# mschubert/NMFconsensus

Measured on AMD Instinct MI355X. Metric: NMF restarts/sec (k=2..10 sweep, 20k×500 fp64) + fp64-MFMA/HBM roofline %, higher is better.
Workload: dtype f64

## Files before the change

### nmfconsensus_amd/build.py

```python
from __future__ import annotations

import os
import subprocess
import sys

HERE = os.path.dirname(os.path.abspath(__file__))
ROOT = os.path.dirname(HERE)
CSRC = os.path.join(HERE, "csrc")
LIB = os.path.join(HERE, "lib", "libnmf.so")
SOURCES = ["engine.hip", "compat.hip", "brunet.hip", "generic.hip", "solo.hip", "hclust.cpp"]
HEADERS = ["nmfc_kernels.hpp", "nmfc_tuning.hpp", "nmfc_internal.hpp", "lane_pool.hpp", "rmt.hpp", "../../include/nmfc.h", "../../include/libnmf_compat.h"]
ARCH = os.environ.get("NMFC_OFFLOAD_ARCH", "gfx950")
HIPCC = os.environ.get("HIPCC", "/opt/rocm/bin/hipcc")


def source_sha256() -> str:
    import hashlib
    h = hashlib.sha256()
    for f in ("nmfc_kernels.hpp", "engine.hip", "nmfc_tuning.hpp"):
        with open(os.path.join(CSRC, f), "rb") as fh:
            h.update(fh.read())
    return h.hexdigest()


def _stale(target: str, deps: list[str]) -> bool:
    if not os.path.exists(target):
        return True
    t = os.path.getmtime(target)
    return any(os.path.getmtime(d) > t for d in deps)


def build_lib(force: bool = False, verbose: bool = True) -> str:
    os.makedirs(os.path.dirname(LIB), exist_ok=True)
    deps = [os.path.join(CSRC, s) for s in SOURCES + HEADERS]
    if not force and not _stale(LIB, deps):
        return LIB
    from concurrent.futures import ThreadPoolExecutor

    def compile_one(src):
        obj = os.path.join(CSRC, os.path.splitext(src)[0] + ".o")
        lang = [] if src.endswith(".hip") else ["-x", "c++"]
        off = [f"--offload-arch={ARCH}"] if src.endswith(".hip") else []
        cmd = [HIPCC, *off, "-O3", "-fPIC", "-std=c++17", "-Wall", "-Wno-unused-result", "-Wno-unused-function", *lang, "-c",
               os.path.join(CSRC, src), "-o", obj]
        if verbose:
            print(" ".join(cmd), file=sys.stderr)
        subprocess.run(cmd, check=True, cwd=CSRC)
        return obj

    jobs = max(1, min(len(SOURCES), int(os.environ.get("MAX_JOBS", "6"))))
    with ThreadPoolExecutor(max_workers=jobs) as pool:
        objs = list(pool.map(compile_one, SOURCES))
    cmd = [HIPCC, f"--offload-arch={ARCH}", "-shared", "-fPIC", "-o", LIB, *objs,
           "-Wl,-soname,libnmf.so", "-Wl,-rpath,/opt/rocm/lib", "-Wl,-z,defs"]
    if verbose:
        print(" ".join(cmd), file=sys.stderr)
    subprocess.run(cmd, check=True, cwd=CSRC)
    for o in objs:
        os.remove(o)
    return LIB


def build_oracle(verbose: bool = True) -> None:
    odir = os.path.join(ROOT, "oracle")
    subprocess.run(["make", "-s", "-C", odir, "liboracle.so"], check=True)
    if os.path.isdir("/root/reference/libnmf"):
        subprocess.run(["make", "-s", "-C", odir, "ref"], check=True)


if __name__ == "__main__":
    build_lib(force="--force" in sys.argv)
    build_oracle()
```

### nmfconsensus_amd/csrc/engine.hip

```cpp
#include <hip/hip_runtime.h>

#include <algorithm>
#include <chrono>
#include <climits>
#include <cmath>
#include <cstdarg>
#include <cstdio>
#include <cstdlib>
#include <cstring>
#include <string>
#include <vector>

#include "../../include/nmfc.h"
#include "nmfc_internal.hpp"
#include "nmfc_kernels.hpp"

using namespace nmfc;

namespace {

thread_local std::string g_err;

void set_err(const char* fmt, ...) {
  char buf[512];
  va_list ap;
  va_start(ap, fmt);
  vsnprintf(buf, sizeof buf, fmt, ap);
  va_end(ap);
  g_err = buf;
}

#define HCHECK(expr)                                                                        \
  do {                                                                                      \
    hipError_t e_ = (expr);                                                                 \
    if (e_ != hipSuccess) {                                                                 \
      set_err("%s failed: %s (%s:%d)", #expr, hipGetErrorString(e_), __FILE__, __LINE__); \
      return -1;                                                                            \
    }                                                                                       \
  } while (0)

long round_up(long v, long a) { return (v + a - 1) / a * a; }

struct DevBuf {
  void* p = nullptr;
  size_t bytes = 0;
  DevBuf() = default;
  DevBuf(const DevBuf&) = delete;
  DevBuf& operator=(const DevBuf&) = delete;
  ~DevBuf() { release(); }
  int ensure(size_t need) {
    if (need <= bytes) return 0;
    if (p) (void)hipFree(p);
    p = nullptr;
    bytes = 0;
    if (need == 0) return 0;
    hipError_t e = hipMalloc(&p, need);
    if (e != hipSuccess) {
      set_err("hipMalloc(%zu) failed: %s", need, hipGetErrorString(e));
      p = nullptr;
      return -1;
    }
    bytes = need;
    return 0;
  }
  void release() {
    if (p) (void)hipFree(p);
    p = nullptr;
    bytes = 0;
  }
  template <class T>
  T* as() const {
    return static_cast<T*>(p);
  }
};

void mat_mul31(const uint32_t* A, const uint32_t* B, uint32_t* C) {
  for (int i = 0; i < 31; ++i)
    for (int j = 0; j < 31; ++j) {
      uint32_t s = 0;
      for (int q = 0; q < 31; ++q) s += A[i * 31 + q] * B[q * 31 + j];
      C[i * 31 + j] = s;
    }
}

std::vector<uint32_t> make_jump_table(int nchunks, int rchunk) {
  std::vector<uint32_t> M(31 * 31, 0), P(31 * 31, 0), T(31 * 31);
  for (int q = 0; q < 30; ++q) M[q * 31 + q + 1] = 1;
  M[30 * 31 + 0] = 1;
  M[30 * 31 + 28] += 1;
  for (int i = 0; i < 31; ++i) P[i * 31 + i] = 1;
  std::vector<uint32_t> base = M;
  for (int e = rchunk; e > 0; e >>= 1) {
    if (e & 1) {
      mat_mul31(P.data(), base.data(), T.data());
      P = T;
    }
    mat_mul31(base.data(), base.data(), T.data());
    base = T;
  }
  std::vector<uint32_t> table((size_t)std::max(nchunks, 1) * 961, 0);
  for (int i = 0; i < 31; ++i) table[i * 31 + i] = 1;
  for (int c = 1; c < nchunks; ++c) mat_mul31(P.data(), &table[(size_t)(c - 1) * 961], &table[(size_t)c * 961]);
  return table;
}

enum { KID_WTA = 0, KID_HUPD = 1, KID_AHTW = 2, KID_INIT = 3, KID_OTHER = 4, KID_LABELS = 5, KID_COUNTS = 6, KID_SMALL = 7, KID_RESID = 8, KID_N = 9 };

constexpr int WTA_NPT = 4;
constexpr int NARROW_NBUF = NMFC_NARROW_NBUF;
constexpr bool WTA_MID_GREG = NMFC_WTA_MID_GREG != 0;
constexpr bool SMALL_NW8 = NMFC_SMALL_NW8 != 0;
constexpr bool WTA_GREG = NMFC_WTA_GREG != 0;
constexpr bool WTA_W16 = NMFC_WTA_W16 != 0 && WTA_GREG;
constexpr int WTA_MID_NBUF = NMFC_WTA_MID_NBUF;
constexpr int WTA_MID_MINW = NMFC_WTA_MID_MINW;
constexpr int AHTW_NBUF = NMFC_AHTW_NBUF;
constexpr bool AHTW_LATE = NMFC_AHTW_LATE != 0;
struct Packing {
  std::vector<RestartInfo> ri;
  std::vector<int> prb, pre;
  std::vector<ColInfo> ci;
  int npanels = 0;
};

Packing pack(const std::vector<RestartInfo>& in) {
  std::vector<RestartInfo> srt(in);
  std::stable_sort(srt.begin(), srt.end(), [](const RestartInfo& a, const RestartInfo& b) {
    return a.k != b.k ? a.k > b.k : a.rid < b.rid;
  });
  std::vector<int> fill;
  std::vector<std::vector<RestartInfo>> members;
  size_t first_open = 0;
  for (RestartInfo r : srt) {
    size_t b = first_open;
    while (b < fill.size() && fill[b] + r.k > 16) ++b;
    if (b == fill.size()) {
      fill.push_back(0);
      members.emplace_back();
    }
    r.col0 = (int)b * 16 + fill[b];
    fill[b] += r.k;
    members[b].push_back(r);
    while (first_open < fill.size() && fill[first_open] > 14) ++first_open;
  }
  const int nblocks = (int)members.size();
  Packing pk;
  pk.npanels = std::max(1, (nblocks + 3) / 4);
  for (int p = 0; p < pk.npanels; ++p) {
    pk.prb.push_back((int)pk.ri.size());
    for (int b = 4 * p; b < std::min(nblocks, 4 * p + 4); ++b)
      for (const RestartInfo& r : members[b]) pk.ri.push_back(r);
    pk.pre.push_back((int)pk.ri.size());
  }
  while (pk.npanels % WTA_NPT) {
    pk.prb.push_back((int)in.size());
    pk.pre.push_back((int)in.size());
    ++pk.npanels;
  }
  pk.ci.assign((size_t)pk.npanels * PANEL, ColInfo{0, 0, 0, 0});
  for (const RestartInfo& r : pk.ri)
    for (int a = 0; a < r.k; ++a) pk.ci[r.col0 + a] = ColInfo{r.sq_off, r.col0 % PANEL, r.k, r.rid};
  return pk;
}

int narrow_blocks(const Packing& pk, int maxb) {
  if (pk.ri.empty()) return 0;
  int nb = 0;
  for (const RestartInfo& r : pk.ri) {
    if (r.col0 / 16 != (r.col0 + r.k - 1) / 16) return 0;
    nb = std::max(nb, (r.col0 + r.k + 15) / 16);
  }
  return nb <= maxb ? nb : 0;
}

Packing pack_small(const std::vector<RestartInfo>& in, std::vector<SmallBlock>& blocks) {
  std::vector<RestartInfo> srt(in);
  std::stable_sort(srt.begin(), srt.end(), [](const RestartInfo& a, const RestartInfo& b) {
    return a.k != b.k ? a.k > b.k : a.rid < b.rid;
  });
  std::vector<int> fill;
  blocks.clear();
  Packing pk;
  for (RestartInfo r : srt) {
    size_t b = 0;
    while (b < fill.size() && (fill[b] + r.k > 16 || blocks[b].nr == SMALL_MAXR)) ++b;
    if (b == fill.size()) {
      fill.push_back(0);
      SmallBlock sb{};
      sb.col0 = (int)b * 16;
      blocks.push_back(sb);
    }
    SmallBlock& sb = blocks[b];
    r.col0 = sb.col0 + fill[b];
    sb.rid[sb.nr] = r.rid;
    sb.k[sb.nr] = r.k;
    sb.lc0[sb.nr] = fill[b];
    ++sb.nr;
    fill[b] += r.k;
    pk.ri.push_back(r);
  }
  pk.npanels = std::max(1, (int)((blocks.size() * 16 + PANEL - 1) / PANEL));
  while (pk.npanels % WTA_NPT) ++pk.npanels;
  pk.prb.assign(pk.npanels, 0);
  pk.pre.assign(pk.npanels, 0);
  pk.ci.assign((size_t)pk.npanels * PANEL, ColInfo{0, 0, 0, 0});
  return pk;
}

int live_panels(const Packing& pk) {
  int np = 0;
  for (int p = 0; p < pk.npanels; ++p)
    if (pk.pre[p] > pk.prb[p]) np = p + 1;
  return np;
}

std::vector<SoloJob> place_solo(Packing& pk, std::vector<RestartInfo> solo, int col_base, int n) {
  std::stable_sort(solo.begin(), solo.end(), [n](const RestartInfo& a, const RestartInfo& b) {
    const int ka = nmfc_solo_batch_rank(n, a.k), kb = nmfc_solo_batch_rank(n, b.k);
    return ka != kb ? ka > kb : a.k != b.k ? a.k > b.k : a.rid < b.rid;
  });
  std::vector<SoloJob> jobs;
  int col = col_base;
  for (RestartInfo r : solo) {
    r.col0 = col;
    col += nmfc_solo_batch_rank(n, r.k) <= 4 ? 4 : 8;
    pk.ri.push_back(r);
    jobs.push_back(SoloJob{r.col0, r.k, r.rid, 0});
  }
  pk.npanels = std::max(pk.npanels, (col + PANEL - 1) / PANEL);
  while (pk.npanels % WTA_NPT) ++pk.npanels;
  pk.prb.assign(pk.npanels, 0);
  pk.pre.assign(pk.npanels, 0);
  pk.ci.assign((size_t)pk.npanels * PANEL, ColInfo{0, 0, 0, 0});
  return jobs;
}

}

void nmfc_set_error(const char* msg) { g_err = msg; }

struct nmfc_engine {
  int dev = 0;
  hipStream_t st = nullptr;
  int m = 0, n = 0;
  long m_pad = 0, n_pad = 0, n_cols_pad = 0;
  int kchunk = 0, nsplit = 0, ngt = 0;
  int ncu = 256;
  int force_wta = -1, force_ahtw = -1;
  int repack_div = 20;
  bool narrow_ok = true;
  int narrow_maxb = 3;
  bool small_ok = true;
  int small_kernel = 0;
  DevBuf Acm, Arm, Ablk;
  DevBuf W[2], H[2], Gpart, SWpart, SH, SHP, colact, Hfin, Wfin;
  DevBuf rinfo, stop_iter, stop_reason, unchanged, classes, n_stopped, Hstat, Wsnap;
  DevBuf prb, pre, colinfo, moves, finfo;
  DevBuf initjobs, chunk_job, chunk_idx, jump, labels, slot, grp_begin, grp_list, counts_tmp, cons_tmp, smallblk;
  DevBuf teamG, teamSW, teamFlag;
  DevBuf solojobs;
  bool narrow_lc = true;
  bool wta_sk = true;
  bool wta_sk_mid = true;
  bool wta_lastsum = false;
  int sk_dp_xcd = 0;
  DevBuf skfix, skflag, sktcnt;
  unsigned sk_epoch = 0;
  bool gram_model = true;
  bool solo_ok = true;
  hipStream_t aux[4] = {nullptr, nullptr, nullptr, nullptr};
  hipEvent_t fork_ev = nullptr, join_ev[4] = {nullptr, nullptr, nullptr, nullptr};
  int team_occ = 0;
  DevBuf mu1_dev, mu1_G, mu1_SW, mu1_flag;
  char* mu1_host = nullptr;
  size_t mu1_host_bytes = 0;
  int mu1_base = -1;
  int mu1_kprev = 16;
  int jump_chunks = 0, jump_rchunk = 0;
  int* h_stopped = nullptr;
  bool timing = false;
  int timing_stride = 1;
  std::vector<hipEvent_t> ev_pool;
  struct Pending {
    int kid;
    hipEvent_t a, b;
  };
  std::vector<Pending> pending;
  double kms[KID_N] = {0};
  long long kcount[KID_N] = {0};
  long long klaunch[KID_N] = {0};
  double kflops[KID_N] = {0};
  double kbytes[KID_N] = {0};
  double kbytes_algo[KID_N] = {0};
  int repacks = 0;
  struct RunInfo {
    int small = 0, repacks_skipped = 0, polls = 0, iterations_enqueued = 0, panels_first = 0, panels_min = 0;
    long long wta_narrow = 0, wta_sk = 0, wta_big = 0, wta_mid = 0, wta_small = 0, wta_tiny = 0;
    long long ahtw_narrow = 0, ahtw_128 = 0, ahtw_64 = 0;
  } info;
  std::string info_str;
  bool residuals = false, resid_valid = false;
  DevBuf ssq, respart;
  std::vector<double> h_ssq;
  std::vector<int> last_ks, last_row;
  long last_jb = 0;
};

namespace {

struct TileChoice {
  int wta;
  bool ahtw_small;
};

constexpr double WTA_SK_COST = 1.01;
bool sk_big_ok(const nmfc_engine* e, int ntj) { return e->wta_sk && WTA_W16 && ntj >= 4; }
bool sk_mid_ok(const nmfc_engine* e, int ntj) { return e->wta_sk && e->wta_sk_mid && WTA_MID_GREG && ntj >= 4; }
bool sk_grid_fits(const nmfc_engine* e, long ngroups, int ntj) {
  const long ipc = ngroups * ntj, nitems = ipc * e->nsplit;
  const long nst_full = e->kchunk / 16, nst_last = (e->m_pad - (long)(e->nsplit - 1) * e->kchunk) / 16;
  const long nst_max = e->nsplit > 1 ? nst_full : nst_last;
  const long S = ipc * (e->nsplit - 1) * nst_full + ipc * nst_last;
  return nitems >= e->ncu && S >= (long)e->ncu * nst_max;
}
int sk_groups(const nmfc_engine* e, int tile, int big_panels, int mid_panels, int ntj) {
  const bool big = tile == 0 && sk_big_ok(e, ntj), mid = tile == 3 && sk_mid_ok(e, ntj);
  if (!big && !mid) return 0;
  const int ng = big ? (big_panels + WTA_NPT - 1) / WTA_NPT : (mid_panels + 1) / 2;
  return sk_grid_fits(e, ng, ntj) ? ng : 0;
}

TileChoice choose_tiles(const nmfc_engine* e, int np_live, int ntj) {
  const long ns = e->nsplit, cu = e->ncu;
  const long np = std::max(np_live, 1);
  struct Cand {
    int id;
    double wgs;
    long slots;
    double t;
  } cands[4] = {{0, (double)(ns * ((np + 3) / 4) * ntj), cu, 2.0},
                {3, (double)(ns * ((np + 1) / 2) * ntj), cu, 1.0},
                {1, (double)(ns * np) * (2 * ntj + (e->gram_model ? 0.75 : 0.0)), 3 * cu, 0.8},
                {2, (double)(ns * np) * (4 * ntj + (e->gram_model ? 1.5 : 0.0)), 4 * cu, 0.6}};
  TileChoice tc{0, false};
  double best = 1e300;
  for (const Cand& c : cands) {
    const bool sk = sk_groups(e, c.id, (int)np, (int)np, ntj) > 0;
    const double est = sk ? c.wgs / (double)c.slots * c.t * WTA_SK_COST : std::ceil(c.wgs / (double)c.slots) * c.t;
    if (est < best - 1e-9) {
      best = est;
      tc.wta = c.id;
    }
  }
  tc.ahtw_small = np * e->ngt < 16 * cu;
  if (e->force_wta >= 0) tc.wta = e->force_wta;
  if (e->force_ahtw >= 0) tc.ahtw_small = e->force_ahtw == 1;
  return tc;
}

template <int GBW, int NW>
hipError_t launch_small_g(nmfc_engine* e, int nblocks, int maxiter, int stop_rule) {
  const int jb = (e->n + 15) / 16;
  auto args = [&](auto kern) {
    hipLaunchKernelGGL(kern, dim3(nblocks), dim3(64 * NW), 0, e->st, e->smallblk.as<SmallBlock>(),
                       e->Arm.as<double>(), e->n_pad, e->Acm.as<double>(), e->m_pad, e->n, e->n_pad,
                       e->W[0].as<double>(), e->H[0].as<double>(), maxiter, stop_rule, e->stop_iter.as<int>(),
                       e->stop_reason.as<int>());
  };
  switch (jb) {
    case 1: args(k_small_mu<GBW, 1, 0, NW>); break;
    case 2: args(k_small_mu<GBW, 2, 0, NW>); break;
    case 3: args(k_small_mu<GBW, 3, 0, NW>); break;
    default: args(k_small_mu<GBW, 4, 0, NW>); break;
  }
  return hipGetLastError();
}

int team_count(nmfc_engine* e, int nblocks) {
  const int P = (int)(e->m_pad / TEAM_ROWS);
  if (!e->team_occ) {
    int occ = 0;
    if (hipOccupancyMaxActiveBlocksPerMultiprocessor(&occ, k_team_mu<4>, 256, 0) != hipSuccess || occ < 1) occ = 1;
    e->team_occ = std::min(occ, 6);
  }
  return std::max(1, std::min(nblocks, (int)((long)e->team_occ * e->ncu / P)));
}

int launch_team(nmfc_engine* e, int nblocks, int maxiter, int stop_rule) {
  const int jb = (e->n + 15) / 16;
  const int P = (int)(e->m_pad / TEAM_ROWS);
  if (e->m_pad % TEAM_ROWS != 0 || P > TEAM_PMAX || jb < 1 || jb > 4) {
    set_err("k_team_mu: m_pad %ld / n %d unsupported", e->m_pad, e->n);
    return -1;
  }
  auto kern = jb == 1 ? k_team_mu<1> : jb == 2 ? k_team_mu<2> : jb == 3 ? k_team_mu<3> : k_team_mu<4>;
  const int nteams = team_count(e, nblocks);
  const long np = 16L * jb;
  if (e->teamG.ensure(sizeof(double) * nteams * 2 * TEAM_PMAX * 16 * np) ||
      e->teamSW.ensure(sizeof(double) * nteams * 2 * TEAM_PMAX * 256) ||
      e->teamFlag.ensure(sizeof(unsigned) * (nteams * TEAM_PMAX + 16)))
    return -1;
  HCHECK(hipMemsetAsync(e->teamFlag.p, 0, sizeof(unsigned) * (nteams * TEAM_PMAX + 16), e->st));
  hipLaunchKernelGGL(kern, dim3(nteams * P), dim3(256), 0, e->st, e->smallblk.as<SmallBlock>(), nblocks, P,
                     e->Acm.as<double>(), e->m_pad, e->n, e->n_pad, e->W[0].as<double>(), e->H[0].as<double>(), maxiter,
                     stop_rule, e->stop_iter.as<int>(), e->stop_reason.as<int>(), e->teamG.as<double>(),
                     e->teamSW.as<double>(), e->teamFlag.as<unsigned>(), 0u,
                     reinterpret_cast<int*>(e->teamFlag.as<unsigned>() + nteams * TEAM_PMAX), nullptr);
  hipError_t err = hipGetLastError();
  if (err != hipSuccess) {
    set_err("k_team_mu launch: %s", hipGetErrorString(err));
    return -1;
  }
  return 0;
}

int team_failed(nmfc_engine* e, int nblocks) {
  int v = 0;
  const unsigned* w = e->teamFlag.as<unsigned>() + team_count(e, nblocks) * TEAM_PMAX;
  if (hipMemcpy(&v, w, sizeof(int), hipMemcpyDeviceToHost) != hipSuccess) return 1;
  return v != 0;
}

bool use_team(nmfc_engine* e, int nblocks) {
  (void)nblocks;
  return e->small_kernel == 1;
}

int launch_small(nmfc_engine* e, int nblocks, int maxiter, int stop_rule) {
  if (use_team(e, nblocks)) return launch_team(e, nblocks, maxiter, stop_rule);
  hipError_t err;
  const int jb = (e->n + 15) / 16;
  if (e->m_pad % 64 != 0 || e->n_pad != (jb <= 2 ? 32 : 64)) {
    set_err("k_small_mu: m_pad %ld / n_pad %ld unsupported for n = %d", e->m_pad, e->n_pad, e->n);
    return -1;
  }
  if (SMALL_NW8 && e->m_pad % 256 == 0) {
    switch (e->m_pad / 128) {
      case 2: err = launch_small_g<2, 8>(e, nblocks, maxiter, stop_rule); break;
      case 4: err = launch_small_g<4, 8>(e, nblocks, maxiter, stop_rule); break;
      case 6: err = launch_small_g<6, 8>(e, nblocks, maxiter, stop_rule); break;
      case 8: err = launch_small_g<8, 8>(e, nblocks, maxiter, stop_rule); break;
      default: set_err("k_small_mu: m_pad %ld unsupported", e->m_pad); return -1;
    }
  } else {
    switch (e->m_pad / 64) {
      case 2: err = launch_small_g<2, 4>(e, nblocks, maxiter, stop_rule); break;
      case 4: err = launch_small_g<4, 4>(e, nblocks, maxiter, stop_rule); break;
      case 6: err = launch_small_g<6, 4>(e, nblocks, maxiter, stop_rule); break;
      case 8: err = launch_small_g<8, 4>(e, nblocks, maxiter, stop_rule); break;
      case 10: err = launch_small_g<10, 4>(e, nblocks, maxiter, stop_rule); break;
      case 12: err = launch_small_g<12, 4>(e, nblocks, maxiter, stop_rule); break;
      case 14: err = launch_small_g<14, 4>(e, nblocks, maxiter, stop_rule); break;
      case 16: err = launch_small_g<16, 4>(e, nblocks, maxiter, stop_rule); break;
      default: set_err("k_small_mu: m_pad %ld unsupported", e->m_pad); return -1;
    }
  }
  if (err != hipSuccess) {
    set_err("k_small_mu launch: %s", hipGetErrorString(err));
    return -1;
  }
  return 0;
}

hipEvent_t take_event(nmfc_engine* e) {
  if (!e->ev_pool.empty()) {
    hipEvent_t ev = e->ev_pool.back();
    e->ev_pool.pop_back();
    return ev;
  }
  hipEvent_t ev;
  if (hipEventCreate(&ev) != hipSuccess) return nullptr;
  return ev;
}

void drain_timing(nmfc_engine* e) {
  for (auto& pnd : e->pending) {
    float ms = 0.f;
    if (hipEventSynchronize(pnd.b) == hipSuccess && hipEventElapsedTime(&ms, pnd.a, pnd.b) == hipSuccess) {
      e->kms[pnd.kid] += ms;
      e->kcount[pnd.kid] += 1;
    }
    e->ev_pool.push_back(pnd.a);
    e->ev_pool.push_back(pnd.b);
  }
  e->pending.clear();
}

struct TimedLaunch {
  nmfc_engine* e;
  int kid;
  hipEvent_t a = nullptr;
  TimedLaunch(nmfc_engine* e_, int kid_, bool sample = true) : e(e_), kid(kid_) {
    e->klaunch[kid] += 1;
    if (e->timing && sample) {
      a = take_event(e);
      if (a) (void)hipEventRecord(a, e->st);
    }
  }
  ~TimedLaunch() {
    if (a) {
      hipEvent_t b = take_event(e);
      if (b) {
        (void)hipEventRecord(b, e->st);
        e->pending.push_back({kid, a, b});
      } else {
        e->ev_pool.push_back(a);
      }
    }
  }
};


struct PollEvents {
  hipEvent_t ev[2] = {nullptr, nullptr};
  ~PollEvents() {
    for (hipEvent_t x : ev)
      if (x) (void)hipEventDestroy(x);
  }
};

struct Sweep {
  nmfc_engine* e = nullptr;
  nmfc_sweep_opts opts;
  const int* ks = nullptr;
  int nk = 0, R = 0;
  long jb = 0;
  int nj = 0;
  std::vector<RestartInfo> all;
  std::vector<int> rslot;
  std::vector<int> hoff;
  long sw_total = 0;
  bool small = false;
  Packing pk;
  std::vector<SmallBlock> sblocks;
  std::vector<SoloJob> solo;
  long cap_cols = 0;
  int ntj = 0;
  long g_ld = 0, g_split = 0, cls_ld = 0;
  bool want_w = false, tolx = false;
  int cur = 0;
  int nact = 0;
  std::vector<char> archived;
  std::vector<int> si, sr;
  int it = 0;
  int polls = 0, checked = 0;
  int stopped_at_pack = 0;
  PollEvents pe;
  long long tot_iters = 0;
  int max_it = 0;
  std::vector<RestartInfo> fin;
  int job_k(int s) const { return ks[(jb + s) % nk]; }
};

void factor_offsets(const Sweep& s, std::vector<long>& woff, std::vector<long>& ho) {
  woff.assign(s.nj + 1, 0);
  ho.assign(s.nj + 1, 0);
  for (int j = 0; j < s.nj; ++j) {
    woff[j + 1] = woff[j] + (long)s.e->m * s.job_k(j);
    ho[j + 1] = ho[j] + (long)s.job_k(j) * s.e->n;
  }
}

void transpose(const double* src, int rows, int cols, double* dst) {
  for (int r = 0; r < rows; ++r)
    for (int c = 0; c < cols; ++c) dst[(size_t)c * rows + r] = src[(size_t)r * cols + c];
}

int check_args(Sweep& s, nmfc_engine* e, const int* ks, int nk, int R, const nmfc_sweep_opts* opts_in) {
  if (!e || !ks || nk <= 0 || R <= 0) {
    set_err("nmfc_engine_run: bad arguments");
    return -1;
  }
  s.e = e;
  s.ks = ks;
  s.nk = nk;
  s.R = R;
  nmfc_sweep_opts& opts = s.opts;
  if (opts_in)
    opts = *opts_in;
  else
    nmfc_default_opts(&opts);
  if (opts.check_every <= 0) opts.check_every = 4;
  const int m = e->m, n = e->n;
  for (int i = 0; i < nk; ++i) {
    if (ks[i] < 2 || ks[i] > KMAX || ks[i] > n || ks[i] > m) {
      set_err("nmfc_engine_run: k=%d unsupported (need 2 <= k <= min(%d, m, n))", ks[i], KMAX);
      return -1;
    }
    if ((long)m * ks[i] + (long)ks[i] * n + 31L * 32 >= (long)INT_MAX) {
      set_err("nmfc_engine_run: m k + k n = %ld draws per restart exceeds the init kernel's 32-bit index range",
              (long)m * ks[i] + (long)ks[i] * n);
      return -1;
    }
  }
  if (opts.maxiter < 0) {
    set_err("nmfc_engine_run: maxiter must be >= 0");
    return -1;
  }
  if (opts.stop_rule < 0 || opts.stop_rule > 3 || opts.label_rule < 0 || opts.label_rule > 1 ||
      opts.init_stream < 0 || opts.init_stream > 1) {
    set_err("nmfc_engine_run: bad stop rule, label rule or init stream");
    return -1;
  }
  HCHECK(hipSetDevice(e->dev));
  return 0;
}

int plan_jobs(Sweep& s) {
  nmfc_engine* e = s.e;
  const int m = e->m, n = e->n;
  const long njobs_all = (long)s.nk * s.R;
  const long jb = std::max(0, s.opts.job_begin);
  const long je = (s.opts.job_end < 0) ? njobs_all : std::min<long>(s.opts.job_end, njobs_all);
  if (jb >= je) {
    set_err("nmfc_engine_run: empty job range [%ld, %ld)", jb, je);
    return -1;
  }
  s.jb = jb;
  const int nj = s.nj = (int)(je - jb);

  std::vector<int> order(nj);
  for (int i = 0; i < nj; ++i) order[i] = i;
  std::stable_sort(order.begin(), order.end(), [&](int a, int b) { return s.job_k(a) > s.job_k(b); });
  s.all.resize(nj);
  s.rslot.resize(nj);
  s.hoff.assign(nj + 1, 0);
  for (int rid = 0; rid < nj; ++rid) {
    RestartInfo& r = s.all[rid];
    r.k = s.job_k(order[rid]);
    r.rid = rid;
    r.sq_off = (int)s.sw_total;
    r.col0 = 0;
    s.rslot[rid] = order[rid];
    s.sw_total += (long)r.k * r.k;
    s.hoff[rid + 1] = s.hoff[rid] + r.k;
  }
  s.small = e->small_ok && e->m_pad <= 1024 && n <= 64 && s.opts.stop_rule != NMFC_STOP_TOLX;
  std::vector<RestartInfo> blk_jobs, solo_jobs;
  for (const RestartInfo& r : s.all)
    (s.small && e->solo_ok && nmfc_mu_solo_fits(m, n, r.k) ? solo_jobs : blk_jobs).push_back(r);
  s.pk = s.small ? pack_small(blk_jobs, s.sblocks) : pack(s.all);
  if (s.small && !solo_jobs.empty()) s.solo = place_solo(s.pk, solo_jobs, (int)s.sblocks.size() * 16, n);
  s.cap_cols = (long)s.pk.npanels * PANEL;
  e->info.small = s.small;
  e->info.panels_first = e->info.panels_min = s.pk.npanels;
  s.ntj = (int)(e->n_cols_pad / 128);
  s.g_ld = e->n_cols_pad;
  s.g_split = s.cap_cols * s.g_ld;
  s.cls_ld = std::max<long>(n, KMAX);
  s.tolx = s.opts.stop_rule == NMFC_STOP_TOLX;
  s.nact = nj;
  s.archived.assign(nj, 0);
  s.si.assign(nj, 0);
  s.sr.assign(nj, 0);
  return 0;
}

int upload_packing(nmfc_engine* e, const Packing& p) {
  hipStream_t st = e->st;
  HCHECK(hipMemcpyAsync(e->rinfo.p, p.ri.data(), sizeof(RestartInfo) * std::max<size_t>(p.ri.size(), 1),
                        hipMemcpyHostToDevice, st));
  HCHECK(hipMemcpyAsync(e->prb.p, p.prb.data(), sizeof(int) * p.npanels, hipMemcpyHostToDevice, st));
  HCHECK(hipMemcpyAsync(e->pre.p, p.pre.data(), sizeof(int) * p.npanels, hipMemcpyHostToDevice, st));
  HCHECK(hipMemcpyAsync(e->colinfo.p, p.ci.data(), sizeof(ColInfo) * p.ci.size(), hipMemcpyHostToDevice, st));
  return 0;
}

int ensure_buffers(Sweep& s) {
  nmfc_engine* e = s.e;
  const int n = e->n, nj = s.nj;
  const long cap_cols = s.cap_cols, fin_rows = s.hoff[nj];
  const Packing& pk = s.pk;
  if (e->W[0].ensure(sizeof(double) * cap_cols * e->m_pad) || e->H[0].ensure(sizeof(double) * cap_cols * e->n_pad) ||
      e->W[1].ensure(sizeof(double) * cap_cols * e->m_pad) || e->H[1].ensure(sizeof(double) * cap_cols * e->n_pad) ||
      e->Gpart.ensure(sizeof(double) * s.g_split * e->nsplit) || e->SWpart.ensure(sizeof(double) * s.sw_total * e->nsplit) ||
      e->SH.ensure(sizeof(double) * s.sw_total) || e->Hfin.ensure(sizeof(double) * fin_rows * e->n_pad) ||
      e->SHP.ensure(sizeof(double) * cap_cols * KMAX) || e->colact.ensure(sizeof(int) * cap_cols) ||
      (s.want_w && e->Wfin.ensure(sizeof(double) * fin_rows * e->m_pad)) || e->rinfo.ensure(sizeof(RestartInfo) * nj) ||
      e->finfo.ensure(sizeof(RestartInfo) * nj) || e->stop_iter.ensure(sizeof(int) * nj) ||
      e->stop_reason.ensure(sizeof(int) * nj) || e->unchanged.ensure(sizeof(int) * nj) ||
      e->classes.ensure(sizeof(int) * nj * s.cls_ld) || e->n_stopped.ensure(sizeof(int)) ||
      e->prb.ensure(sizeof(int) * pk.npanels) || e->pre.ensure(sizeof(int) * pk.npanels) ||
      e->colinfo.ensure(sizeof(ColInfo) * pk.npanels * PANEL) ||
      e->moves.ensure(sizeof(MoveJob) * nj) || e->labels.ensure(sizeof(int32_t) * (size_t)nj * n) ||
      e->slot.ensure(sizeof(int) * nj) || e->Hstat.ensure(sizeof(double) * nj))
    return -1;
  if (s.tolx && e->Wsnap.ensure(sizeof(double) * cap_cols * e->m_pad)) return -1;
  hipStream_t st = e->st;
  if (upload_packing(e, pk)) return -1;
  HCHECK(hipMemcpyAsync(e->slot.p, s.rslot.data(), sizeof(int) * nj, hipMemcpyHostToDevice, st));
  HCHECK(hipMemsetAsync(e->stop_iter.p, 0, sizeof(int) * nj, st));
  HCHECK(hipMemsetAsync(e->stop_reason.p, 0, sizeof(int) * nj, st));
  HCHECK(hipMemsetAsync(e->unchanged.p, 0, sizeof(int) * nj, st));
  HCHECK(hipMemsetAsync(e->classes.p, 0, sizeof(int) * nj * s.cls_ld, st));
  HCHECK(hipMemsetAsync(e->n_stopped.p, 0, sizeof(int), st));
  HCHECK(hipMemsetAsync(e->colact.p, 0, sizeof(int) * cap_cols, st));
  HCHECK(hipMemsetAsync(e->W[0].p, 0, sizeof(double) * cap_cols * e->m_pad, st));
  HCHECK(hipMemsetAsync(e->H[0].p, 0, sizeof(double) * cap_cols * e->n_pad, st));
  HCHECK(hipMemsetAsync(e->W[1].p, 0, sizeof(double) * cap_cols * e->m_pad, st));
  HCHECK(hipMemsetAsync(e->H[1].p, 0, sizeof(double) * cap_cols * e->n_pad, st));
  return 0;
}

int init_from_caller(Sweep& s, const double* W_init, const double* H_init) {
  nmfc_engine* e = s.e;
  hipStream_t st = e->st;
  const int m = e->m, n = e->n;
  std::vector<long> woff, ho;
  factor_offsets(s, woff, ho);
  std::vector<double> hrow;
  for (const RestartInfo& r : s.pk.ri) {
    const int j = s.rslot[r.rid], k = r.k;
    HCHECK(hipMemcpy2DAsync(e->W[0].as<double>() + (long)r.col0 * e->m_pad, sizeof(double) * e->m_pad,
                            W_init + woff[j], sizeof(double) * m, sizeof(double) * m, k, hipMemcpyHostToDevice, st));
    hrow.assign((size_t)k * n, 0.0);
    transpose(H_init + ho[j], n, k, hrow.data());
    HCHECK(hipMemcpy2DAsync(e->H[0].as<double>() + (long)r.col0 * e->n_pad, sizeof(double) * e->n_pad, hrow.data(),
                            sizeof(double) * n, sizeof(double) * n, k, hipMemcpyHostToDevice, st));
    HCHECK(hipStreamSynchronize(st));
  }
  return 0;
}

int init_r_runif(Sweep& s) {
  nmfc_engine* e = s.e;
  hipStream_t st = e->st;
  const int nj = s.nj;
  std::vector<InitJob> ij(nj);
  for (int i = 0; i < nj; ++i) {
    const RestartInfo& r = s.pk.ri[i];
    ij[i] = InitJob{(uint32_t)(s.opts.seed + (uint32_t)(s.jb + s.rslot[r.rid])), r.col0, r.k, 0};
  }
  if (e->initjobs.ensure(sizeof(InitJob) * nj)) return -1;
  HCHECK(hipMemcpyAsync(e->initjobs.p, ij.data(), sizeof(InitJob) * nj, hipMemcpyHostToDevice, st));
  {
    TimedLaunch tl(e, KID_INIT);
    hipLaunchKernelGGL(k_init_runif, dim3(nj), dim3(NT), 0, st, e->initjobs.as<InitJob>(), e->m, e->n, e->m_pad,
                       e->n_pad, e->W[0].as<double>(), e->H[0].as<double>());
  }
  HCHECK(hipGetLastError());
  HCHECK(hipStreamSynchronize(st));
  return 0;
}

int init_glibc(Sweep& s) {
  nmfc_engine* e = s.e;
  hipStream_t st = e->st;
  const int m = e->m, n = e->n, nj = s.nj;
  const Packing& pk = s.pk;
  std::vector<InitJob> ij(nj);
  std::vector<int> cj, ci;
  int maxch = 1;
  long draws = 0;
  for (int i = 0; i < nj; ++i) draws += (long)m * pk.ri[i].k + (long)pk.ri[i].k * n;
  int rchunk = RCHUNK;
  while (rchunk > 62 && draws / rchunk < 65536) rchunk /= 2;
  for (int i = 0; i < nj; ++i) {
    const RestartInfo& r = pk.ri[i];
    const long total = (long)m * r.k + (long)r.k * n;
    const int nch = (int)((total + rchunk - 1) / rchunk);
    ij[i].seed = (uint32_t)(s.opts.seed + (uint32_t)(s.jb + s.rslot[r.rid]));
    ij[i].col0 = r.col0;
    ij[i].k = r.k;
    ij[i].nchunks = nch;
    maxch = std::max(maxch, nch);
    for (int c = 0; c < nch; ++c) {
      cj.push_back(i);
      ci.push_back(c);
    }
  }
  if (maxch > e->jump_chunks || rchunk != e->jump_rchunk) {
    std::vector<uint32_t> tab = make_jump_table(maxch, rchunk);
    if (e->jump.ensure(sizeof(uint32_t) * tab.size())) return -1;
    HCHECK(hipMemcpyAsync(e->jump.p, tab.data(), sizeof(uint32_t) * tab.size(), hipMemcpyHostToDevice, st));
    HCHECK(hipStreamSynchronize(st));
    e->jump_chunks = maxch;
    e->jump_rchunk = rchunk;
  }
  if (e->initjobs.ensure(sizeof(InitJob) * nj) || e->chunk_job.ensure(sizeof(int) * cj.size()) ||
      e->chunk_idx.ensure(sizeof(int) * ci.size()))
    return -1;
  HCHECK(hipMemcpyAsync(e->initjobs.p, ij.data(), sizeof(InitJob) * nj, hipMemcpyHostToDevice, st));
  HCHECK(hipMemcpyAsync(e->chunk_job.p, cj.data(), sizeof(int) * cj.size(), hipMemcpyHostToDevice, st));
  HCHECK(hipMemcpyAsync(e->chunk_idx.p, ci.data(), sizeof(int) * ci.size(), hipMemcpyHostToDevice, st));
  const int total_chunks = (int)cj.size();
  {
    TimedLaunch tl(e, KID_INIT);
    hipLaunchKernelGGL(k_init, dim3((total_chunks + NT - 1) / NT), dim3(NT), 0, st, e->initjobs.as<InitJob>(),
                       e->chunk_job.as<int>(), e->chunk_idx.as<int>(), total_chunks, e->jump.as<uint32_t>(), rchunk / 31,
                       m, n, e->m_pad, e->n_pad, s.opts.min_init, s.opts.max_init, e->W[0].as<double>(),
                       e->H[0].as<double>());
  }
  HCHECK(hipGetLastError());
  HCHECK(hipStreamSynchronize(st));
  return 0;
}

int archive(Sweep& s, const std::vector<RestartInfo>& list) {
  if (list.empty()) return 0;
  nmfc_engine* e = s.e;
  hipStream_t st = e->st;
  std::vector<MoveJob> mv(list.size());
  for (size_t x = 0; x < list.size(); ++x) mv[x] = {list[x].col0, s.hoff[list[x].rid], list[x].k};
  HCHECK(hipMemcpyAsync(e->moves.p, mv.data(), sizeof(MoveJob) * mv.size(), hipMemcpyHostToDevice, st));
  {
    TimedLaunch tl(e, KID_OTHER);
    hipLaunchKernelGGL(k_move_rows, dim3((unsigned)mv.size(), 2), dim3(NT), 0, st, e->moves.as<MoveJob>(),
                       e->H[s.cur].as<double>(), e->n_pad, e->Hfin.as<double>(), e->n_pad, e->n_pad);
    if (s.want_w)
      hipLaunchKernelGGL(k_move_rows, dim3((unsigned)mv.size(), 16), dim3(NT), 0, st, e->moves.as<MoveJob>(),
                         e->W[s.cur].as<double>(), e->m_pad, e->Wfin.as<double>(), e->m_pad, e->m_pad);
  }
  HCHECK(hipGetLastError());
  HCHECK(hipStreamSynchronize(st));
  for (const RestartInfo& r : list) s.archived[r.rid] = 1;
  return 0;
}

int archive_rest(Sweep& s) {
  std::vector<RestartInfo> rest;
  for (const RestartInfo& r : s.pk.ri)
    if (!s.archived[r.rid]) rest.push_back(r);
  return archive(s, rest);
}

int launch_solo_beside_blocks(Sweep& s) {
  nmfc_engine* e = s.e;
  const int n = e->n;
  const std::vector<SoloJob>& solo = s.solo;
  const long free_cu = std::max<long>(1, e->ncu - (long)s.sblocks.size());
  auto wt = [](int kp) -> long { return kp <= 2 ? 4 : kp <= 4 ? 6 : 12; };
  long wsum = 0;
  for (const SoloJob& job : solo) wsum += wt(nmfc_solo_batch_rank(n, job.k));
  std::vector<std::pair<size_t, size_t>> groups;
  for (size_t g0 = 0; g0 < solo.size();) {
    const int kp = nmfc_solo_batch_rank(n, solo[g0].k);
    size_t g1 = g0;
    while (g1 < solo.size() && nmfc_solo_batch_rank(n, solo[g1].k) == kp) ++g1;
    groups.emplace_back(g0, g1);
    g0 = g1;
  }
  for (int g = 0; g < (int)groups.size(); ++g) {
    const size_t g0 = groups[g].first, g1 = groups[g].second;
    const int kp = nmfc_solo_batch_rank(n, solo[g0].k);
    const long nq = (long)(g1 - g0);
    const long share = std::min<long>(nq, std::max<long>(1, free_cu * nq * wt(kp) / wsum));
    HCHECK(hipStreamWaitEvent(e->aux[g], e->fork_ev, 0));
    if (nmfc_solo_batch_launch(e->Acm.as<double>(), e->m_pad, e->m, n, e->W[0].as<double>(), e->m_pad,
                               e->H[0].as<double>(), e->n_pad, e->solojobs.as<SoloJob>() + g0, (int)nq, kp,
                               s.opts.maxiter, s.opts.stop_rule, e->stop_iter.as<int>(), e->stop_reason.as<int>(),
                               (int)share, e->aux[g]))
      return -1;
    HCHECK(hipEventRecord(e->join_ev[g], e->aux[g]));
  }
  for (int g = 0; g < (int)groups.size(); ++g) HCHECK(hipStreamWaitEvent(e->st, e->join_ev[g], 0));
  return 0;
}

int small_phase(Sweep& s) {
  nmfc_engine* e = s.e;
  hipStream_t st = e->st;
  const std::vector<SmallBlock>& sblocks = s.sblocks;
  const std::vector<SoloJob>& solo = s.solo;
  if (!sblocks.empty()) {
    if (e->smallblk.ensure(sizeof(SmallBlock) * sblocks.size())) return -1;
    HCHECK(hipMemcpyAsync(e->smallblk.p, sblocks.data(), sizeof(SmallBlock) * sblocks.size(), hipMemcpyHostToDevice, st));
  }
  if (!solo.empty()) {
    if (e->solojobs.ensure(sizeof(SoloJob) * solo.size())) return -1;
    HCHECK(hipMemcpyAsync(e->solojobs.p, solo.data(), sizeof(SoloJob) * solo.size(), hipMemcpyHostToDevice, st));
    for (int x = 0; x < 4; ++x) {
      if (!e->aux[x]) HCHECK(hipStreamCreateWithFlags(&e->aux[x], hipStreamNonBlocking));
      if (!e->join_ev[x]) HCHECK(hipEventCreateWithFlags(&e->join_ev[x], hipEventDisableTiming));
    }
    if (!e->fork_ev) HCHECK(hipEventCreateWithFlags(&e->fork_ev, hipEventDisableTiming));
  }
  {
    TimedLaunch tl(e, KID_SMALL);
    const bool team = use_team(e, (int)sblocks.size());
    if (!solo.empty() && !team) HCHECK(hipEventRecord(e->fork_ev, st));
    if (!sblocks.empty() && launch_small(e, (int)sblocks.size(), s.opts.maxiter, s.opts.stop_rule)) return -1;
    if (!solo.empty() && (sblocks.empty() || team)) {
      if (nmfc_solo_batch_launch(e->Acm.as<double>(), e->m_pad, e->m, e->n, e->W[0].as<double>(), e->m_pad,
                                 e->H[0].as<double>(), e->n_pad, e->solojobs.as<SoloJob>(), (int)solo.size(), 0,
                                 s.opts.maxiter, s.opts.stop_rule, e->stop_iter.as<int>(), e->stop_reason.as<int>(),
                                 (int)solo.size(), st))
        return -1;
    } else if (!solo.empty()) {
      if (launch_solo_beside_blocks(s)) return -1;
    }
  }
  HCHECK(hipStreamSynchronize(st));
  if (!sblocks.empty() && use_team(e, (int)sblocks.size()) && team_failed(e, (int)sblocks.size())) {
    set_err("k_team_mu: a team of workgroups could not meet (not co-resident?)");
    return -1;
  }
  if (e->timing) drain_timing(e);
  s.it = s.opts.maxiter;
  return 0;
}


using Wta2Kernel = decltype(&k_wta2<1, 64, 2, 2, 1, GT_NBUF, 1, true, true, true>);
using AhtwKernel = decltype(&k_ahtw4<GT, AHTW_NBUF, 1, PANEL, 4, AHTW_LATE>);

void launch_wta_narrow(const Sweep& s, int nblk) {
  nmfc_engine* e = s.e;
  const int ntq = (int)(e->n_cols_pad / 16);
  auto kn = e->narrow_lc ? k_wta_narrow_lc<16, NARROW_NBUF, true> : k_wta_narrow<16, NARROW_NBUF, true>;
  ++e->info.wta_narrow;
  hipLaunchKernelGGL(kn, dim3(e->nsplit * nblk * (ntq + 1)), dim3(e->narrow_lc ? 128 : 64), 0, e->st,
                     e->W[s.cur].as<double>(), e->Ablk.as<double>(), e->m_pad, ntq, e->nsplit, e->kchunk, nblk,
                     e->colinfo.as<ColInfo>(), e->Gpart.as<double>(), s.g_ld, s.g_split, e->SWpart.as<double>(),
                     s.sw_total);
}

int launch_wta_sk(Sweep& s, bool big, int ng, int* gsplit) {
  nmfc_engine* e = s.e;
  hipStream_t st = e->st;
  if (!e->skflag.p) {
    if (e->skfix.ensure(sizeof(double) * SK_FIX * e->ncu) || e->skflag.ensure(sizeof(unsigned) * e->ncu)) return -1;
    HCHECK(hipMemsetAsync(e->skflag.p, 0, sizeof(unsigned) * e->ncu, st));
  }
  ++e->info.wta_sk;
  const long tiles = (long)ng * s.ntj;
  const bool lastsum = e->wta_lastsum && big;
  if (lastsum && e->sktcnt.bytes < sizeof(unsigned) * tiles) {
    if (e->sktcnt.ensure(sizeof(unsigned) * tiles)) return -1;
    HCHECK(hipMemsetAsync(e->sktcnt.p, 0, sizeof(unsigned) * tiles, st));
  }
  const SkArgs a{e->W[s.cur].as<double>(), e->Ablk.as<double>(), e->m_pad, ng, s.ntj, e->kchunk,
                 e->prb.as<int>(), e->pre.as<int>(), e->rinfo.as<RestartInfo>(), e->colinfo.as<ColInfo>(),
                 e->stop_iter.as<int>(), e->Gpart.as<double>(), s.g_ld, s.g_split, e->SWpart.as<double>(), s.sw_total,
                 e->skfix.as<double>(), e->skflag.as<unsigned>(), ++e->sk_epoch, e->nsplit,
                 e->sktcnt.as<unsigned>(), e->sk_dp_xcd};
  if (!big) {
    hipLaunchKernelGGL((k_wta2_sk<WTA_MID_NBUF, false, false, 2>), dim3(e->ncu), dim3(SK_THREADS / 2), 0, st, a);
  } else if (lastsum) {
    hipLaunchKernelGGL((k_wta2_sk<GT_NBUF, false, true>), dim3(e->ncu), dim3(SK_THREADS), 0, st, a);
    *gsplit = 1;
  } else {
    hipLaunchKernelGGL(k_wta2_sk<GT_NBUF>, dim3(e->ncu), dim3(SK_THREADS), 0, st, a);
  }
  return 0;
}

struct Wta2Launch {
  Wta2Kernel kern;
  int threads;
  int ngroups;
  int tiles;
  int gram_wgs;
  int tile;
};

Wta2Launch pick_wta2(const nmfc_engine* e, int tile, int ntj, int live, int npanels) {
  const int lp = std::max(1, live);
  if (tile == 0) {
    Wta2Kernel kw = (ntj >= 4)   ? (WTA_W16 ? k_wta2<WTA_NPT, 128, 4, 4, 1, GT_NBUF, 1, true, true, false, true>
                                            : k_wta2<WTA_NPT, 128, 4, 2, 1, GT_NBUF, 1, true, true, false, WTA_GREG>)
                    : (ntj >= 2) ? k_wta2<WTA_NPT, 128, 4, 2, 2, GT_NBUF, 1, true>
                                 : k_wta2<WTA_NPT, 128, 4, 2, 4, GT_NBUF, 1, true>;
    return {kw, (ntj >= 4 && WTA_W16) ? 1024 : 512, npanels / WTA_NPT, ntj, 0, 0};
  }
  if (tile == 3) {
    Wta2Kernel kw = (ntj >= 4 && WTA_MID_GREG) ? k_wta2<2, 128, 2, 4, 1, WTA_MID_NBUF, WTA_MID_MINW, true, true, false, true>
                    : (ntj >= 2)               ? k_wta2<2, 128, 4, 2, 1, WTA_MID_NBUF, WTA_MID_MINW, true>
                                               : k_wta2<2, 128, 4, 2, 2, WTA_MID_NBUF, WTA_MID_MINW, true>;
    return {kw, 512, (lp + 1) / 2, ntj, 0, 3};
  }
  if (tile != 2)
    return {k_wta2<1, 64, 2, 2, 1, GT_NBUF, 1, true, true, true>, 256, lp, 2 * ntj, 3, 1};
  Wta2Kernel kw = (long)e->nsplit * live * 4 * ntj <= e->ncu ? k_wta2<1, 32, 4, 1, 1, 8, 1, true, true, true>
                                                             : k_wta2<1, 32, 4, 1, 1, GT_NBUF, 1, true, true, true>;
  return {kw, 256, lp, 4 * ntj, 3, 2};
}

void launch_wta2(const Sweep& s, const Wta2Launch& l) {
  nmfc_engine* e = s.e;
  ++(l.tile == 0 ? e->info.wta_big : l.tile == 3 ? e->info.wta_mid : l.tile == 1 ? e->info.wta_small : e->info.wta_tiny);
  hipLaunchKernelGGL(l.kern, dim3(e->nsplit * l.ngroups * (l.tiles + l.gram_wgs)), dim3(l.threads), 0, e->st,
                     e->W[s.cur].as<double>(), e->Ablk.as<double>(), e->m_pad, l.ngroups, l.tiles, e->nsplit, e->kchunk,
                     e->prb.as<int>(), e->pre.as<int>(), e->rinfo.as<RestartInfo>(), e->colinfo.as<ColInfo>(),
                     e->stop_iter.as<int>(), e->Gpart.as<double>(), s.g_ld, s.g_split, e->SWpart.as<double>(),
                     s.sw_total);
}

struct ChunkPlan {
  TileChoice tc;
  int nblk;
  int live;
  int lp;
  int ngt_ahtw, grid_ahtw;
  AhtwKernel ka;
};

int launch_wta(Sweep& s, const ChunkPlan& cp, int* gsplit) {
  if (cp.nblk > 0) {
    launch_wta_narrow(s, cp.nblk);
  } else if (const int ng = sk_groups(s.e, cp.tc.wta, s.pk.npanels, cp.lp, s.ntj)) {
    return launch_wta_sk(s, cp.tc.wta == 0, ng, gsplit);
  } else {
    launch_wta2(s, pick_wta2(s.e, cp.tc.wta, s.ntj, cp.live, s.pk.npanels));
  }
  return 0;
}

void launch_hupdate(const Sweep& s, int iter, int gsplit) {
  nmfc_engine* e = s.e;
  hipLaunchKernelGGL(k_hupdate<>, dim3(s.nact), dim3(NTH), 0, e->st, iter, s.opts.maxiter, s.opts.stop_rule,
                     e->rinfo.as<RestartInfo>(), e->n, e->n_pad, e->Gpart.as<double>(), s.g_ld, s.g_split, gsplit,
                     e->nsplit, e->SWpart.as<double>(), s.sw_total, e->H[s.cur].as<double>(), e->SH.as<double>(),
                     e->stop_iter.as<int>(), e->stop_reason.as<int>(), e->unchanged.as<int>(),
                     e->classes.as<int>(), s.cls_ld, e->n_stopped.as<int>(), e->SHP.as<double>(),
                     e->colact.as<int>(), e->Hstat.as<double>());
}

void launch_ahtw(const Sweep& s, const ChunkPlan& cp, int iter) {
  nmfc_engine* e = s.e;
  ++(cp.nblk > 0 ? e->info.ahtw_narrow : cp.tc.ahtw_small ? e->info.ahtw_64 : e->info.ahtw_128);
  if (cp.nblk > 0)
    hipLaunchKernelGGL((k_ahtw4<GT / 4, GT_NBUF, 1, 16, 2>), dim3(4 * e->ngt * cp.nblk), dim3(128), 0, e->st,
                       iter, e->H[s.cur].as<double>(), e->n_pad, e->Arm.as<double>(), e->m_pad,
                       e->W[s.cur].as<double>(), e->SHP.as<double>(), e->colinfo.as<ColInfo>(),
                       e->colact.as<int>(), cp.nblk, 4 * e->ngt);
  else
    hipLaunchKernelGGL(cp.ka, dim3(cp.grid_ahtw), dim3(256), 0, e->st, iter, e->H[s.cur].as<double>(), e->n_pad,
                       e->Arm.as<double>(), e->m_pad, e->W[s.cur].as<double>(), e->SHP.as<double>(),
                       e->colinfo.as<ColInfo>(), e->colact.as<int>(), cp.lp, cp.ngt_ahtw);
}

ChunkPlan plan_chunk(const Sweep& s) {
  const nmfc_engine* e = s.e;
  ChunkPlan cp;
  cp.live = live_panels(s.pk);
  cp.lp = std::max(1, cp.live);
  cp.tc = choose_tiles(e, cp.live, s.ntj);
  cp.nblk = e->narrow_ok ? narrow_blocks(s.pk, e->narrow_maxb) : 0;
  cp.ngt_ahtw = e->ngt * (cp.tc.ahtw_small ? 2 : 1);
  cp.grid_ahtw = cp.lp * cp.ngt_ahtw;
  const bool kh = AHTW_KSKIP && AHTW_NBUF == 2 && e->n_pad - e->n >= 8;
  cp.ka = cp.tc.ahtw_small ? (kh ? k_ahtw4<GT / 2, AHTW_NBUF, 1, PANEL, 4, AHTW_LATE, AHTW_NBUF == 2>
                                 : k_ahtw4<GT / 2, AHTW_NBUF, 1, PANEL, 4, AHTW_LATE>)
                           : (kh ? k_ahtw4<GT, AHTW_NBUF, 1, PANEL, 4, AHTW_LATE, AHTW_NBUF == 2>
                                 : k_ahtw4<GT, AHTW_NBUF, 1, PANEL, 4, AHTW_LATE>);
  return cp;
}

void launch_wstat(const Sweep& s, int iter) {
  nmfc_engine* e = s.e;
  hipLaunchKernelGGL(k_wstat, dim3(s.nact), dim3(NT), 0, e->st, iter, e->rinfo.as<RestartInfo>(),
                     e->W[s.cur].as<double>(), e->Wsnap.as<double>(), e->m_pad, e->m, e->colact.as<int>(),
                     e->Hstat.as<double>(), s.opts.TolX, s.opts.TolFun, e->stop_iter.as<int>(),
                     e->stop_reason.as<int>(), e->n_stopped.as<int>());
}

int enqueue_iteration(Sweep& s, const ChunkPlan& cp, int iter) {
  nmfc_engine* e = s.e;
  const bool sample = iter % e->timing_stride == 0;
  int gsplit = e->nsplit;
  {
    TimedLaunch tl(e, KID_WTA, sample);
    if (launch_wta(s, cp, &gsplit)) return -1;
  }
  {
    TimedLaunch tl(e, KID_HUPD, sample);
    launch_hupdate(s, iter, gsplit);
  }
  const bool tol_check = s.tolx && iter > 1 && iter % 2 == 0;
  if (tol_check)
    HCHECK(hipMemcpyAsync(e->Wsnap.p, e->W[s.cur].p, sizeof(double) * (size_t)s.pk.npanels * PANEL * e->m_pad,
                          hipMemcpyDeviceToDevice, e->st));
  {
    TimedLaunch tl(e, KID_AHTW, sample);
    launch_ahtw(s, cp, iter);
  }
  if (tol_check) {
    TimedLaunch tl(e, KID_OTHER);
    launch_wstat(s, iter);
  }
  return 0;
}

int enqueue_chunk(Sweep& s) {
  nmfc_engine* e = s.e;
  const int chunk = std::min(s.opts.check_every, s.opts.maxiter - s.it);
  const ChunkPlan cp = plan_chunk(s);
  for (int c = 1; c <= chunk; ++c)
    if (enqueue_iteration(s, cp, s.it + c)) return -1;
  HCHECK(hipGetLastError());
  s.it += chunk;
  HCHECK(hipMemcpyAsync(&e->h_stopped[s.polls & 1], e->n_stopped.p, sizeof(int), hipMemcpyDeviceToHost, e->st));
  HCHECK(hipEventRecord(s.pe.ev[s.polls & 1], e->st));
  ++s.polls;
  return 0;
}

int consume_polls(Sweep& s, int* stopped, bool* done) {
  const int target = (s.it < s.opts.maxiter) ? s.polls - 1 : s.polls;
  while (s.checked < target) {
    HCHECK(hipEventSynchronize(s.pe.ev[s.checked & 1]));
    *stopped = s.e->h_stopped[s.checked & 1];
    if (*stopped >= s.nj) *done = true;
    ++s.checked;
  }
  return 0;
}

int repack(Sweep& s, int stopped) {
  nmfc_engine* e = s.e;
  hipStream_t st = e->st;
  const int nj = s.nj;
  HCHECK(hipStreamSynchronize(st));
  if (e->timing) drain_timing(e);
  s.checked = s.polls;
  HCHECK(hipMemcpy(s.si.data(), e->stop_iter.p, sizeof(int) * nj, hipMemcpyDeviceToHost));
  std::vector<RestartInfo> gone, live;
  for (const RestartInfo& r : s.pk.ri) {
    if (!s.si[r.rid])
      live.push_back(r);
    else if (!s.archived[r.rid])
      gone.push_back(r);
  }
  if (archive(s, gone)) return -1;
  Packing np = pack(live);
  if ((long)np.npanels * PANEL > s.cap_cols) {
    s.stopped_at_pack = stopped;
    ++e->info.repacks_skipped;
    return 0;
  }
  std::vector<int> old_col(nj, -1);
  for (const RestartInfo& r : live) old_col[r.rid] = r.col0;
  std::vector<MoveJob> mv(np.ri.size());
  for (size_t x = 0; x < np.ri.size(); ++x) mv[x] = {old_col[np.ri[x].rid], np.ri[x].col0, np.ri[x].k};
  if (!mv.empty()) {
    HCHECK(hipMemcpyAsync(e->moves.p, mv.data(), sizeof(MoveJob) * mv.size(), hipMemcpyHostToDevice, st));
    {
      TimedLaunch tl(e, KID_OTHER);
      hipLaunchKernelGGL(k_move_rows, dim3((unsigned)mv.size(), 16), dim3(NT), 0, st, e->moves.as<MoveJob>(),
                         e->W[s.cur].as<double>(), e->m_pad, e->W[s.cur ^ 1].as<double>(), e->m_pad, e->m_pad);
      hipLaunchKernelGGL(k_move_rows, dim3((unsigned)mv.size(), 2), dim3(NT), 0, st, e->moves.as<MoveJob>(),
                         e->H[s.cur].as<double>(), e->n_pad, e->H[s.cur ^ 1].as<double>(), e->n_pad, e->n_pad);
    }
    HCHECK(hipGetLastError());
  }
  s.cur ^= 1;
  s.pk = np;
  if (upload_packing(e, s.pk)) return -1;
  HCHECK(hipStreamSynchronize(st));
  s.nact = (int)s.pk.ri.size();
  s.stopped_at_pack = nj - s.nact;
  ++e->repacks;
  e->info.panels_min = std::min(e->info.panels_min, s.pk.npanels);
  return 0;
}

int mfma_loop(Sweep& s) {
  nmfc_engine* e = s.e;
  HCHECK(hipEventCreateWithFlags(&s.pe.ev[0], hipEventDisableTiming));
  HCHECK(hipEventCreateWithFlags(&s.pe.ev[1], hipEventDisableTiming));
  for (;;) {
    if (s.it < s.opts.maxiter && enqueue_chunk(s)) return -1;
    int stopped = 0;
    bool done = false;
    if (consume_polls(s, &stopped, &done)) return -1;
    if (e->timing) drain_timing(e);
    if (done || (s.it >= s.opts.maxiter && s.checked == s.polls)) break;
    if (stopped - s.stopped_at_pack >= std::max(1, s.nact / e->repack_div)) {
      if (repack(s, stopped)) return -1;
      if (s.nact == 0) break;
    }
  }
  return 0;
}

int residual_pass(Sweep& s) {
  nmfc_engine* e = s.e;
  if (!e->residuals) return 0;
  hipStream_t st = e->st;
  const int nj = s.nj;
  const int nst = (e->n + RES_ST - 1) / RES_ST, ntiles = (e->m + RES_GT - 1) / RES_GT * nst;
  const int ngroups = (nj + RES_JG - 1) / RES_JG;
  if (ngroups > 65535) {
    set_err("nmfc_engine_run: residuals of %d jobs exceed the residual pass's grid", nj);
    return -1;
  }
  if (e->ssq.ensure(sizeof(double) * nj) || e->respart.ensure(sizeof(double) * (size_t)nj * ntiles)) return -1;
  s.fin.resize(nj);
  for (int rid = 0; rid < nj; ++rid) s.fin[rid] = {s.hoff[rid], s.all[rid].k, rid, s.all[rid].sq_off};
  HCHECK(hipMemcpyAsync(e->finfo.p, s.fin.data(), sizeof(RestartInfo) * nj, hipMemcpyHostToDevice, st));
  {
    TimedLaunch tl(e, KID_RESID);
    hipLaunchKernelGGL(k_resid, dim3(ntiles, ngroups), dim3(NT), 0, st, e->finfo.as<RestartInfo>(), nj,
                       e->Ablk.as<double>(), e->n_cols_pad, e->Wfin.as<double>(), e->m_pad, e->Hfin.as<double>(), e->n_pad,
                       e->m, e->n, nst, e->respart.as<double>());
    hipLaunchKernelGGL(k_resid_sum, dim3(nj), dim3(64), 0, st, e->respart.as<double>(), ntiles, e->slot.as<int>(),
                       e->ssq.as<double>());
  }
  HCHECK(hipGetLastError());
  e->h_ssq.assign(nj, 0.0);
  HCHECK(hipMemcpyAsync(e->h_ssq.data(), e->ssq.p, sizeof(double) * nj, hipMemcpyDeviceToHost, st));
  double fl = 0, bw = 0, bh = 0;
  for (int rid = 0; rid < nj; ++rid) {
    const double k = s.all[rid].k;
    fl += (2.0 * k + 3.0) * e->m * e->n;
    bw += 8.0 * k * e->m;
    bh += 8.0 * k * e->n;
  }
  const double a_bytes = 8.0 * e->m * e->n;
  e->kflops[KID_RESID] = fl;
  e->kbytes_algo[KID_RESID] = a_bytes + bw + bh + 8.0 * nj;
  e->kbytes[KID_RESID] = a_bytes * ngroups + bw * nst + bh * (ntiles / nst) + 16.0 * nj * ntiles + 8.0 * nj;
  return 0;
}

int labels_counts_consensus(Sweep& s, nmfc_result* out) {
  nmfc_engine* e = s.e;
  hipStream_t st = e->st;
  const int n = e->n, nj = s.nj, nk = s.nk;
  std::vector<RestartInfo> fin(nj);
  for (int rid = 0; rid < nj; ++rid) fin[rid] = {s.hoff[rid], s.all[rid].k, rid, s.all[rid].sq_off};
  HCHECK(hipMemcpyAsync(e->finfo.p, fin.data(), sizeof(RestartInfo) * nj, hipMemcpyHostToDevice, st));
  {
    TimedLaunch tl(e, KID_LABELS);
    hipLaunchKernelGGL(k_labels, dim3((n + NT - 1) / NT, nj), dim3(NT), 0, st, e->finfo.as<RestartInfo>(),
                       e->slot.as<int>(), e->Hfin.as<double>(), e->n_pad, n, s.opts.label_rule, e->labels.as<int32_t>());
  }
  HCHECK(hipGetLastError());
  std::vector<int> gb(nk + 1, 0), gl;
  for (int g = 0; g < nk; ++g) {
    gb[g] = (int)gl.size();
    for (int j = 0; j < nj; ++j)
      if ((s.jb + j) % nk == g) gl.push_back(j);
  }
  gb[nk] = (int)gl.size();
  const size_t cnt_len = (size_t)nk * n * n;
  if (out && (out->counts || out->consensus)) {
    if (e->grp_begin.ensure(sizeof(int) * (nk + 1)) || e->grp_list.ensure(sizeof(int) * std::max<size_t>(gl.size(), 1)))
      return -1;
    HCHECK(hipMemcpyAsync(e->grp_begin.p, gb.data(), sizeof(int) * (nk + 1), hipMemcpyHostToDevice, st));
    if (!gl.empty()) HCHECK(hipMemcpyAsync(e->grp_list.p, gl.data(), sizeof(int) * gl.size(), hipMemcpyHostToDevice, st));
    int32_t* dcounts;
    if (out->counts && out->counts_on_device) {
      dcounts = out->counts;
    } else {
      if (e->counts_tmp.ensure(sizeof(int32_t) * cnt_len)) return -1;
      dcounts = e->counts_tmp.as<int32_t>();
    }
    {
      TimedLaunch tl(e, KID_COUNTS);
      hipLaunchKernelGGL(k_counts, dim3((n + CNT_T - 1) / CNT_T, (n + CNT_T - 1) / CNT_T, nk), dim3(NT), 0, st, e->labels.as<int32_t>(),
                         e->grp_begin.as<int>(), e->grp_list.as<int>(), n, dcounts);
    }
    HCHECK(hipGetLastError());
    if (out->consensus) {
      if (e->cons_tmp.ensure(sizeof(double) * cnt_len)) return -1;
      hipLaunchKernelGGL(k_divide, dim3((unsigned)((cnt_len + NT - 1) / NT)), dim3(NT), 0, st, dcounts, (double)s.R,
                         (long)cnt_len, e->cons_tmp.as<double>());
      HCHECK(hipGetLastError());
      HCHECK(hipMemcpyAsync(out->consensus, e->cons_tmp.p, sizeof(double) * cnt_len, hipMemcpyDeviceToHost, st));
    }
    if (out->counts && !out->counts_on_device)
      HCHECK(hipMemcpyAsync(out->counts, dcounts, sizeof(int32_t) * cnt_len, hipMemcpyDeviceToHost, st));
  }
  HCHECK(hipMemcpyAsync(s.si.data(), e->stop_iter.p, sizeof(int) * nj, hipMemcpyDeviceToHost, st));
  HCHECK(hipMemcpyAsync(s.sr.data(), e->stop_reason.p, sizeof(int) * nj, hipMemcpyDeviceToHost, st));
  if (out && out->labels)
    HCHECK(hipMemcpyAsync(out->labels, e->labels.p, sizeof(int32_t) * (size_t)nj * n, hipMemcpyDeviceToHost, st));
  HCHECK(hipStreamSynchronize(st));
  if (e->timing) drain_timing(e);
  return 0;
}

void account_kernels(Sweep& s, nmfc_result* out) {
  nmfc_engine* e = s.e;
  const int m = e->m, n = e->n, nj = s.nj;
  double fl_wta = 0, fl_ahtw = 0;
  double b_wta = 0, ba_wta = 0, b_ahtw = 0, ba_ahtw = 0, b_hupd = 0, ba_hupd = 0, b_lab = 0;
  const double ns = e->nsplit;
  for (int rid = 0; rid < nj; ++rid) {
    const int itr = s.si[rid] ? s.si[rid] : s.it;
    s.tot_iters += itr;
    s.max_it = std::max(s.max_it, itr);
    const double k = s.all[rid].k;
    fl_wta += (double)itr * (2.0 * m * n * k + 2.0 * m * k * k);
    fl_ahtw += (double)itr * (2.0 * m * n * k + 2.0 * m * k * k);
    ba_wta += itr * 8.0 * k * (m + n);
    b_wta += itr * 8.0 * k * (m + ns * n + ns * k);
    ba_ahtw += itr * 8.0 * k * (2.0 * m + n);
    b_ahtw += itr * 8.0 * k * (2.0 * m + n + KMAX);
    ba_hupd += itr * 32.0 * n * k;
    b_hupd += itr * 8.0 * (k * n * (ns + 2.0) + k * k * (ns + 2.0) + k * KMAX);
    b_lab += 8.0 * k * n + 4.0 * n;
    if (out && out->iters) out->iters[s.rslot[rid]] = itr;
    if (out && out->stopped_early) out->stopped_early[s.rslot[rid]] = (s.sr[rid] == 1 || s.sr[rid] == 3);
  }
  const double a_bytes = 8.0 * m * n;
  if (const long long c = e->klaunch[KID_WTA]) {
    e->kflops[KID_WTA] = fl_wta / c;
    e->kbytes_algo[KID_WTA] = a_bytes + ba_wta / c;
    e->kbytes[KID_WTA] = a_bytes + b_wta / c;
  }
  if (const long long c = e->klaunch[KID_AHTW]) {
    e->kflops[KID_AHTW] = fl_ahtw / c;
    e->kbytes_algo[KID_AHTW] = a_bytes + ba_ahtw / c;
    e->kbytes[KID_AHTW] = a_bytes + b_ahtw / c;
  }
  if (const long long c = e->klaunch[KID_SMALL]) {
    e->kflops[KID_SMALL] = (fl_wta + fl_ahtw) / c;
    e->kbytes_algo[KID_SMALL] = (ba_wta + ba_ahtw + ba_hupd) / c;
    e->kbytes[KID_SMALL] = e->kbytes_algo[KID_SMALL];
  }
  if (const long long c = e->klaunch[KID_HUPD]) {
    e->kbytes_algo[KID_HUPD] = ba_hupd / c;
    e->kbytes[KID_HUPD] = b_hupd / c;
  }
  if (e->klaunch[KID_LABELS]) e->kbytes[KID_LABELS] = e->kbytes_algo[KID_LABELS] = b_lab;
  if (e->klaunch[KID_COUNTS]) {
    e->kbytes_algo[KID_COUNTS] = 4.0 * nj * n + 4.0 * s.nk * n * n;
    e->kbytes[KID_COUNTS] = e->kbytes_algo[KID_COUNTS];
  }
}

int download_factors(Sweep& s, nmfc_result* out) {
  if (!out || !(out->W || out->H)) return 0;
  nmfc_engine* e = s.e;
  hipStream_t st = e->st;
  const int m = e->m, n = e->n;
  std::vector<long> woff, ho;
  factor_offsets(s, woff, ho);
  std::vector<double> hrow;
  for (int rid = 0; rid < s.nj; ++rid) {
    const int j = s.rslot[rid], k = s.all[rid].k;
    if (out->W)
      HCHECK(hipMemcpy2DAsync(out->W + woff[j], sizeof(double) * m, e->Wfin.as<double>() + (long)s.hoff[rid] * e->m_pad,
                              sizeof(double) * e->m_pad, sizeof(double) * m, k, hipMemcpyDeviceToHost, st));
    if (out->H) {
      hrow.assign((size_t)k * n, 0.0);
      HCHECK(hipMemcpy2DAsync(hrow.data(), sizeof(double) * n, e->Hfin.as<double>() + (long)s.hoff[rid] * e->n_pad,
                              sizeof(double) * e->n_pad, sizeof(double) * n, k, hipMemcpyDeviceToHost, st));
      HCHECK(hipStreamSynchronize(st));
      transpose(hrow.data(), k, n, out->H + ho[j]);
    }
  }
  HCHECK(hipStreamSynchronize(st));
  return 0;
}

}

extern "C" {

const char* nmfc_last_error(void) { return g_err.c_str(); }

const char* nmfc_build_tuning(void) { return NMFC_TUNING_MU; }
const char* nmfc_version(void) { return "nmfconsensus_amd 0.2 (gfx950, fp64 MFMA)"; }

void nmfc_default_opts(nmfc_sweep_opts* o) {
  memset(o, 0, sizeof *o);
  o->maxiter = 10000;
  o->stop_rule = NMFC_STOP_REF_COMPAT;
  o->label_rule = NMFC_LABEL_ARGMAX;
  o->seed = 123;
  o->min_init = 0;
  o->max_init = 1;
  o->job_begin = 0;
  o->job_end = -1;
  o->check_every = 4;
  o->verbose = 0;
  o->TolX = 1.0E-04;
  o->TolFun = 1.0E-04;
}

nmfc_engine* nmfc_engine_create(int device, const double* A, int m, int n, int a_on_device) {
  if (!A || m <= 0 || n <= 0) {
    set_err("nmfc_engine_create: bad arguments (A=%p m=%d n=%d)", (const void*)A, m, n);
    return nullptr;
  }
  nmfc_engine* e = new nmfc_engine();
  auto fail = [&](const char* what, hipError_t err) -> nmfc_engine* {
    set_err("nmfc_engine_create: %s: %s", what, hipGetErrorString(err));
    nmfc_engine_destroy(e);
    return nullptr;
  };
  hipError_t err;
  if (device >= 0) {
    if ((err = hipSetDevice(device)) != hipSuccess) return fail("hipSetDevice", err);
  }
  if ((err = hipGetDevice(&e->dev)) != hipSuccess) return fail("hipGetDevice", err);
  {
    int ncu = 0;
    if (hipDeviceGetAttribute(&ncu, hipDeviceAttributeMultiprocessorCount, e->dev) == hipSuccess && ncu > 0) e->ncu = ncu;
  }
  if (const char* s = getenv("NMFC_WTA_TILE")) {
    const std::string v(s);
    e->force_wta = v == "big" ? 0 : v == "small" ? 1 : v == "tiny" ? 2 : v == "mid" ? 3 : -1;
  }
  if (const char* s = getenv("NMFC_REPACK_DIV")) e->repack_div = std::max(1, atoi(s));
  if (const char* s = getenv("NMFC_NARROW")) e->narrow_ok = atoi(s) != 0;
  if (const char* s = getenv("NMFC_NARROW_MAXB")) e->narrow_maxb = std::min(8, std::max(1, atoi(s)));
  if (const char* s = getenv("NMFC_SMALL")) e->small_ok = atoi(s) != 0;
  if (const char* s = getenv("NMFC_SOLO")) e->solo_ok = atoi(s) != 0;
  if (const char* s = getenv("NMFC_NARROW_LC")) e->narrow_lc = atoi(s) != 0;
  if (const char* s = getenv("NMFC_WTA_SK")) e->wta_sk = atoi(s) != 0;
  if (const char* s = getenv("NMFC_WTA_SK_MID")) e->wta_sk_mid = atoi(s) != 0;
  if (const char* s = getenv("NMFC_WTA_LASTSUM")) e->wta_lastsum = atoi(s) != 0;
  if (const char* s = getenv("NMFC_SK_DP_XCD")) e->sk_dp_xcd = atoi(s) != 0;
  if (const char* s = getenv("NMFC_GRAM_MODEL")) e->gram_model = atoi(s) != 0;
  if (const char* s = getenv("NMFC_SMALL_KERNEL"))
    e->small_kernel = std::string(s) == "team" ? 1 : std::string(s) == "single" ? 2 : 0;
  if (const char* s = getenv("NMFC_AHTW_TILE")) {
    const std::string v(s);
    e->force_ahtw = v == "128" ? 0 : v == "64" ? 1 : -1;
  }
  if ((err = hipStreamCreateWithFlags(&e->st, hipStreamNonBlocking)) != hipSuccess) return fail("hipStreamCreate", err);
  if ((err = hipHostMalloc((void**)&e->h_stopped, 2 * sizeof(int), 0)) != hipSuccess) return fail("hipHostMalloc", err);
  e->m = m;
  e->n = n;
  e->m_pad = round_up(m, GT);
  e->n_pad = round_up(n, BK);
  e->n_cols_pad = round_up(n, 128);
  e->ngt = (int)(e->m_pad / GT);
  int kchunk = 2048;
  if (const char* v = getenv("NMFC_KCHUNK")) {
    const int x = atoi(v);
    if (x == 512 || x == 1024 || x == 2048 || x == 4096) kchunk = x;
  }
  e->kchunk = (int)std::min<long>(kchunk, e->m_pad);
  e->nsplit = (int)((e->m_pad + e->kchunk - 1) / e->kchunk);
  const bool small_shape = e->m_pad <= (long)TEAM_ROWS * TEAM_PMAX && n <= 64;
  if ((small_shape && e->Acm.ensure(sizeof(double) * e->n_cols_pad * e->m_pad)) ||
      e->Ablk.ensure(sizeof(double) * e->n_cols_pad * e->m_pad) || e->Arm.ensure(sizeof(double) * e->m_pad * e->n_pad)) {
    nmfc_engine_destroy(e);
    return nullptr;
  }
  if (small_shape && (err = hipMemsetAsync(e->Acm.p, 0, e->Acm.bytes, e->st)) != hipSuccess) return fail("memset", err);
  if ((err = hipMemsetAsync(e->Ablk.p, 0, e->Ablk.bytes, e->st)) != hipSuccess) return fail("memset", err);
  if ((err = hipMemsetAsync(e->Arm.p, 0, e->Arm.bytes, e->st)) != hipSuccess) return fail("memset", err);
  const double* dA = A;
  DevBuf tmp;
  if (!a_on_device) {
    if (tmp.ensure(sizeof(double) * (size_t)m * n)) {
      nmfc_engine_destroy(e);
      return nullptr;
    }
    if ((err = hipMemcpyAsync(tmp.p, A, sizeof(double) * (size_t)m * n, hipMemcpyHostToDevice, e->st)) != hipSuccess)
      return fail("upload A", err);
    dA = tmp.as<double>();
  }
  dim3 grid((m + NT - 1) / NT, n);
  hipLaunchKernelGGL(k_layout_a, grid, dim3(NT), 0, e->st, dA, (long)m, m, n, e->m_pad, e->n_pad,
                     small_shape ? e->Acm.as<double>() : nullptr, e->Arm.as<double>());
  hipLaunchKernelGGL(k_layout_ablk, dim3((unsigned)((m + NT - 1) / NT), (unsigned)((n + 15) / 16)), dim3(NT), 0,
                     e->st, dA, (long)m, m, n, e->n_cols_pad, e->Ablk.as<double>());
  if ((err = hipGetLastError()) != hipSuccess) return fail("k_layout_a", err);
  if ((err = hipStreamSynchronize(e->st)) != hipSuccess) return fail("sync", err);
  tmp.release();
  return e;
}

void nmfc_engine_destroy(nmfc_engine* e) {
  if (!e) return;
  if (e->st) (void)hipStreamSynchronize(e->st);
  drain_timing(e);
  for (auto ev : e->ev_pool) (void)hipEventDestroy(ev);
  for (int x = 0; x < 4; ++x) {
    if (e->aux[x]) (void)hipStreamDestroy(e->aux[x]);
    if (e->join_ev[x]) (void)hipEventDestroy(e->join_ev[x]);
  }
  if (e->fork_ev) (void)hipEventDestroy(e->fork_ev);
  if (e->h_stopped) (void)hipHostFree(e->h_stopped);
  if (e->mu1_host) (void)hipHostFree(e->mu1_host);
  if (e->st) (void)hipStreamDestroy(e->st);
  delete e;
}

int nmfc_engine_device(const nmfc_engine* e) { return e ? e->dev : -1; }

int nmfc_current_device(void) {
  int d = -1;
  return hipGetDevice(&d) == hipSuccess ? d : -1;
}

void nmfc_engine_set_timing(nmfc_engine* e, int enable) {
  if (!e) return;
  e->timing = enable > 0;
  e->timing_stride = std::max(1, enable);
}

void nmfc_engine_set_residuals(nmfc_engine* e, int enable) {
  if (e) e->residuals = enable != 0;
}

namespace {
double resid_norm(const nmfc_engine* e, int slot) { return sqrt(e->h_ssq[slot]) / sqrt((double)e->m * e->n); }

int resid_ready(const nmfc_engine* e, const char* who) {
  if (!e) {
    set_err("%s: no engine", who);
    return -1;
  }
  if (!e->resid_valid) {
    set_err("%s: the last run on this engine had residuals disabled or failed (nmfc_engine_set_residuals)", who);
    return -1;
  }
  return 0;
}
}

int nmfc_engine_residuals(nmfc_engine* e, double* dnorm_out) {
  if (resid_ready(e, "nmfc_engine_residuals")) return -1;
  if (!dnorm_out) {
    set_err("nmfc_engine_residuals: dnorm_out is NULL");
    return -1;
  }
  const int nj = (int)e->h_ssq.size();
  for (int j = 0; j < nj; ++j) dnorm_out[j] = resid_norm(e, j);
  return nj;
}

int nmfc_engine_best(nmfc_engine* e, int32_t* best_job_out, double* best_dnorm_out, double* W_out, double* H_out) {
  if (resid_ready(e, "nmfc_engine_best")) return -1;
  const int nk = (int)e->last_ks.size(), nj = (int)e->h_ssq.size(), m = e->m, n = e->n;
  std::vector<int> best(nk, -1);
  std::vector<double> bd(nk, NAN);
  for (int j = 0; j < nj; ++j) {
    const int g = (int)((e->last_jb + j) % nk);
    const double d = resid_norm(e, j);
    if (best[g] < 0 || d < bd[g]) {
      best[g] = j;
      bd[g] = d;
    }
  }
  if (W_out || H_out) HCHECK(hipSetDevice(e->dev));
  std::vector<double> hrow;
  long woff = 0, hoff = 0;
  for (int g = 0; g < nk; ++g) {
    const int k = e->last_ks[g], j = best[g];
    if (best_job_out) best_job_out[g] = j < 0 ? -1 : (int32_t)(e->last_jb + j);
    if (best_dnorm_out) best_dnorm_out[g] = bd[g];
    if (j >= 0 && W_out)
      HCHECK(hipMemcpy2DAsync(W_out + woff, sizeof(double) * m, e->Wfin.as<double>() + (long)e->last_row[j] * e->m_pad,
                              sizeof(double) * e->m_pad, sizeof(double) * m, k, hipMemcpyDeviceToHost, e->st));
    if (j >= 0 && H_out) {
      hrow.assign((size_t)k * n, 0.0);
      HCHECK(hipMemcpy2DAsync(hrow.data(), sizeof(double) * n, e->Hfin.as<double>() + (long)e->last_row[j] * e->n_pad,
                              sizeof(double) * e->n_pad, sizeof(double) * n, k, hipMemcpyDeviceToHost, e->st));
      HCHECK(hipStreamSynchronize(e->st));
      transpose(hrow.data(), k, n, H_out + hoff);
    }
    woff += (long)m * k;
    hoff += (long)k * n;
  }
  HCHECK(hipStreamSynchronize(e->st));
  return nk;
}

long long nmfc_engine_kernel_time(nmfc_engine* e, int kid, double* ms_out) {
  if (!e || kid < 0 || kid >= KID_N) return -1;
  if (ms_out) *ms_out = e->kms[kid];
  return e->kcount[kid];
}

double nmfc_engine_kernel_flops(nmfc_engine* e, int kid) {
  if (!e || kid < 0 || kid >= KID_N) return 0.0;
  return e->kflops[kid];
}

double nmfc_engine_kernel_bytes(nmfc_engine* e, int kid, double* algo_bytes_out) {
  if (!e || kid < 0 || kid >= KID_N) return 0.0;
  if (algo_bytes_out) *algo_bytes_out = e->kbytes_algo[kid];
  return e->kbytes[kid];
}

const char* nmfc_engine_run_info(nmfc_engine* e) {
  if (!e) return "";
  const nmfc_engine::RunInfo& i = e->info;
  char buf[640];
  snprintf(buf, sizeof buf,
           "small=%d;repacks=%d;repacks_skipped=%d;polls=%d;iterations_enqueued=%d;panels_first=%d;panels_min=%d;"
           "wta_narrow=%lld;wta_sk=%lld;wta_big=%lld;wta_mid=%lld;wta_small=%lld;wta_tiny=%lld;"
           "ahtw_narrow=%lld;ahtw_128=%lld;ahtw_64=%lld",
           i.small, e->repacks, i.repacks_skipped, i.polls, i.iterations_enqueued, i.panels_first, i.panels_min,
           i.wta_narrow, i.wta_sk, i.wta_big, i.wta_mid, i.wta_small, i.wta_tiny, i.ahtw_narrow, i.ahtw_128, i.ahtw_64);
  e->info_str = buf;
  return e->info_str.c_str();
}

int nmfc_engine_run(nmfc_engine* e, const int* ks, int nk, int R, const nmfc_sweep_opts* opts_in,
                    const double* W_init, const double* H_init, nmfc_result* out) {
  using clk = std::chrono::steady_clock;
  Sweep s;
  if (e) e->resid_valid = false;
  if (check_args(s, e, ks, nk, R, opts_in)) return -1;
  const auto t_start = clk::now();
  for (int x = 0; x < KID_N; ++x) {
    e->kms[x] = 0;
    e->kcount[x] = 0;
    e->klaunch[x] = 0;
    e->kflops[x] = 0;
    e->kbytes[x] = 0;
    e->kbytes_algo[x] = 0;
  }
  e->repacks = 0;
  e->info = nmfc_engine::RunInfo();
  s.want_w = (out && out->W) || e->residuals;
  if (plan_jobs(s) || ensure_buffers(s)) return -1;
  if (W_init && H_init ? init_from_caller(s, W_init, H_init)
                       : s.opts.init_stream == NMFC_INIT_R_RUNIF ? init_r_runif(s) : init_glibc(s))
    return -1;

  const auto t_iter0 = clk::now();
  if (s.small ? small_phase(s) : mfma_loop(s)) return -1;
  HCHECK(hipStreamSynchronize(e->st));
  if (e->timing) drain_timing(e);
  e->info.polls = s.polls;
  e->info.iterations_enqueued = s.it;
  const auto t_iter1 = clk::now();

  if (archive_rest(s) || residual_pass(s) || labels_counts_consensus(s, out)) return -1;
  account_kernels(s, out);
  if (download_factors(s, out)) return -1;
  if (e->residuals) {
    e->last_ks.assign(ks, ks + nk);
    e->last_jb = s.jb;
    e->last_row.assign(s.nj, 0);
    for (int rid = 0; rid < s.nj; ++rid) e->last_row[s.rslot[rid]] = s.hoff[rid];
    e->resid_valid = true;
  }
  const auto t_end = clk::now();
  if (out) {
    out->seconds_total = std::chrono::duration<double>(t_end - t_start).count();
    out->seconds_iterate = std::chrono::duration<double>(t_iter1 - t_iter0).count();
    out->restart_iterations = s.tot_iters;
    out->max_iter_run = s.max_it;
  }
  if (s.opts.verbose) {
    fprintf(stderr, "[nmfc] %d restarts, %d iterations enqueued, max %d, mean %.1f, %d repacks, %.3f s\n", s.nj,
            e->info.iterations_enqueued, s.max_it, (double)s.tot_iters / s.nj, e->repacks, std::chrono::duration<double>(t_end - t_start).count());
  }
  return 0;
}

int nmfc_engine_mu1(nmfc_engine* e, int k, int maxiter, int stop_rule, const double* W0, const double* H0,
                    double* W_out, double* H_out, int* iters, int* early) {
  if (!e || !W0 || !H0 || !W_out || !H_out || maxiter < 0 || k < 1 || k > 16 || k > e->m || k > e->n ||
      !nmfc_mu_stop_rule_ok(stop_rule)) {
    set_err("nmfc_engine_mu1: bad arguments");
    return -1;
  }
  const int m = e->m, n = e->n;
  const int jb = (n + 15) / 16;
  const int P = (int)(e->m_pad / TEAM_ROWS);
  if (!e->small_ok || e->small_kernel == 2 || n > 64 || P > TEAM_PMAX) {
    set_err("nmfc_engine_mu1: shape %d x %d is not a team shape (m rounded up to 128 <= %d, n <= 64)", m, n,
            TEAM_ROWS * TEAM_PMAX);
    return -1;
  }
  HCHECK(hipSetDevice(e->dev));
  const long mp = e->m_pad, np = e->n_pad;
  const size_t off_stop = 256, off_w = 512, off_h = off_w + sizeof(double) * 16 * mp;
  const size_t total = off_h + sizeof(double) * 16 * np;
  if (e->mu1_host_bytes < total) {
    if (e->mu1_host) (void)hipHostFree(e->mu1_host);
    e->mu1_host = nullptr;
    e->mu1_host_bytes = 0;
    HCHECK(hipHostMalloc((void**)&e->mu1_host, total, 0));
    memset(e->mu1_host, 0, total);
    e->mu1_host_bytes = total;
    e->mu1_kprev = 16;
  }
  if (e->mu1_dev.ensure(total) || e->mu1_G.ensure(sizeof(double) * 2 * TEAM_PMAX * 16 * 16 * jb) ||
      e->mu1_SW.ensure(sizeof(double) * 2 * TEAM_PMAX * 256))
    return -1;
  if (!e->mu1_flag.p) e->mu1_base = -1;
  if (e->mu1_flag.ensure(sizeof(unsigned) * TEAM_PMAX)) return -1;
  if (e->mu1_base < 0 || e->mu1_base > (1 << 30)) {
    HCHECK(hipMemsetAsync(e->mu1_flag.p, 0, sizeof(unsigned) * TEAM_PMAX, e->st));
    e->mu1_base = 0;
  }
  char* hb = e->mu1_host;
  SmallBlock blk{};
  blk.col0 = 0;
  blk.nr = 1;
  blk.rid[0] = 0;
  blk.k[0] = k;
  blk.lc0[0] = 0;
  memcpy(hb, &blk, sizeof(blk));
  int* hstop = reinterpret_cast<int*>(hb + off_stop);
  hstop[0] = hstop[1] = hstop[2] = 0;
  double* hw = reinterpret_cast<double*>(hb + off_w);
  double* hh = reinterpret_cast<double*>(hb + off_h);
  for (int c = 0; c < k; ++c) memcpy(hw + c * mp, W0 + (long)c * m, sizeof(double) * m);
  for (int c = 0; c < k; ++c)
    for (int j = 0; j < n; ++j) hh[c * np + j] = H0[c + (long)j * k];
  if (e->mu1_kprev > k) {
    memset(hw + k * mp, 0, sizeof(double) * (e->mu1_kprev - k) * mp);
    memset(hh + k * np, 0, sizeof(double) * (e->mu1_kprev - k) * np);
  }
  e->mu1_kprev = k;
  char* db = static_cast<char*>(e->mu1_dev.p);
  HCHECK(hipMemcpyAsync(db, hb, total, hipMemcpyHostToDevice, e->st));
  auto kern = jb == 1 ? k_team_mu<1> : jb == 2 ? k_team_mu<2> : jb == 3 ? k_team_mu<3> : k_team_mu<4>;
  int* dstop = reinterpret_cast<int*>(db + off_stop);
  hipLaunchKernelGGL(kern, dim3(P), dim3(256), 0, e->st, reinterpret_cast<const SmallBlock*>(db), 1, P, e->Acm.as<double>(),
                     mp, n, np, reinterpret_cast<double*>(db + off_w), reinterpret_cast<double*>(db + off_h), maxiter,
                     stop_rule, dstop, dstop + 1, e->mu1_G.as<double>(), e->mu1_SW.as<double>(),
                     e->mu1_flag.as<unsigned>(), (unsigned)e->mu1_base, dstop + 2, nullptr);
  HCHECK(hipGetLastError());
  HCHECK(hipMemcpyAsync(hb + off_stop, db + off_stop, total - off_stop, hipMemcpyDeviceToHost, e->st));
  HCHECK(hipStreamSynchronize(e->st));
  if (hstop[2]) {
    e->mu1_base = -1;
    set_err("k_team_mu: the team could not meet (not co-resident?)");
    return -1;
  }
  const int it = maxiter == 0 ? 0 : hstop[0];
  e->mu1_base += it;
  for (int c = 0; c < k; ++c) memcpy(W_out + (long)c * m, hw + c * mp, sizeof(double) * m);
  for (int c = 0; c < k; ++c)
    for (int j = 0; j < n; ++j) H_out[c + (long)j * k] = hh[c * np + j];
  if (iters) *iters = it;
  if (early) *early = hstop[1] == 1;
  return 0;
}

int nmfc_consensus(const double* Hs, int k, int n, int R, int label_rule, int32_t* labels, int32_t* counts,
                   double* consensus) {
  if (!Hs || k < 1 || n < 1 || R < 1 || label_rule < 0 || label_rule > 1) {
    set_err("nmfc_consensus: bad arguments");
    return -1;
  }
  std::vector<double> hrows((size_t)R * k * n);
  for (int r = 0; r < R; ++r)
    for (int j = 0; j < n; ++j)
      for (int a = 0; a < k; ++a) hrows[((size_t)r * k + a) * n + j] = Hs[(size_t)r * k * n + (size_t)j * k + a];
  std::vector<RestartInfo> ri(R);
// ... 41 lines not shown
```

### nmfconsensus_amd/csrc/nmfc_kernels.hpp

```cpp
#pragma once
#include <hip/hip_runtime.h>
#include <stdint.h>

#include <type_traits>

#include "nmfc_tuning.hpp"
#include "rmt.hpp"

namespace nmfc {

typedef double d4 __attribute__((ext_vector_type(4)));
typedef double d2 __attribute__((ext_vector_type(2)));
typedef unsigned int u32x2 __attribute__((__vector_size__(2 * sizeof(unsigned int))));

constexpr int PANEL = 64;
constexpr int BK = 32;
constexpr int NT = 256;
constexpr int KMAX = 16;
constexpr int GT = 128;
constexpr int STOP_FIXED = 0, STOP_REF_COMPAT = 1, STOP_ARGMAX_STABLE = 2, STOP_TOLX = 3;
constexpr double SQRTEPS = 1.0536712127723509e-08;
constexpr double DIV_BY_ZERO_AVOIDANCE = 1E-09;

__device__ __forceinline__ double mu_rule(double old, double num, double den) {
  if (old == 0.0 || num == 0.0) return 0.0;
  const double q = num / (den + DIV_BY_ZERO_AVOIDANCE);
  const double t = old * q;
  return t < 0.0 ? 0.0 : t;
}

__device__ __forceinline__ int wave_id() { return __builtin_amdgcn_readfirstlane(threadIdx.x >> 6); }
__device__ __forceinline__ int lane_id() { return (int)__builtin_amdgcn_mbcnt_hi(~0u, __builtin_amdgcn_mbcnt_lo(~0u, 0u)); }

__device__ __forceinline__ double mu_rule_sel(double old, double num, double den) {
  const double q = num / (den + DIV_BY_ZERO_AVOIDANCE);
  const double t = old * q;
  return (old == 0.0 || num == 0.0 || t < 0.0) ? 0.0 : t;
}

__device__ __forceinline__ int xcd_item(int b, int nblocks) {
  const int xcd = b & 7, idx = b >> 3;
  const int q = nblocks >> 3, r = nblocks & 7;
  return (xcd < r ? xcd * (q + 1) : r * (q + 1) + (xcd - r) * q) + idx;
}

constexpr int BK2 = 16;
constexpr int GT_NBUF = 3;
constexpr bool GT_PRIO = NMFC_GT_PRIO != 0;

__device__ __forceinline__ void lds_dma16(__amdgpu_buffer_rsrc_t r, uint32_t lds_addr, int voff, int soff) {
  __builtin_amdgcn_raw_ptr_buffer_load_lds(r, (__attribute__((address_space(3))) void*)(uintptr_t)lds_addr, 16, voff,
                                           soff, 0, 0);
}

template <int N>
__device__ __forceinline__ void wait_vmcnt() {
  asm volatile("s_waitcnt vmcnt(%0)" ::"n"(N) : "memory");
}

__device__ __forceinline__ void step_barrier() {
  asm volatile("s_waitcnt lgkmcnt(0)" ::: "memory");
  __builtin_amdgcn_s_barrier();
  asm volatile("" ::: "memory");
}

template <int RP, int RQ, int WR, int WC, int NBUF = GT_NBUF, bool QBLK = false, bool GREG = false, bool SPLIT = true,
          bool OPQ = false>
struct GTile {
  static_assert(NBUF >= 2 && NBUF <= 16, "ring of 2..16 stages");
  static constexpr int NW = WR * WC;
  static constexpr int NTH = NW * 64;
  static constexpr int STAGE_BYTES = (RP + RQ) * BK2 * 8;
  static constexpr int LDS_BYTES = NBUF * STAGE_BYTES;
  static constexpr int PIECES = (RP + RQ) / 8;
  static constexpr int PPW = PIECES / NW;
  static constexpr int PPW_P = RP / 8 / NW;
  static_assert(PIECES % NW == 0 && (RP / 8) % NW == 0, "pieces must split evenly over waves");
  static constexpr int MB = RP / WR / 16;
  static constexpr int NB = RQ / WC / 16;
  static_assert(!GREG || NBUF >= 3, "register Gram on the split-step ring only");

  d4 acc[MB][NB];
  d4 gacc;
  int gi = -1, gj = -1;
  __amdgpu_buffer_rsrc_t rp, rq;
  int voff[PPW];
  int qkm;
  int tix = 0;
  int wo = 0;

  __device__ __forceinline__ int lane_ix() const { return OPQ ? tix : (int)(threadIdx.x & 63); }
  __device__ __forceinline__ void bind(const double* P, long ldp, const double* Q, long ldq, int kend) {
    if constexpr (OPQ) {
      tix = lane_id();
      asm volatile("" : "+v"(tix));
    }
    const int w = wave_id() - wo, l = lane_ix();
    rp = __builtin_amdgcn_make_buffer_rsrc(const_cast<double*>(P), 0, (int)(RP * ldp * 8), 0x00020000);
    rq = __builtin_amdgcn_make_buffer_rsrc(const_cast<double*>(Q), 0, QBLK ? (int)((long)kend * ldq * 8) : (int)(RQ * ldq * 8),
                                           0x00020000);
    qkm = QBLK ? (int)ldq * 8 : 8;
#pragma unroll
    for (int i = 0; i < PPW; ++i) {
      const int piece = w + NW * i;
      const bool isq = i >= PPW_P;
      const int row = (isq ? piece - RP / 8 : piece) * 8 + (l >> 3);
      const int slot = (l & 7) ^ ((row >> 1) & 7);
      voff[i] = (int)((long)row * (isq ? (QBLK ? 16 : ldq) : ldp) * 8 + slot * 16);
    }
  }

  __device__ __forceinline__ void zero() {
#pragma unroll
    for (int i = 0; i < MB; ++i)
#pragma unroll
      for (int j = 0; j < NB; ++j) acc[i][j] = (d4){0.0, 0.0, 0.0, 0.0};
    gacc = (d4){0.0, 0.0, 0.0, 0.0};
  }

  __device__ __forceinline__ void issue(uint32_t buf, int k0) const {
#pragma unroll
    for (int i = 0; i < PPW; ++i) issue_piece(buf, k0, i);
  }
  __device__ __forceinline__ void issue_piece(uint32_t buf, int k0, int i) const {
    const int w = wave_id() - wo;
    const uint32_t dst = buf + (uint32_t)(w + NW * i) * 1024u;
    if (i >= PPW_P)
      lds_dma16(rq, dst, voff[i], k0 * qkm);
    else
      lds_dma16(rp, dst, voff[i], k0 * 8);
  }

  __device__ __forceinline__ static uint32_t off(int row, int slot) {
    return (uint32_t)(row * 128 + ((slot ^ ((row >> 1) & 7)) << 4));
  }

  struct Frag {
    d2 a[MB], b[NB];
  };
  __device__ __forceinline__ void load_frag(const char* __restrict__ st, int kk, Frag& f) const {
    const int w = wave_id() - wo, l = lane_ix();
    const int wr = w / WC, wc = w % WC;
    const int fr = l & 15, g = l >> 4;
    const char* sp = st + (wr * (RP / WR) + fr) * 128;
    const char* sq = st + RP * 128 + (wc * (RQ / WC) + fr) * 128;
    const int so = ((4 * kk + g) ^ (fr >> 1)) << 4;
#pragma unroll
    for (int i = 0; i < MB; ++i) f.a[i] = *reinterpret_cast<const d2*>(sp + i * 16 * 128 + so);
#pragma unroll
    for (int j = 0; j < NB; ++j) f.b[j] = *reinterpret_cast<const d2*>(sq + j * 16 * 128 + so);
  }
  static constexpr int GC_DYN = -2;
  template <int GC = GC_DYN>
  __device__ __forceinline__ void mfma_frag(const Frag& f) {
    if constexpr (GT_PRIO) __builtin_amdgcn_s_setprio(1);
    mfma_frag_body<GC>(f);
    if constexpr (GT_PRIO) __builtin_amdgcn_s_setprio(0);
  }
  template <int GC = GC_DYN>
  __device__ __forceinline__ void mfma_frag_body(const Frag& f) {
#pragma unroll
    for (int i = 0; i < MB; ++i)
#pragma unroll
      for (int j = 0; j < NB; ++j) acc[i][j] = __builtin_amdgcn_mfma_f64_16x16x4f64(f.a[i].x, f.b[j].x, acc[i][j], 0, 0, 0);
#pragma unroll
    for (int i = 0; i < MB; ++i)
#pragma unroll
      for (int j = 0; j < NB; ++j) acc[i][j] = __builtin_amdgcn_mfma_f64_16x16x4f64(f.a[i].y, f.b[j].y, acc[i][j], 0, 0, 0);
// ... 14 lines not shown
    }
  }
  template <int NKK = 2>
  __device__ __forceinline__ void compute(const char* __restrict__ st) {
    const int w = wave_id() - wo, l = threadIdx.x & 63;
    const int wr = w / WC, wc = w % WC;
    const int fr = l & 15, g = l >> 4;
    const char* sp = st + (wr * (RP / WR) + fr) * 128;
    const char* sq = st + RP * 128 + (wc * (RQ / WC) + fr) * 128;
#pragma unroll
    for (int kk = 0; kk < NKK; ++kk) {
      const int so = ((4 * kk + g) ^ (fr >> 1)) << 4;
      d2 a[MB], b[NB];
#pragma unroll
      for (int i = 0; i < MB; ++i) a[i] = *reinterpret_cast<const d2*>(sp + i * 16 * 128 + so);
#pragma unroll
      for (int j = 0; j < NB; ++j) b[j] = *reinterpret_cast<const d2*>(sq + j * 16 * 128 + so);
#pragma unroll
      for (int i = 0; i < MB; ++i)
#pragma unroll
        for (int j = 0; j < NB; ++j) acc[i][j] = __builtin_amdgcn_mfma_f64_16x16x4f64(a[i].x, b[j].x, acc[i][j], 0, 0, 0);
#pragma unroll
      for (int i = 0; i < MB; ++i)
#pragma unroll
        for (int j = 0; j < NB; ++j) acc[i][j] = __builtin_amdgcn_mfma_f64_16x16x4f64(a[i].y, b[j].y, acc[i][j], 0, 0, 0);
    }
  }

  template <class Extra>
  __device__ __forceinline__ void run(const double* __restrict__ P, long ldp, const double* __restrict__ Q, long ldq,
                                      int kbeg, int kend, char* __restrict__ smem, Extra extra) {
    run(P, ldp, Q, ldq, kbeg, kend, smem, extra, [] {});
  }

  template <int XL = 0, class Extra, class AtLast>
  __device__ __forceinline__ void run(const double* __restrict__ P, long ldp, const double* __restrict__ Q, long ldq,
                                      int kbeg, int kend, char* __restrict__ smem, Extra extra, AtLast at_last) {
    (void)run<XL>(P, ldp, Q, ldq, kbeg, kend, smem, [] { return true; }, extra, at_last);
  }

  template <int XL = 0, int LASTKK = 2, int GC = GC_DYN, class Pre, class Extra, class AtLast>
  __device__ __forceinline__ bool run(const double* __restrict__ P, long ldp, const double* __restrict__ Q, long ldq,
                                      int kbeg, int kend, char* __restrict__ smem, Pre pre, Extra extra, AtLast at_last) {
    static_assert(LASTKK == 2 || NBUF == 2, "half last stage on the two-stage ring only");
    const int nst = (kend - kbeg) / BK2;
    bind(P, ldp, Q, ldq, kend);
    const uint32_t base = (uint32_t)(uintptr_t)smem;
    if constexpr (NBUF == 2) {
      issue(base, kbeg);
      if (!pre()) {
        wait_vmcnt<0>();
        return false;
      }
      wait_vmcnt<0>();
      step_barrier();
      if (nst == 1) at_last();
      for (int s = 0; s + 1 < nst; ++s) {
        const int b = s & 1;
        issue(base + (b ^ 1) * STAGE_BYTES, kbeg + (s + 1) * BK2);
        if (s + 2 == nst) at_last();
        const char* cur = smem + b * STAGE_BYTES;
        compute(cur);
        extra(cur);
        if (s + 2 == nst)
          wait_vmcnt<XL>();
        else
          wait_vmcnt<0>();
        step_barrier();
      }
      {
        const char* cur = smem + ((nst - 1) & 1) * STAGE_BYTES;
        compute<LASTKK>(cur);
        extra(cur);
      }
      return true;
    }
    constexpr int D = NBUF - 1;
    static_assert(PPW * (D - 1) + XL <= 63, "vmcnt holds at most 63 outstanding operations");
    const int npro = nst < D ? nst : D;
    bool xl = false;
    for (int q = 0; q < npro; ++q) issue(base + q * STAGE_BYTES, kbeg + q * BK2);
    if (!pre()) {
      wait_vmcnt<0>();
      return false;
    }
    if (nst <= D) {
      at_last();
      xl = true;
    }
    wait_stages<D - 1, XL>(npro - 1, xl);
    step_barrier();
    int b = 0;
    if constexpr (!SPLIT) {
      for (int s = 0; s < nst; ++s) {
        const char* cur = smem + b * STAGE_BYTES;
        if (s + D < nst) {
          const int bd = (b + D >= NBUF) ? b + D - NBUF : b + D;
          issue(base + bd * STAGE_BYTES, kbeg + (s + D) * BK2);
          if (s + D + 1 == nst) {
            at_last();
            xl = true;
          }
        }
        Frag f;
        load_frag(cur, 0, f);
        mfma_frag<GC>(f);
        load_frag(cur, 1, f);
        mfma_frag<GC>(f);
        extra(cur);
        if (s + 1 < nst) {
          const int left = nst - s - 2;
          wait_stages<D - 1, XL>(left < D - 1 ? left : D - 1, xl);
          step_barrier();
        }
        b = (b + 1 == NBUF) ? 0 : b + 1;
      }
      return true;
    }
    Frag f0, f1;
    load_frag(smem, 0, f0);
    for (int s = 0; s + 1 < nst; ++s) {
      const char* cur = smem + b * STAGE_BYTES;
      if (s + D < nst) {
        const int bd = (b + D >= NBUF) ? b + D - NBUF : b + D;
        issue(base + bd * STAGE_BYTES, kbeg + (s + D) * BK2);
        if (s + D + 1 == nst) {
          at_last();
          xl = true;
        }
      }
      load_frag(cur, 1, f1);
      mfma_frag<GC>(f0);
      extra(cur);
      const int bn = (b + 1 == NBUF) ? 0 : b + 1;
      const int left = nst - s - 2;
      __builtin_amdgcn_sched_barrier(0);
      wait_stages<D - 1, XL>(left < D - 1 ? left : D - 1, xl);
      step_barrier();
      load_frag(smem + bn * STAGE_BYTES, 0, f0);
      __builtin_amdgcn_sched_barrier(0);
      mfma_frag<GC>(f1);
      b = bn;
    }
    {
      const char* cur = smem + b * STAGE_BYTES;
      load_frag(cur, 1, f1);
      mfma_frag<GC>(f0);
      extra(cur);
      mfma_frag<GC>(f1);
    }
    return true;
  }

  template <int J, int XL>
  __device__ __forceinline__ static void wait_stages(int j, bool xl) {
    if (j >= J) {
      if (xl)
        wait_vmcnt<PPW * J + XL>();
      else
        wait_vmcnt<PPW * J>();
    } else if constexpr (J > 0) {
      wait_stages<J - 1, XL>(j, xl);
    }
  }

  __device__ __forceinline__ static int row_of(int mb, int reg) {
    const int w = wave_id(), l = lane_id();
    return (w / WC) * (RP / WR) + mb * 16 + (l >> 4) + 4 * reg;
  }
  __device__ __forceinline__ static int col_of(int nb) {
    const int w = wave_id(), l = lane_id();
    return (w % WC) * (RQ / WC) + nb * 16 + (l & 15);
  }
};

struct RestartInfo {
  int col0;
  int k;
  int rid;
  int sq_off;
};

struct ColInfo {
  int sq_off;
  int lc0;
  int k;
  int rid;
};

__device__ __forceinline__ bool panel_live(const int* __restrict__ prb, const int* __restrict__ pre, int p,
                                           const RestartInfo* __restrict__ ri, const int* __restrict__ stop_iter,
                                           int iter) {
  const int b = prb[p], e = pre[p];
  for (int q = b; q < e; ++q) {
    const int s = stop_iter[ri[q].rid];
    if (s == 0 || s == iter) return true;
  }
  return false;
}

template <int NPT>
__device__ __forceinline__ void gram_cand(int cand, int& q, int& br, int& bc) {
  if (cand < 4 * NPT) {
    q = cand >> 2;
    br = bc = cand & 3;
  } else {
    const int s = cand - 4 * NPT;
    q = s / 3;
    br = s % 3;
    bc = br + 1;
  }
}

template <int NPT, int RQ, int WR, int WC, int GPW, int NBUF = GT_NBUF, int MINW = 1, bool ABLK = false, bool GRAM = true,
          bool GITEM = false, bool GREG = false, bool SPLIT = true>
static __global__ __launch_bounds__(WR * WC * 64, MINW) void k_wta2(const double* __restrict__ W, const double* __restrict__ Acm,
                                                              long m_pad, int ngroups, int ntj, int nsplit, int kchunk,
                                                              const int* __restrict__ prb, const int* __restrict__ pre,
                                                              const RestartInfo* __restrict__ ri,
                                                              const ColInfo* __restrict__ ci,
                                                              const int* __restrict__ stop_iter, double* __restrict__ Gpart,
                                                              long g_ld, long g_split, double* __restrict__ SWpart,
                                                              long sw_total) {
  using T = GTile<64 * NPT, RQ, WR, WC, NBUF, ABLK, GREG, SPLIT>;
  static_assert(!GREG || (WR == NPT && GPW == 1 && GRAM && !GITEM), "register Gram: one panel per wave row");
  constexpr int NCAND = 7 * NPT;
  __shared__ __attribute__((aligned(1024))) char smem[T::LDS_BYTES + 64];
  int* need = reinterpret_cast<int*>(smem + T::LDS_BYTES);
  constexpr int NGW = GITEM ? 3 : 0;
  const int ntt = ntj + NGW;
  const int nitems = nsplit * ngroups * ntt;
  const int item = xcd_item(blockIdx.x, nitems);
  const int t = item % ntt;
  const int pg = (item / ntt) % ngroups;
  const int s = item / (ntt * ngroups);
  if constexpr (GITEM) {
    static_assert(NPT == 1 && T::NW >= 3, "Gram items: 1-panel tiles of at least 3 waves");
    using TG = GTile<16, 16, 1, 1, NBUF, false>;
    static_assert(3 * TG::LDS_BYTES <= T::LDS_BYTES, "three Gram rings fit the tile's");
    if (t >= ntj) {
      const int w = wave_id(), l = threadIdx.x & 63, fr = l & 15, g = l >> 4;
      const int x = 3 * (t - ntj) + w;
      if (w >= 3 || x >= 7) return;
      if (!panel_live(prb, pre, pg, ri, stop_iter, 0)) return;
      const int br = x < 4 ? x : x - 4, bc = x < 4 ? x : x - 3;
      const ColInfo* cp = ci + (long)pg * PANEL;
      if (br != bc) {
        const ColInfo c = cp[16 * bc];
        if (!(c.k > 0 && c.lc0 < 16 * bc)) return;
      }
      const int kbeg = s * kchunk;
      const int kend = (int)min((long)kbeg + kchunk, m_pad);
      TG tg;
      tg.wo = w;
      tg.zero();
      const double* Pr = W + ((long)pg * PANEL + 16 * br) * m_pad + kbeg;
      const double* Qr = W + ((long)pg * PANEL + 16 * bc) * m_pad + kbeg;
      tg.run(Pr, m_pad, Qr, m_pad, 0, kend - kbeg, smem + w * TG::LDS_BYTES, [](const char*) {});
      double* so = SWpart + (long)s * sw_total;
#pragma unroll
      for (int reg = 0; reg < 4; ++reg) {
        const int lr = 16 * br + g + 4 * reg, lcn = 16 * bc + fr;
        const ColInfo cr = cp[lr];
        if (cr.k == 0 || cr.lc0 != cp[lcn].lc0 || cp[lcn].k == 0) continue;
        const int a = lr - cr.lc0, b = lcn - cr.lc0;
        so[cr.sq_off + a * cr.k + b] = tg.acc[0][0][reg];
        so[cr.sq_off + b * cr.k + a] = tg.acc[0][0][reg];
      }
      return;
    }
  }
  bool live[NPT];
  bool any = false;
#pragma unroll
  for (int q = 0; q < NPT; ++q) {
    live[q] = panel_live(prb, pre, NPT * pg + q, ri, stop_iter, 0);
    any = any || live[q];
  }
  if (!any) return;
  if (threadIdx.x < NCAND) {
    int q, br, bc;
    gram_cand<NPT>(threadIdx.x, q, br, bc);
    int nd = live[q];
    if (nd && br != bc) {
      const ColInfo c = ci[(long)(NPT * pg + q) * PANEL + 16 * bc];
      nd = (c.k > 0 && c.lc0 < 16 * bc);
    }
    need[threadIdx.x] = nd;
  }
  const int kbeg = s * kchunk;
  const int kend = (int)min((long)kbeg + kchunk, m_pad);
  const long ldq = ABLK ? (long)ntj * RQ : m_pad;
  const double* Q = ABLK ? Acm + (long)kbeg * ldq + (long)t * RQ * 16 : Acm + (long)t * RQ * m_pad + kbeg;
  T tl;
  tl.zero();
  d4 gacc[GPW];
#pragma unroll
  for (int x = 0; x < GPW; ++x) gacc[x] = (d4){0.0, 0.0, 0.0, 0.0};
  const int w = wave_id(), l = threadIdx.x & 63;
  const int fr = l & 15, g = l >> 4;
  __syncthreads();
  int my_need[GPW], my_ra[GPW], my_rb[GPW];
  bool gram = false;
#pragma unroll
  for (int x = 0; x < GPW; ++x) {
    const int cand = t + ntj * (w + T::NW * x);
    my_need[x] = 0;
    my_ra[x] = 0;
    my_rb[x] = 0;
    if (cand < NCAND) {
      int q, br, bc;
      gram_cand<NPT>(cand, q, br, bc);
      my_need[x] = (GREG && (cand < 4 * NPT || WC == 4)) ? 0 : need[cand];
      my_ra[x] = 64 * q + 16 * br;
      my_rb[x] = 64 * q + 16 * bc;
      gram = GRAM && !GITEM && (gram || my_need[x]);
    }
  }
  if constexpr (GREG) {
    const int wr = w / WC, wc = w % WC;
    int gi = -1, gj = -1;
    if constexpr (WC == 4) {
      int kth = 0;
#pragma unroll
      for (int c = 0; c < 7; ++c) {
        const int cand = c < 4 ? 4 * wr + c : 4 * NPT + 3 * wr + (c - 4);
        if (cand % ntj != t) continue;
        if (wc == ((t + wr + 2 * kth) & 3) && need[cand]) {
          gi = c < 4 ? c : c - 4;
          gj = c < 4 ? c : c - 3;
        }
        ++kth;
      }
    } else if (wc == ((wr >> 1) & 1) % WC) {
#pragma unroll
      for (int br = 0; br < 4; ++br)
        if ((4 * wr + br) % ntj == t && need[4 * wr + br]) gi = gj = br;
    }
    tl.gi = __builtin_amdgcn_readfirstlane(gi);
    tl.gj = __builtin_amdgcn_readfirstlane(gj);
  }
  const double* P = W + (long)pg * 64 * NPT * m_pad + kbeg;
  auto lds_gram = [&](const char* stg) {
#pragma unroll
    for (int x = 0; x < GPW; ++x) {
      if (!my_need[x]) continue;
      const char* pa = stg + (my_ra[x] + fr) * 128;
      const char* pb = stg + (my_rb[x] + fr) * 128;
#pragma unroll
      for (int kk = 0; kk < 2; ++kk) {
        const int so = ((4 * kk + g) ^ (fr >> 1)) << 4;
        const d2 a = *reinterpret_cast<const d2*>(pa + so);
        const d2 b = *reinterpret_cast<const d2*>(pb + so);
        gacc[x] = __builtin_amdgcn_mfma_f64_16x16x4f64(a.x, b.x, gacc[x], 0, 0, 0);
        gacc[x] = __builtin_amdgcn_mfma_f64_16x16x4f64(a.y, b.y, gacc[x], 0, 0, 0);
      }
    }
  };
  constexpr bool LDSG = GRAM && !GITEM && !(GREG && WC == 4);
  if constexpr (GREG && WC == 4) {
    auto go = [&](auto gc) {
      tl.template run<0, 2, decltype(gc)::value>(P, m_pad, Q, ldq, 0, kend - kbeg, smem, [] { return true; },
                                                 [](const char*) {}, [] {});
    };
    switch (tl.gi < 0 ? -1 : 4 * tl.gi + tl.gj) {
      case 0: go(std::integral_constant<int, 0>{}); break;
      case 5: go(std::integral_constant<int, 5>{}); break;
      case 10: go(std::integral_constant<int, 10>{}); break;
      case 15: go(std::integral_constant<int, 15>{}); break;
      case 1: go(std::integral_constant<int, 1>{}); break;
      case 6: go(std::integral_constant<int, 6>{}); break;
      case 11: go(std::integral_constant<int, 11>{}); break;
      default: go(std::integral_constant<int, -1>{}); break;
    }
  } else if (LDSG && gram) {
    tl.run(P, m_pad, Q, ldq, 0, kend - kbeg, smem, lds_gram);
  } else {
    tl.run(P, m_pad, Q, ldq, 0, kend - kbeg, smem, [](const char*) {});
  }
  double* out = Gpart + (long)s * g_split + (long)pg * 64 * NPT * g_ld + (long)t * RQ;
#pragma unroll
  for (int mb = 0; mb < T::MB; ++mb)
#pragma unroll
    for (int nb = 0; nb < T::NB; ++nb)
#pragma unroll
      for (int reg = 0; reg < 4; ++reg) out[(long)T::row_of(mb, reg) * g_ld + T::col_of(nb)] = tl.acc[mb][nb][reg];
  auto put_gram = [&](int ra, int rb, const d4& v) {
    double* so = SWpart + (long)s * sw_total;
    const int pnl = ra >> 6;
    const ColInfo* cp = ci + (long)(NPT * pg + pnl) * PANEL;
    const int ln = lane_id();
#pragma unroll
    for (int reg = 0; reg < 4; ++reg) {
      const int lr = (ra & 63) + (ln >> 4) + 4 * reg;
      const int lcn = (rb & 63) + (ln & 15);
      const ColInfo cr = cp[lr];
      if (cr.k == 0 || cr.lc0 != cp[lcn].lc0 || cp[lcn].k == 0) continue;
      const int a = lr - cr.lc0, b = lcn - cr.lc0;
      so[cr.sq_off + a * cr.k + b] = v[reg];
      so[cr.sq_off + b * cr.k + a] = v[reg];
    }
  };
  if (gram) {
#pragma unroll
    for (int x = 0; x < GPW; ++x)
      if (my_need[x]) put_gram(my_ra[x], my_rb[x], gacc[x]);
  }
  if constexpr (GREG) {
    if (tl.gi >= 0) put_gram(64 * (w / WC) + 16 * tl.gi, 64 * (w / WC) + 16 * tl.gj, tl.gacc);
  }
}

constexpr int SK_THREADS = 1024;
constexpr long SK_FIX = 9L * 4 * SK_THREADS;
constexpr int SK_POLLS = 256;

__device__ __forceinline__ int uni(int v) { return __builtin_amdgcn_readfirstlane(v); }
__device__ __forceinline__ long uni(long v) {
  const unsigned long long u = (unsigned long long)v;
  return (long)(((unsigned long long)(unsigned)__builtin_amdgcn_readfirstlane((int)(u >> 32)) << 32) |
                (unsigned)__builtin_amdgcn_readfirstlane((int)(u & 0xffffffffu)));
}
template <class P>
__device__ __forceinline__ P* uni(P* p) {
  return reinterpret_cast<P*>(uni(reinterpret_cast<long>(p)));
}
template <class V>
__device__ __forceinline__ V opaque(V v) {
  asm volatile("" : "+s"(v));
  return v;
}

struct SkArgs {
  const double* W;
  const double* Acm;
  long m_pad;
  int ngroups, ntj, kchunk;
  const int* prb;
  const int* pre;
  const RestartInfo* ri;
  const ColInfo* ci;
  const int* stop_iter;
  double* Gpart;
  long g_ld, g_split;
  double* SWpart;
  long sw_total;
  double* fix;
  unsigned* flags;
  unsigned epoch;
  int nsplit;
  unsigned* tcnt;
  int dp_xcd;
};
typedef const SkArgs __attribute__((address_space(4)))* SkArgsK;

__device__ __forceinline__ SkArgsK sk_args() {
  unsigned long long u = (unsigned long long)__builtin_amdgcn_kernarg_segment_ptr();
  asm volatile("" : "+s"(u));
  return (SkArgsK)u;
}

template <int NBUF, bool NOWAIT, bool LSUM = false, int NPT = 4>
__device__ __forceinline__ void wta_sk_piece(int r, int item_in, int s0_in, int s1_in, int mode_in,
                                             char* __restrict__ smem) {
  constexpr int RQ = 128, WC = 4;
  using T = GTile<64 * NPT, RQ, NPT, WC, NBUF, true, true, true, true>;
  static_assert(T::MB * T::NB == 8 && T::NTH <= SK_THREADS, "a slot holds 8 accumulator blocks + the Gram chain per lane");
  SkArgsK A = sk_args();
  const double* W = A->W;
  const double* Acm = A->Acm;
  const long m_pad = A->m_pad;
  const int ngroups = A->ngroups, ntj = A->ntj, kchunk = A->kchunk;
  const int* prb = A->prb;
  const int* pre = A->pre;
  const RestartInfo* ri = A->ri;
  const ColInfo* ci = A->ci;
  const int* stop_iter = A->stop_iter;
  r = uni(r);
  const int item = uni(item_in), s0 = uni(s0_in), s1 = uni(s1_in), mode = uni(mode_in);
  const unsigned epoch = A->epoch;
  auto lane = [] {
    int v = lane_id();
    asm volatile("" : "+v"(v));
    return v;
  };
  int* need = reinterpret_cast<int*>(smem + T::LDS_BYTES);
  int* okw = need + 7 * NPT;
  const int w = wave_id();
  const int t = uni(item % ntj);
  const int pg = uni((item / ntj) % ngroups);
  const int s = uni(item / (ngroups * ntj));
  bool live[NPT];
  bool any = false;
#pragma unroll
  for (int q = 0; q < NPT; ++q) {
    live[q] = panel_live(prb, pre, NPT * pg + q, ri, stop_iter, 0);
    any = any || live[q];
  }
  if (!any) return;
  const int tid = 64 * w + lane();
  if (tid < 7 * NPT) {
    int q, br, bc;
    gram_cand<NPT>(tid, q, br, bc);
    int nd = live[q];
    if (nd && br != bc) {
      const ColInfo c = ci[(long)(NPT * pg + q) * PANEL + 16 * bc];
      nd = (c.k > 0 && c.lc0 < 16 * bc);
    }
    need[tid] = nd;
  }
  unsigned* flags = A->flags;
  double* fix = A->fix;
  if (mode == 2 && tid == 0) {
    int ok = 0;
    for (int i = 0; i < (NOWAIT ? 0 : SK_POLLS); ++i) {
      if (__hip_atomic_load(flags + (r - 1), __ATOMIC_RELAXED, __HIP_MEMORY_SCOPE_AGENT) == epoch) {
        ok = 1;
        break;
      }
      __builtin_amdgcn_s_sleep(127);
    }
    __builtin_amdgcn_fence(__ATOMIC_ACQUIRE, "agent");
    asm volatile("s_waitcnt vmcnt(0)" ::: "memory");
    *okw = ok;
  }
  const int kbeg = s * kchunk;
  const long ldq = (long)ntj * RQ;
  const double* Q = Acm + (long)kbeg * ldq + (long)t * RQ * 16;
  T tl;
  tl.zero();
  __syncthreads();
  const bool cont = mode == 2 && uni(*okw) != 0;
  const int resume = uni(cont ? s0 : (mode == 2 ? 0 : s0));
  auto load_chains = [&] {
    if (cont) {
      const double* src = fix + (long)(r - 1) * SK_FIX + 4L * (64 * w);
      const int ln = lane();
#pragma unroll
      for (int mb = 0; mb < T::MB; ++mb)
#pragma unroll
        for (int nb = 0; nb < T::NB; ++nb)
          tl.acc[mb][nb] = *reinterpret_cast<const d4*>(src + ((long)(mb * T::NB + nb) * SK_THREADS + ln) * 4);
      tl.gacc = *reinterpret_cast<const d4*>(src + ((long)T::MB * T::NB * SK_THREADS + ln) * 4);
    }
    return true;
  };
  {
    const int wr = w / WC, wc = w % WC;
    int gi = -1, gj = -1, kth = 0;
#pragma unroll
    for (int c = 0; c < 7; ++c) {
      const int cand = c < 4 ? 4 * wr + c : 4 * NPT + 3 * wr + (c - 4);
      if (cand % ntj != t) continue;
      if (wc == ((t + wr + 2 * kth) & 3) && need[cand]) {
        gi = c < 4 ? c : c - 4;
        gj = c < 4 ? c : c - 3;
      }
      ++kth;
    }
    tl.gi = __builtin_amdgcn_readfirstlane(gi);
    tl.gj = __builtin_amdgcn_readfirstlane(gj);
  }
  const double* P = W + (long)pg * 64 * NPT * m_pad + kbeg;
  auto go = [&](auto gc) {
    tl.template run<0, 2, decltype(gc)::value>(P, m_pad, Q, ldq, BK2 * resume, BK2 * s1, smem, load_chains,
                                               [](const char*) {}, [] {});
  };
  switch (tl.gi < 0 ? -1 : 4 * tl.gi + tl.gj) {
    case 0: go(std::integral_constant<int, 0>{}); break;
    case 5: go(std::integral_constant<int, 5>{}); break;
    case 10: go(std::integral_constant<int, 10>{}); break;
    case 15: go(std::integral_constant<int, 15>{}); break;
    case 1: go(std::integral_constant<int, 1>{}); break;
    case 6: go(std::integral_constant<int, 6>{}); break;
    case 11: go(std::integral_constant<int, 11>{}); break;
    default: go(std::integral_constant<int, -1>{}); break;
  }
  if (mode == 1) {
    A = sk_args();
    fix = A->fix;
    flags = A->flags;
    double* dst = fix + (long)r * SK_FIX + 4L * (64 * w);
    const int ln = lane();
#pragma unroll
    for (int mb = 0; mb < T::MB; ++mb)
#pragma unroll
      for (int nb = 0; nb < T::NB; ++nb)
        *reinterpret_cast<d4*>(dst + ((long)(mb * T::NB + nb) * SK_THREADS + ln) * 4) = tl.acc[mb][nb];
    *reinterpret_cast<d4*>(dst + ((long)T::MB * T::NB * SK_THREADS + ln) * 4) = tl.gacc;
    asm volatile("s_waitcnt vmcnt(0)" ::: "memory");
    __syncthreads();
    if (w == 0 && ln == 0) {
      __builtin_amdgcn_fence(__ATOMIC_RELEASE, "agent");
      asm volatile("s_waitcnt vmcnt(0)" ::: "memory");
      __hip_atomic_store(flags + r, A->epoch, __ATOMIC_RELAXED, __HIP_MEMORY_SCOPE_AGENT);
    }
    return;
  }
  A = sk_args();
  const long g_ld = A->g_ld, g_split = A->g_split;
  double* out = A->Gpart + (long)s * g_split + (long)pg * 64 * NPT * g_ld + (long)t * RQ;
  {
    const int ln = lane();
    const int r0 = (w / WC) * 64 + (ln >> 4), c0 = (w % WC) * (RQ / WC) + (ln & 15);
#pragma unroll
    for (int mb = 0; mb < T::MB; ++mb)
#pragma unroll
      for (int nb = 0; nb < T::NB; ++nb)
#pragma unroll
        for (int reg = 0; reg < 4; ++reg) out[(long)(r0 + mb * 16 + 4 * reg) * g_ld + c0 + nb * 16] = tl.acc[mb][nb][reg];
  }
  if (tl.gi >= 0) {
    const int ra = 64 * (w / WC) + 16 * tl.gi, rb = 64 * (w / WC) + 16 * tl.gj;
    double* so = A->SWpart + (long)s * A->sw_total;
    const ColInfo* cp = ci + (long)(NPT * pg + (ra >> 6)) * PANEL;
    const int ln = lane();
#pragma unroll
    for (int reg = 0; reg < 4; ++reg) {
      const int lr = (ra & 63) + (ln >> 4) + 4 * reg;
      const int lcn = (rb & 63) + (ln & 15);
      const ColInfo cr = cp[lr];
      if (cr.k == 0 || cr.lc0 != cp[lcn].lc0 || cp[lcn].k == 0) continue;
      const int a = lr - cr.lc0, bq = lcn - cr.lc0;
      so[cr.sq_off + a * cr.k + bq] = tl.gacc[reg];
      so[cr.sq_off + bq * cr.k + a] = tl.gacc[reg];
    }
  }
  if constexpr (LSUM) {
    A = sk_args();
    const int nsplit = A->nsplit;
    if (nsplit > 1) {
      asm volatile("s_waitcnt vmcnt(0)" ::: "memory");
      __syncthreads();
      const int ntj2 = A->ntj, ng2 = A->ngroups;
      const int tile = item % (ng2 * ntj2), pg2 = (item / ntj2) % ng2, t2 = item % ntj2;
      if (w == 0 && lane() == 0) {
        __builtin_amdgcn_fence(__ATOMIC_RELEASE, "agent");
        asm volatile("s_waitcnt vmcnt(0)" ::: "memory");
        const unsigned old = __hip_atomic_fetch_add(A->tcnt + tile, 1u, __ATOMIC_RELAXED, __HIP_MEMORY_SCOPE_AGENT);
        const int last = (old + 1) % (unsigned)nsplit == 0;
        if (last) {
          __builtin_amdgcn_fence(__ATOMIC_ACQUIRE, "agent");
          asm volatile("s_waitcnt vmcnt(0)" ::: "memory");
        }
        *okw = last;
      }
      __syncthreads();
      if (uni(*okw)) {
        const long g_ld2 = A->g_ld, g_split2 = A->g_split;
        double* base = A->Gpart + (long)pg2 * 64 * NPT * g_ld2 + (long)t2 * RQ;
        const int ln = lane();
        const int r0 = (w / WC) * 64 + (ln >> 4), c0 = (w % WC) * (RQ / WC) + (ln & 15);
#pragma unroll
        for (int mb = 0; mb < T::MB; ++mb)
#pragma unroll
          for (int nb = 0; nb < T::NB; ++nb) {
            double v[4];
            double* e0 = base + (long)(r0 + mb * 16) * g_ld2 + c0 + nb * 16;
#pragma unroll
            for (int reg = 0; reg < 4; ++reg) v[reg] = e0[(long)4 * reg * g_ld2];
            for (int c = 1; c < nsplit; ++c) {
              double u[4];
#pragma unroll
              for (int reg = 0; reg < 4; ++reg) u[reg] = e0[(long)c * g_split2 + (long)4 * reg * g_ld2];
#pragma unroll
              for (int reg = 0; reg < 4; ++reg) v[reg] = v[reg] + u[reg];
            }
#pragma unroll
            for (int reg = 0; reg < 4; ++reg) e0[(long)4 * reg * g_ld2] = v[reg];
          }
      }
    }
  }
}

template <int NBUF = GT_NBUF, bool NOWAIT = false, bool LSUM = false, int NPT = 4>
static __global__ __launch_bounds__(64 * NPT * 4, 1) void k_wta2_sk(SkArgs args) {
  using T = GTile<64 * NPT, 128, NPT, 4, NBUF, true, true, true, true>;
  static_assert(NPT == 4 || NPT == 2, "the 16-wave 4-panel tile or the 8-wave 2-panel tile");
  __shared__ __attribute__((aligned(1024))) char smem[T::LDS_BYTES + 128];
  (void)args;
  SkArgsK A = sk_args();
  const int nsplit = A->nsplit;
  const int G = gridDim.x;
  const int r = __builtin_amdgcn_readfirstlane(xcd_item(blockIdx.x, G));
  const int xq = G >> 3, xrem = G & 7, xcd = blockIdx.x & 7;
  const int xc = xq + (xcd < xrem ? 1 : 0), xb = xcd < xrem ? xcd * (xq + 1) : xrem * (xq + 1) + (xcd - xrem) * xq;
  const int ipc = A->ngroups * A->ntj;
  const int nitems = nsplit * ipc;
  const int nst_full = A->kchunk / BK2;
  const int nst_last = (int)((A->m_pad - (long)(nsplit - 1) * A->kchunk) / BK2);
  const int nst_max = nsplit > 1 ? nst_full : nst_last;
  const int c_last = ipc * (nsplit - 1);
  auto nst_of = [&](int item) { return item >= c_last ? nst_last : nst_full; };
  auto off = [&](int item) -> long {
    return item <= c_last ? (long)item * nst_full : (long)c_last * nst_full + (long)(item - c_last) * nst_last;
  };
  auto locate = [&](long x, int& item, int& st) {
    const long lc = (long)c_last * nst_full;
    const int it = x < lc ? (int)(x / nst_full) : c_last + (int)((x - lc) / nst_last);
    item = __builtin_amdgcn_readfirstlane(it);
    st = __builtin_amdgcn_readfirstlane((int)(x - off(it)));
  };
  int D = (nitems / G - 1) * G;
  if (D < 0) D = 0;
  while (D > 0 && off(nitems) - off(D) < (long)G * nst_max) D -= G;
  D = __builtin_amdgcn_readfirstlane(D);
  const long base = off(D), S = off(nitems) - base;
  const long b = base + S * r / G, e = base + S * (r + 1) / G;
  int ib, sb, ie, se;
  locate(b, ib, sb);
  locate(e - 1, ie, se);
  ++se;
  const bool head = sb > 0;
  const bool tail = se < nst_of(ie);
  const int f0 = head ? ib + 1 : ib, f1 = tail ? ie - 1 : ie;
  const int nfull = f1 >= f0 ? f1 - f0 + 1 : 0;
  const int ndp = D / G;
  const int t0 = tail ? 1 : 0;
  const int npieces = t0 + ndp + nfull + (head ? 1 : 0);
  for (int pc = 0; pc < npieces; ++pc) {
    int item, s0, s1, mode;
    if (pc < ndp) {
      item = A->dp_xcd ? ndp * xb + pc * xc + (r - xb) : pc * G + r;
      s0 = 0, s1 = nst_of(item), mode = 0;
    } else if (pc < ndp + t0) {
      item = ie, s0 = 0, s1 = se, mode = 1;
    } else if (head && pc == npieces - 1) {
      item = ib, s0 = sb, s1 = nst_of(ib), mode = 2;
    } else {
      item = f0 + pc - t0 - ndp, s0 = 0, s1 = nst_of(item), mode = 0;
    }
    __syncthreads();
    wta_sk_piece<NBUF, NOWAIT, LSUM, NPT>(r, item, s0, s1, mode, smem);
  }
}

template <int RQ, int NBUF, bool ABLK = false>
static __global__ __launch_bounds__(64) void k_wta_narrow(const double* __restrict__ W, const double* __restrict__ Acm,
                                                          long m_pad, int ntq, int nsplit, int kchunk, int nblk,
                                                          const ColInfo* __restrict__ ci, double* __restrict__ Gpart,
                                                          long g_ld, long g_split, double* __restrict__ SWpart,
                                                          long sw_total) {
  using T = GTile<16, RQ, 1, 1, NBUF, ABLK>;
  using TG = GTile<16, 16, 1, 1, NBUF, false>;
  static_assert(TG::LDS_BYTES <= T::LDS_BYTES, "the Gram item's ring fits the tile's");
  __shared__ __attribute__((aligned(1024))) char smem[T::LDS_BYTES];
  const int nt = ntq + 1;
  const int item = xcd_item(blockIdx.x, nsplit * nblk * nt);
  const int t = item % nt, bk = (item / nt) % nblk, s = item / (nt * nblk);
  const int kbeg = s * kchunk;
  const int kend = (int)min((long)kbeg + kchunk, m_pad);
  const int l = threadIdx.x, fr = l & 15, g = l >> 4;
  const double* Wb = W + (long)bk * 16 * m_pad + kbeg;
  if (t == ntq) {
    TG tg;
    tg.zero();
    tg.run(Wb, m_pad, Wb, m_pad, 0, kend - kbeg, smem, [](const char*) {});
    double* so = SWpart + (long)s * sw_total;
    const ColInfo* cb = ci + (long)bk * 16;
#pragma unroll
    for (int reg = 0; reg < 4; ++reg) {
      const int lr = g + 4 * reg, lcn = fr;
      const ColInfo cr = cb[lr];
      if (cr.k == 0 || cr.lc0 != cb[lcn].lc0 || cb[lcn].k == 0) continue;
      const int a = lr - (cr.lc0 & 15), b = lcn - (cr.lc0 & 15);
      so[cr.sq_off + a * cr.k + b] = tg.acc[0][0][reg];
      so[cr.sq_off + b * cr.k + a] = tg.acc[0][0][reg];
    }
    return;
  }
  T tl;
  tl.zero();
  const long ldq = ABLK ? (long)ntq * RQ : m_pad;
  const double* Q = ABLK ? Acm + (long)kbeg * ldq + (long)t * RQ * 16 : Acm + (long)t * RQ * m_pad + kbeg;
  tl.run(Wb, m_pad, Q, ldq, 0, kend - kbeg, smem, [](const char*) {});
  double* out = Gpart + (long)s * g_split + (long)bk * 16 * g_ld + (long)t * RQ;
#pragma unroll
  for (int nb = 0; nb < T::NB; ++nb)
#pragma unroll
    for (int reg = 0; reg < 4; ++reg) out[(long)T::row_of(0, reg) * g_ld + T::col_of(nb)] = tl.acc[0][nb][reg];
}

template <int RQ, int NBUF, bool ABLK = false>
static __global__ __launch_bounds__(128) void k_wta_narrow_lc(const double* __restrict__ W, const double* __restrict__ Acm,
                                                             long m_pad, int ntq, int nsplit, int kchunk, int nblk,
                                                             const ColInfo* __restrict__ ci, double* __restrict__ Gpart,
                                                             long g_ld, long g_split, double* __restrict__ SWpart,
                                                             long sw_total) {
  static_assert(RQ == 16, "the Gram item shares the tile type: RQ = 16");
  using T = GTile<16, RQ, 1, 1, NBUF, ABLK>;
  __shared__ __attribute__((aligned(1024))) char smem[T::LDS_BYTES];
  const int nt = ntq + 1;
  const int item = xcd_item(blockIdx.x, nsplit * nblk * nt);
  const int t = item % nt, bk = (item / nt) % nblk, s = item / (nt * nblk);
  const int kbeg = s * kchunk;
  const int kend = (int)min((long)kbeg + kchunk, m_pad);
  const int wave = wave_id(), l = threadIdx.x & 63, fr = l & 15, g = l >> 4;
  const bool gram = t == ntq;
  const double* Wb = W + (long)bk * 16 * m_pad + kbeg;
  const long ldq = gram ? m_pad : (ABLK ? (long)ntq * RQ : m_pad);
  const double* Q = gram ? Wb : (ABLK ? Acm + (long)kbeg * ldq + (long)t * RQ * 16 : Acm + (long)t * RQ * m_pad + kbeg);
  const int nst = (kend - kbeg) / BK2;
  constexpr int D = NBUF - 1;
  const uint32_t base = (uint32_t)(uintptr_t)smem;
  T tl;
  tl.wo = wave;
  if (wave == 1) {
    if (gram) {
      GTile<16, RQ, 1, 1, NBUF, false> tg;
      tg.wo = 1;
      tg.bind(Wb, m_pad, Q, ldq, kend - kbeg);
      const int npro = nst < D ? nst : D;
      for (int q = 0; q < npro; ++q) tg.issue(base + q * T::STAGE_BYTES, q * BK2);
      T::template wait_stages<D - 1, 0>(npro - 1, false);
      step_barrier();
      for (int st = 0; st + 1 < nst; ++st) {
        if (st + D < nst) tg.issue(base + ((st + D) % NBUF) * T::STAGE_BYTES, (st + D) * BK2);
        const int left = nst - st - 2;
        T::template wait_stages<D - 1, 0>(left < D - 1 ? left : D - 1, false);
        step_barrier();
      }
    } else {
      tl.bind(Wb, m_pad, Q, ldq, kend - kbeg);
      const int npro = nst < D ? nst : D;
      for (int q = 0; q < npro; ++q) tl.issue(base + q * T::STAGE_BYTES, q * BK2);
      T::template wait_stages<D - 1, 0>(npro - 1, false);
      step_barrier();
      for (int st = 0; st + 1 < nst; ++st) {
        if (st + D < nst) tl.issue(base + ((st + D) % NBUF) * T::STAGE_BYTES, (st + D) * BK2);
        const int left = nst - st - 2;
        T::template wait_stages<D - 1, 0>(left < D - 1 ? left : D - 1, false);
        step_barrier();
      }
    }
    return;
  }
  tl.zero();
  step_barrier();
  typename T::Frag f0, f1;
  int b = 0;
  tl.load_frag(smem, 0, f0);
  for (int st = 0; st + 1 < nst; ++st) {
    const char* cur = smem + b * T::STAGE_BYTES;
    tl.load_frag(cur, 1, f1);
    tl.mfma_frag(f0);
    const int bn = (b + 1 == NBUF) ? 0 : b + 1;
    __builtin_amdgcn_sched_barrier(0);
    step_barrier();
    tl.load_frag(smem + bn * T::STAGE_BYTES, 0, f0);
    __builtin_amdgcn_sched_barrier(0);
    tl.mfma_frag(f1);
    b = bn;
  }
  {
    const char* cur = smem + b * T::STAGE_BYTES;
    tl.load_frag(cur, 1, f1);
    tl.mfma_frag(f0);
    tl.mfma_frag(f1);
  }
  if (gram) {
    double* so = SWpart + (long)s * sw_total;
    const ColInfo* cb = ci + (long)bk * 16;
#pragma unroll
    for (int reg = 0; reg < 4; ++reg) {
      const int lr = g + 4 * reg, lcn = fr;
      const ColInfo cr = cb[lr];
      if (cr.k == 0 || cr.lc0 != cb[lcn].lc0 || cb[lcn].k == 0) continue;
      const int a = lr - (cr.lc0 & 15), bb = lcn - (cr.lc0 & 15);
      so[cr.sq_off + a * cr.k + bb] = tl.acc[0][0][reg];
      so[cr.sq_off + bb * cr.k + a] = tl.acc[0][0][reg];
    }
    return;
  }
  double* out = Gpart + (long)s * g_split + (long)bk * 16 * g_ld + (long)t * RQ;
#pragma unroll
  for (int nb = 0; nb < T::NB; ++nb)
#pragma unroll
    for (int reg = 0; reg < 4; ++reg) out[(long)T::row_of(0, reg) * g_ld + T::col_of(nb)] = tl.acc[0][nb][reg];
}

constexpr int NTH = 512;
constexpr int HCH2 = NTH;

struct HupdSmem {
// ... 252 lines not shown
template <int GTG = GT, int NBUF = GT_NBUF, int NPT = 1, int PR = PANEL, int WC = 4, bool LATE = false, bool KHALF = false>
static __global__ __launch_bounds__(64 * NPT * WC,
                                    (163840 / ahtw4_lds<GTG, NBUF, NPT, PR, WC, LATE>()) * NPT * WC / 4 > 8
                                        ? 8
                                        : (163840 / ahtw4_lds<GTG, NBUF, NPT, PR, WC, LATE>()) * NPT * WC / 4)
void k_ahtw4(int iter, const double* __restrict__ H, long n_pad, const double* __restrict__ Arm, long m_pad,
             double* __restrict__ W, const double* __restrict__ SHP, const ColInfo* __restrict__ ci,
             const int* __restrict__ colact, int npanels, int ngt) {
  using TileW4 = GTile<PR * NPT, GTG, NPT, WC, NBUF>;
  constexpr int AHTW4_SH = TileW4::LDS_BYTES;
  constexpr int AHTW4_LDS = ahtw4_lds<GTG, NBUF, NPT, PR, WC, LATE>();
  static_assert(AHTW4_LDS <= 163840, "LDS of one CU");
  static_assert(PR == PANEL || (PR == 16 && NPT == 1), "narrow tiles: one 16-column block");
  static_assert(!LATE || TileW4::STAGE_BYTES >= NPT * PR * KMAX * 8, "h h^T rows fit one ring stage");
  constexpr int NTH = 64 * NPT * WC;
  __shared__ __attribute__((aligned(1024))) char smem[AHTW4_LDS];
  double* SHl = reinterpret_cast<double*>(smem + AHTW4_SH);
  int pp, gt;
  ahtw_map(xcd_item(blockIdx.x, (npanels / NPT) * ngt), npanels / NPT, ngt, pp, gt);
  const int p0 = pp * NPT;
  const int tid = threadIdx.x, lane = tid & 63, w = wave_id(), wr = w / WC, wc = w % WC;
  const int p = p0 + wr;
  ColInfo cc;
  uint64_t actmask = 0;
  TileW4 tl;
  tl.zero();
  const __amdgpu_buffer_rsrc_t rw = __builtin_amdgcn_make_buffer_rsrc(
      W + (long)p * PR * m_pad + (long)gt * GTG + (GTG / WC) * wc, 0, (int)(PR * m_pad * 8), 0x00020000);
  const int wvoff = (int)(((lane >> 4) * m_pad + (lane & 15)) * 8);
  auto woff = [&](int mb, int reg, int nb) { return (int)(((16 * mb + 4 * reg) * m_pad + 16 * nb) * 8); };
  double w0[TileW4::MB][TileW4::NB][4];
  auto load_w0_block = [&](int mb) {
#pragma unroll
    for (int reg = 0; reg < 4; ++reg)
#pragma unroll
      for (int nb = 0; nb < TileW4::NB; ++nb)
        w0[mb][nb][reg] = __builtin_bit_cast(double, __builtin_amdgcn_raw_buffer_load_b64(rw, wvoff, woff(mb, reg, nb), 0));
  };
  auto load_w0 = [&] {
#pragma unroll
    for (int mb = 0; mb < TileW4::MB; ++mb) load_w0_block(mb);
  };
  constexpr int NSH = NPT * PR * KMAX / 2 / NTH;
  static_assert(NSH * 2 * NTH == NPT * PR * KMAX, "h h^T rows split evenly over the threads");
  d2 shv[NSH];
  constexpr bool EARLY = LATE && NBUF == 2 && TileW4::MB >= 2;
  constexpr int XL = LATE ? (EARLY ? 2 * TileW4::NB * 4 : 0) : TileW4::MB * TileW4::NB * 4;
  const bool live = tl.template run<XL, KHALF ? 1 : 2>(
      H + (long)p0 * PR * n_pad, n_pad, Arm + (long)gt * GTG * n_pad, n_pad, 0, (int)n_pad, smem,
      [&] {
        cc = lane < PR ? ci[(long)p * PR + lane] : ColInfo{0, 0, 0, 0};
        int ca[NPT];
#pragma unroll
        for (int q = 0; q < NPT; ++q) ca[q] = lane < PR ? colact[(long)(p0 + q) * PR + lane] : -1;
        const d2* src = reinterpret_cast<const d2*>(SHP + (long)p0 * PR * KMAX);
#pragma unroll
        for (int j = 0; j < NSH; ++j) shv[j] = src[tid + NTH * j];
        bool any = false;
#pragma unroll
        for (int q = 0; q < NPT; ++q) {
          const uint64_t mk = __ballot(ca[q] == iter);
          if (q == wr) actmask = mk;
          any = any || mk != 0;
        }
        if (!any) return false;
        if constexpr (!LATE) {
#pragma unroll
          for (int j = 0; j < NSH; ++j) reinterpret_cast<d2*>(SHl)[tid + NTH * j] = shv[j];
        }
        return true;
      },
      [](const char*) {},
      [&] {
        if constexpr (!LATE) load_w0();
        if constexpr (EARLY) {
          load_w0_block(0);
          load_w0_block(1);
        }
      });
  if (!live) return;
  if constexpr (LATE) {
    const int nst = (int)n_pad / BK2;
    SHl = reinterpret_cast<double*>(smem + ((nst - 2) % NBUF) * TileW4::STAGE_BYTES);
#pragma unroll
    for (int j = 0; j < NSH; ++j) reinterpret_cast<d2*>(SHl)[tid + NTH * j] = shv[j];
    if constexpr (!EARLY) {
#pragma unroll
      for (int mb = 0; mb < (TileW4::MB < 2 ? TileW4::MB : 2); ++mb) load_w0_block(mb);
    }
  }
  const bool cross = ((actmask >> lane) & 1) && ((cc.lc0 & (PR - 1)) >> 4) != (((cc.lc0 & (PR - 1)) + cc.k - 1) >> 4);
  const bool aligned = __ballot(cross) == 0;
  if constexpr (LATE) __syncthreads();
  if (actmask == 0) return;
  const double* SHw = SHl + (long)wr * PR * KMAX;
#pragma unroll
  for (int mb = 0; mb < TileW4::MB; ++mb) {
    if constexpr (LATE) {
      if (mb + 2 < TileW4::MB) load_w0_block(mb + 2);
    }
    const int ra = 16 * mb + (lane & 15);
    const int alc = __shfl(cc.lc0, ra) & (PR - 1);
    const int ak = ((actmask >> ra) & 1) ? __shfl(cc.k, ra) : 0;
    d4 e[TileW4::NB];
#pragma unroll
    for (int nb = 0; nb < TileW4::NB; ++nb) e[nb] = d4{0.0, 0.0, 0.0, 0.0};
    if (aligned) {
      double av[4];
#pragma unroll
      for (int q = 0; q < 4; ++q) {
        const int bb = 16 * mb + 4 * q + (lane >> 4) - alc;
        av[q] = (bb >= 0 && bb < ak) ? SHw[ra * KMAX + bb] : 0.0;
      }
#pragma unroll
      for (int q = 0; q < 4; ++q)
#pragma unroll
        for (int nb = 0; nb < TileW4::NB; ++nb)
          e[nb] = __builtin_amdgcn_mfma_f64_16x16x4f64(av[q], w0[mb][nb][q], e[nb], 0, 0, 0);
    } else {
      int lo = ak ? alc : PANEL, hi = ak ? alc + ak : 0;
#pragma unroll
      for (int off = 8; off >= 1; off >>= 1) {
        lo = min(lo, __shfl_xor(lo, off));
        hi = max(hi, __shfl_xor(hi, off));
      }
      lo = __builtin_amdgcn_readfirstlane(lo);
      hi = __builtin_amdgcn_readfirstlane(hi);
#pragma unroll
      for (int q = (4 * mb - 4 > 0 ? 4 * mb - 4 : 0); q < (4 * mb + 8 < 4 * TileW4::MB ? 4 * mb + 8 : 4 * TileW4::MB); ++q) {
        if (4 * q + 3 < lo || 4 * q >= hi) continue;
        const int bb = 4 * q + (lane >> 4) - alc;
        const double av = (bb >= 0 && bb < ak) ? SHw[ra * KMAX + bb] : 0.0;
#pragma unroll
        for (int nb = 0; nb < TileW4::NB; ++nb)
          e[nb] = __builtin_amdgcn_mfma_f64_16x16x4f64(av, w0[q >> 2][nb][q & 3], e[nb], 0, 0, 0);
      }
    }
#pragma unroll
    for (int reg = 0; reg < 4; ++reg) {
      const int c = 16 * mb + (lane >> 4) + 4 * reg;
      if (!((actmask >> c) & 1)) continue;
#pragma unroll
      for (int nb = 0; nb < TileW4::NB; ++nb) {
        const double v = mu_rule_sel(w0[mb][nb][reg], tl.acc[mb][nb][reg], e[nb][reg]);
        __builtin_amdgcn_raw_buffer_store_b64(__builtin_bit_cast(u32x2, v), rw, wvoff, woff(mb, reg, nb), 0);
      }
    }
  }
}

constexpr int SMALL_PF = NMFC_SMALL_PF;
constexpr int SMALL_FPF = NMFC_SMALL_FPF;
constexpr int SMALL_NW = 4;
constexpr int SMALL_MAXR = 8;
constexpr int SMALL_GGMAX = 4;

struct SmallBlock {
  int col0;
  int nr;
  int rid[SMALL_MAXR];
  int k[SMALL_MAXR];
  int lc0[SMALL_MAXR];
};

struct SoloJob {
  int col0, k, rid, pad;
};

template <int JB, int NW = SMALL_NW>
struct SmallSmem {
  double H[2][16][16 * JB];
  union {
    double Gp[NW][16][16 * JB];
    double T[NW][SMALL_GGMAX][16][17];
  } u;
  double SWp[NW][16][16];
  double SW[16][16];
  double S[16][16];
  double win[SMALL_MAXR][16][16];
  int cls[SMALL_MAXR][64];
  int colr[16];
  int run[SMALL_MAXR];
  int unch[SMALL_MAXR];
  int changed[SMALL_MAXR];
  int nrun;
};

template <int GBW, int JB, int SKIP = 0, int NW = SMALL_NW>
static __global__ __launch_bounds__(64 * NW) void k_small_mu(
    const SmallBlock* __restrict__ blocks, const double* __restrict__ Arm, long ld_rm, const double* __restrict__ Acm,
    long m_pad, int n, long n_pad, double* __restrict__ W, double* __restrict__ H, int maxiter, int stop_rule,
    int* __restrict__ stop_iter, int* __restrict__ stop_reason) {
  constexpr int NP = 16 * JB;
  constexpr int PF = NW == 8 ? SMALL_PF / 2 : SMALL_PF, FPF = SMALL_FPF;
  __shared__ SmallSmem<JB, NW> sm;
  __shared__ SmallBlock blk;
  if (threadIdx.x == 0) blk = blocks[blockIdx.x];
  __syncthreads();
  const int tid = threadIdx.x, l = tid & 63, w = tid >> 6, lr = l >> 4, lc = l & 15;
  const int nr = blk.nr;
  if (tid < 16) sm.colr[tid] = -1;
  __syncthreads();
  if (tid < nr)
    for (int a = 0; a < blk.k[tid]; ++a) sm.colr[blk.lc0[tid] + a] = tid;
  if (tid < SMALL_MAXR) {
    sm.run[tid] = tid < nr;
    sm.unch[tid] = 0;
  }
  for (int x = tid; x < SMALL_MAXR * 64; x += 64 * NW) (&sm.cls[0][0])[x] = 0;
  for (int x = tid; x < 16 * NP; x += 64 * NW) {
    const int c = x / NP, j = x % NP;
    sm.H[0][c][j] = (j < n) ? H[(long)(blk.col0 + c) * n_pad + j] : 0.0;
  }
  double wr[GBW][4];
#pragma unroll
  for (int gb = 0; gb < GBW; ++gb)
#pragma unroll
    for (int r = 0; r < 4; ++r)
      wr[gb][r] = W[(long)(blk.col0 + lc) * m_pad + 16 * (w * GBW + gb) + 4 * r + lr];
  if (tid == 0) sm.nrun = nr;
  __syncthreads();
  int hb = 0;
  for (int iter = 1; iter <= maxiter; ++iter) {
    long zo = 0;
    asm volatile("" : "+s"(zo));
    const double* __restrict__ ArmI = Arm + zo;
    const double* __restrict__ AcmI = Acm + zo;
    d4 gacc[JB], sacc = (d4){0.0, 0.0, 0.0, 0.0};
#pragma unroll
    for (int jb = 0; jb < JB; ++jb) gacc[jb] = (d4){0.0, 0.0, 0.0, 0.0};
    {
      constexpr int NKS = (SKIP & 1) ? 0 : 4 * GBW;
      double pf[PF][JB];
      constexpr long LDR = (JB <= 2) ? 32 : 64;
      const double* __restrict__ arow = ArmI + (long)(16 * w * GBW + lr) * LDR + lc;
#pragma unroll
      for (int t = 0; t < PF; ++t)
        if (t < NKS) {
#pragma unroll
          for (int jb = 0; jb < JB; ++jb) pf[t][jb] = arow[(long)(4 * t) * LDR + 16 * jb];
        }
#pragma unroll
      for (int t = 0; t < NKS; ++t) {
        const int gb = t >> 2, r = t & 3;
        double av[JB];
#pragma unroll
        for (int jb = 0; jb < JB; ++jb) av[jb] = pf[t % PF][jb];
        if (t + PF < NKS) {
#pragma unroll
          for (int jb = 0; jb < JB; ++jb) pf[t % PF][jb] = arow[(long)(4 * (t + PF)) * LDR + 16 * jb];
        }
#pragma unroll
        for (int jb = 0; jb < JB; ++jb) gacc[jb] = __builtin_amdgcn_mfma_f64_16x16x4f64(wr[gb][r], av[jb], gacc[jb], 0, 0, 0);
        sacc = __builtin_amdgcn_mfma_f64_16x16x4f64(wr[gb][r], wr[gb][r], sacc, 0, 0, 0);
        __builtin_amdgcn_sched_barrier(0);
      }
    }
#pragma unroll
    for (int r = 0; r < 4; ++r) {
#pragma unroll
      for (int jb = 0; jb < JB; ++jb) sm.u.Gp[w][lr + 4 * r][16 * jb + lc] = gacc[jb][r];
      sm.SWp[w][lr + 4 * r][lc] = sacc[r];
    }
    __syncthreads();
    if (tid < 256) {
      const int c = tid >> 4, d = tid & 15;
      double sw = sm.SWp[0][c][d];
#pragma unroll
      for (int v = 1; v < NW; ++v) sw += sm.SWp[v][c][d];
      sm.SW[c][d] = sw;
      if (tid < SMALL_MAXR) sm.changed[tid] = 0;
    }
    __syncthreads();
    int runmask = 0;
#pragma unroll
    for (int q = 0; q < SMALL_MAXR; ++q) runmask |= (q < nr && sm.run[q]) ? (1 << q) : 0;
    {
      const double(*Ho)[NP] = sm.H[hb];
      double(*Hn)[NP] = sm.H[hb ^ 1];
#pragma unroll
      for (int u = 0; u < (16 * NP + 64 * NW - 1) / (64 * NW); ++u) {
        const int x = tid + u * 64 * NW;
        if (x < 16 * NP) {
          const int c = x / NP, j = x % NP;
          const int q = sm.colr[c];
          const double h0 = Ho[c][j];
          double hv = h0;
          if (!(SKIP & 2) && q >= 0 && ((runmask >> q) & 1) && j < n) {
            double gsum = sm.u.Gp[0][c][j];
#pragma unroll
            for (int v = 1; v < NW; ++v) gsum += sm.u.Gp[v][c][j];
            const int b0 = blk.lc0[q], kq = blk.k[q];
            double dsum = 0.0;
            for (int b = 0; b < kq; ++b) dsum = fma(sm.SW[c][b0 + b], Ho[b0 + b][j], dsum);
            hv = mu_rule(h0, gsum, dsum);
          }
          Hn[c][j] = hv;
        }
      }
    }
    hb ^= 1;
    __syncthreads();
    const double(*Hc)[NP] = sm.H[hb];
    const bool check = !(SKIP & 4) && stop_rule != STOP_FIXED && iter > 1 && (iter % 2 == 0);
    if (w == 0 && !(SKIP & 4)) {
      d4 hh = (d4){0.0, 0.0, 0.0, 0.0};
#pragma unroll
      for (int q = 0; q < NP / 4; ++q) {
        const double hv = Hc[lc][4 * q + lr];
        hh = __builtin_amdgcn_mfma_f64_16x16x4f64(hv, hv, hh, 0, 0, 0);
      }
#pragma unroll
      for (int r = 0; r < 4; ++r) {
        const int c = lr + 4 * r, d = lc;
        const int qc = sm.colr[c];
        sm.S[c][d] = (qc >= 0 && qc == sm.colr[d]) ? hh[r] : 0.0;
// ... 971 lines not shown
```

Before: 498.7.

## Tighten restart packing and skip empty panels in stream-K WTA splits

```diff
diff --git a/nmfconsensus_amd/build.py b/nmfconsensus_amd/build.py
--- a/nmfconsensus_amd/build.py
+++ b/nmfconsensus_amd/build.py
@@ -9,7 +9,7 @@
 CSRC = os.path.join(HERE, "csrc")
 LIB = os.path.join(HERE, "lib", "libnmf.so")
 SOURCES = ["engine.hip", "compat.hip", "brunet.hip", "generic.hip", "solo.hip", "hclust.cpp"]
-HEADERS = ["nmfc_kernels.hpp", "nmfc_tuning.hpp", "nmfc_internal.hpp", "lane_pool.hpp", "rmt.hpp", "../../include/nmfc.h", "../../include/libnmf_compat.h"]
+HEADERS = ["nmfc_kernels.hpp", "nmfc_tuning.hpp", "nmfc_internal.hpp", "lane_pool.hpp", "packing.hpp", "sk_split.hpp", "rmt.hpp", "../../include/nmfc.h", "../../include/libnmf_compat.h"]
 ARCH = os.environ.get("NMFC_OFFLOAD_ARCH", "gfx950")
 HIPCC = os.environ.get("HIPCC", "/opt/rocm/bin/hipcc")
 
diff --git a/nmfconsensus_amd/csrc/engine.hip b/nmfconsensus_amd/csrc/engine.hip
--- a/nmfconsensus_amd/csrc/engine.hip
+++ b/nmfconsensus_amd/csrc/engine.hip
@@ -16,6 +16,7 @@
 #include "nmfc_kernels.hpp"
 
 using namespace nmfc;
+using namespace nmfc_host;
 
 namespace {
 
@@ -106,7 +107,6 @@
 
 enum { KID_WTA = 0, KID_HUPD = 1, KID_AHTW = 2, KID_INIT = 3, KID_OTHER = 4, KID_LABELS = 5, KID_COUNTS = 6, KID_SMALL = 7, KID_RESID = 8, KID_N = 9 };
 
-constexpr int WTA_NPT = 4;
 constexpr int NARROW_NBUF = NMFC_NARROW_NBUF;
 constexpr bool WTA_MID_GREG = NMFC_WTA_MID_GREG != 0;
 constexpr bool SMALL_NW8 = NMFC_SMALL_NW8 != 0;
@@ -116,104 +116,6 @@
 constexpr int WTA_MID_MINW = NMFC_WTA_MID_MINW;
 constexpr int AHTW_NBUF = NMFC_AHTW_NBUF;
 constexpr bool AHTW_LATE = NMFC_AHTW_LATE != 0;
-struct Packing {
-  std::vector<RestartInfo> ri;
-  std::vector<int> prb, pre;
-  std::vector<ColInfo> ci;
-  int npanels = 0;
-};
-
-Packing pack(const std::vector<RestartInfo>& in) {
-  std::vector<RestartInfo> srt(in);
-  std::stable_sort(srt.begin(), srt.end(), [](const RestartInfo& a, const RestartInfo& b) {
-    return a.k != b.k ? a.k > b.k : a.rid < b.rid;
-  });
-  std::vector<int> fill;
-  std::vector<std::vector<RestartInfo>> members;
-  size_t first_open = 0;
-  for (RestartInfo r : srt) {
-    size_t b = first_open;
-    while (b < fill.size() && fill[b] + r.k > 16) ++b;
-    if (b == fill.size()) {
-      fill.push_back(0);
-      members.emplace_back();
-    }
-    r.col0 = (int)b * 16 + fill[b];
-    fill[b] += r.k;
-    members[b].push_back(r);
-    while (first_open < fill.size() && fill[first_open] > 14) ++first_open;
-  }
-  const int nblocks = (int)members.size();
-  Packing pk;
-  pk.npanels = std::max(1, (nblocks + 3) / 4);
-  for (int p = 0; p < pk.npanels; ++p) {
-    pk.prb.push_back((int)pk.ri.size());
-    for (int b = 4 * p; b < std::min(nblocks, 4 * p + 4); ++b)
-      for (const RestartInfo& r : members[b]) pk.ri.push_back(r);
-    pk.pre.push_back((int)pk.ri.size());
-  }
-  while (pk.npanels % WTA_NPT) {
-    pk.prb.push_back((int)in.size());
-    pk.pre.push_back((int)in.size());
-    ++pk.npanels;
-  }
-  pk.ci.assign((size_t)pk.npanels * PANEL, ColInfo{0, 0, 0, 0});
-  for (const RestartInfo& r : pk.ri)
-    for (int a = 0; a < r.k; ++a) pk.ci[r.col0 + a] = ColInfo{r.sq_off, r.col0 % PANEL, r.k, r.rid};
-  return pk;
-}
-
-int narrow_blocks(const Packing& pk, int maxb) {
-  if (pk.ri.empty()) return 0;
-  int nb = 0;
-  for (const RestartInfo& r : pk.ri) {
-    if (r.col0 / 16 != (r.col0 + r.k - 1) / 16) return 0;
-    nb = std::max(nb, (r.col0 + r.k + 15) / 16);
-  }
-  return nb <= maxb ? nb : 0;
-}
-
-Packing pack_small(const std::vector<RestartInfo>& in, std::vector<SmallBlock>& blocks) {
-  std::vector<RestartInfo> srt(in);
-  std::stable_sort(srt.begin(), srt.end(), [](const RestartInfo& a, const RestartInfo& b) {
-    return a.k != b.k ? a.k > b.k : a.rid < b.rid;
-  });
-  std::vector<int> fill;
-  blocks.clear();
-  Packing pk;
-  for (RestartInfo r : srt) {
-    size_t b = 0;
-    while (b < fill.size() && (fill[b] + r.k > 16 || blocks[b].nr == SMALL_MAXR)) ++b;
-    if (b == fill.size()) {
-      fill.push_back(0);
-      SmallBlock sb{};
-      sb.col0 = (int)b * 16;
-      blocks.push_back(sb);
-    }
-    SmallBlock& sb = blocks[b];
-    r.col0 = sb.col0 + fill[b];
-    sb.rid[sb.nr] = r.rid;
-    sb.k[sb.nr] = r.k;
-    sb.lc0[sb.nr] = fill[b];
-    ++sb.nr;
-    fill[b] += r.k;
-    pk.ri.push_back(r);
-  }
-  pk.npanels = std::max(1, (int)((blocks.size() * 16 + PANEL - 1) / PANEL));
-  while (pk.npanels % WTA_NPT) ++pk.npanels;
-  pk.prb.assign(pk.npanels, 0);
-  pk.pre.assign(pk.npanels, 0);
-  pk.ci.assign((size_t)pk.npanels * PANEL, ColInfo{0, 0, 0, 0});
-  return pk;
-}
-
-int live_panels(const Packing& pk) {
-  int np = 0;
-  for (int p = 0; p < pk.npanels; ++p)
-    if (pk.pre[p] > pk.prb[p]) np = p + 1;
-  return np;
-}
-
 std::vector<SoloJob> place_solo(Packing& pk, std::vector<RestartInfo> solo, int col_base, int n) {
   std::stable_sort(solo.begin(), solo.end(), [n](const RestartInfo& a, const RestartInfo& b) {
     const int ka = nmfc_solo_batch_rank(n, a.k), kb = nmfc_solo_batch_rank(n, b.k);
@@ -262,9 +164,16 @@
   bool narrow_lc = true;
   bool wta_sk = true;
   bool wta_sk_mid = true;
+  bool pack_tight = true;
+  bool wta_pskip = true;
+  bool sk_even = false;
   bool wta_lastsum = false;
   int sk_dp_xcd = 0;
   DevBuf skfix, skflag, sktcnt;
+  DevBuf sktab;
+  std::vector<int> sktab_host;
+  SkShape sktab_shape{0, 0, 0, 0, 0, 0, 0, 0};
+  int sktab_maxp = 0;
   unsigned sk_epoch = 0;
   bool gram_model = true;
   bool solo_ok = true;
@@ -297,6 +206,7 @@
     int small = 0, repacks_skipped = 0, polls = 0, iterations_enqueued = 0, panels_first = 0, panels_min = 0;
     long long wta_narrow = 0, wta_sk = 0, wta_big = 0, wta_mid = 0, wta_small = 0, wta_tiny = 0;
     long long ahtw_narrow = 0, ahtw_128 = 0, ahtw_64 = 0;
+    long long wta_block_iters = 0, ahtw_block_iters = 0;
   } info;
   std::string info_str;
   bool residuals = false, resid_valid = false;
@@ -316,18 +226,29 @@
 constexpr double WTA_SK_COST = 1.01;
 bool sk_big_ok(const nmfc_engine* e, int ntj) { return e->wta_sk && WTA_W16 && ntj >= 4; }
 bool sk_mid_ok(const nmfc_engine* e, int ntj) { return e->wta_sk && e->wta_sk_mid && WTA_MID_GREG && ntj >= 4; }
-bool sk_grid_fits(const nmfc_engine* e, long ngroups, int ntj) {
-  const long ipc = ngroups * ntj, nitems = ipc * e->nsplit;
-  const long nst_full = e->kchunk / 16, nst_last = (e->m_pad - (long)(e->nsplit - 1) * e->kchunk) / 16;
-  const long nst_max = e->nsplit > 1 ? nst_full : nst_last;
-  const long S = ipc * (e->nsplit - 1) * nst_full + ipc * nst_last;
-  return nitems >= e->ncu && S >= (long)e->ncu * nst_max;
-}
-int sk_groups(const nmfc_engine* e, int tile, int big_panels, int mid_panels, int ntj) {
+SkShape sk_shape(const nmfc_engine* e, int ngroups, int ntj, int npt, int last_w) {
+  SkShape h;
+  h.ng = ngroups, h.ntj = ntj, h.nsplit = e->nsplit;
+  h.nst_full = e->kchunk / 16;
+  h.nst_last = (int)((e->m_pad - (long)(e->nsplit - 1) * e->kchunk) / 16);
+  h.npt = npt, h.last_w = last_w, h.G = e->ncu;
+  return h;
+}
+bool sk_grid_fits(const nmfc_engine* e, int ngroups, int ntj, int npt, int last_w) {
+  return sk_fits(sk_shape(e, ngroups, ntj, npt, last_w));
+}
+struct SkGroups {
+  int ng, last_w, npt;
+};
+SkGroups sk_groups(const nmfc_engine* e, int tile, int big_panels, int mid_panels, int live, int ntj) {
   const bool big = tile == 0 && sk_big_ok(e, ntj), mid = tile == 3 && sk_mid_ok(e, ntj);
-  if (!big && !mid) return 0;
+  const int npt = big ? WTA_NPT : 2;
+  if (!big && !mid) return {0, npt, npt};
   const int ng = big ? (big_panels + WTA_NPT - 1) / WTA_NPT : (mid_panels + 1) / 2;
-  return sk_grid_fits(e, ng, ntj) ? ng : 0;
+  const int lw = live - npt * (ng - 1);
+  const bool lsum = big && e->wta_lastsum;
+  if (e->wta_pskip && !e->sk_even && !lsum && lw >= 1 && lw < npt && sk_grid_fits(e, ng, ntj, npt, lw)) return {ng, lw, npt};
+  return {sk_grid_fits(e, ng, ntj, npt, npt) ? ng : 0, npt, npt};
 }
 
 TileChoice choose_tiles(const nmfc_engine* e, int np_live, int ntj) {
@@ -345,8 +266,9 @@
   TileChoice tc{0, false};
   double best = 1e300;
   for (const Cand& c : cands) {
-    const bool sk = sk_groups(e, c.id, (int)np, (int)np, ntj) > 0;
-    const double est = sk ? c.wgs / (double)c.slots * c.t * WTA_SK_COST : std::ceil(c.wgs / (double)c.slots) * c.t;
+    const SkGroups sk = sk_groups(e, c.id, (int)np, (int)np, (int)np, ntj);
+    const double wgs = c.wgs - (double)(ns * ntj) * (sk.npt - sk.last_w) / sk.npt;
+    const double est = sk.ng ? wgs / (double)c.slots * c.t * WTA_SK_COST : std::ceil(c.wgs / (double)c.slots) * c.t;
     if (est < best - 1e-9) {
       best = est;
       tc.wta = c.id;
@@ -639,7 +561,7 @@
   std::vector<RestartInfo> blk_jobs, solo_jobs;
   for (const RestartInfo& r : s.all)
     (s.small && e->solo_ok && nmfc_mu_solo_fits(m, n, r.k) ? solo_jobs : blk_jobs).push_back(r);
-  s.pk = s.small ? pack_small(blk_jobs, s.sblocks) : pack(s.all);
+  s.pk = s.small ? pack_small(blk_jobs, s.sblocks) : pack(s.all, e->pack_tight);
   if (s.small && !solo_jobs.empty()) s.solo = place_solo(s.pk, solo_jobs, (int)s.sblocks.size() * 16, n);
   s.cap_cols = (long)s.pk.npanels * PANEL;
   e->info.small = s.small;
@@ -915,7 +837,7 @@
                      s.sw_total);
 }
 
-int launch_wta_sk(Sweep& s, bool big, int ng, int* gsplit) {
+int launch_wta_sk(Sweep& s, bool big, int ng, int last_w, int* gsplit) {
   nmfc_engine* e = s.e;
   hipStream_t st = e->st;
   if (!e->skflag.p) {
@@ -923,6 +845,19 @@
     HCHECK(hipMemsetAsync(e->skflag.p, 0, sizeof(unsigned) * e->ncu, st));
   }
   ++e->info.wta_sk;
+  const SkShape h = sk_shape(e, ng, s.ntj, big ? WTA_NPT : 2, last_w);
+  const SkShape& o = e->sktab_shape;
+  if (!e->sktab.p || o.ng != h.ng || o.ntj != h.ntj || o.nsplit != h.nsplit || o.nst_full != h.nst_full ||
+      o.nst_last != h.nst_last || o.npt != h.npt || o.last_w != h.last_w || o.G != h.G) {
+    HCHECK(hipStreamSynchronize(st));
+    const int maxp = sk_table(h, e->sk_dp_xcd, nullptr, 0);
+    e->sktab_host.assign((size_t)h.G * (4 + 4 * maxp), 0);
+    sk_table(h, e->sk_dp_xcd, e->sktab_host.data(), maxp);
+    if (e->sktab.ensure(sizeof(int) * e->sktab_host.size())) return -1;
+    HCHECK(hipMemcpyAsync(e->sktab.p, e->sktab_host.data(), sizeof(int) * e->sktab_host.size(), hipMemcpyHostToDevice, st));
+    e->sktab_shape = h;
+    e->sktab_maxp = maxp;
+  }
   const long tiles = (long)ng * s.ntj;
   const bool lastsum = e->wta_lastsum && big;
   if (lastsum && e->sktcnt.bytes < sizeof(unsigned) * tiles) {
@@ -933,7 +868,7 @@
                  e->prb.as<int>(), e->pre.as<int>(), e->rinfo.as<RestartInfo>(), e->colinfo.as<ColInfo>(),
                  e->stop_iter.as<int>(), e->Gpart.as<double>(), s.g_ld, s.g_split, e->SWpart.as<double>(), s.sw_total,
                  e->skfix.as<double>(), e->skflag.as<unsigned>(), ++e->sk_epoch, e->nsplit,
-                 e->sktcnt.as<unsigned>(), e->sk_dp_xcd};
+                 e->sktcnt.as<unsigned>(), e->sk_dp_xcd, e->wta_pskip ? 1 : 0, e->sktab.as<int>(), e->sktab_maxp};
   if (!big) {
     hipLaunchKernelGGL((k_wta2_sk<WTA_MID_NBUF, false, false, 2>), dim3(e->ncu), dim3(SK_THREADS / 2), 0, st, a);
   } else if (lastsum) {
@@ -983,7 +918,7 @@
                      e->W[s.cur].as<double>(), e->Ablk.as<double>(), e->m_pad, l.ngroups, l.tiles, e->nsplit, e->kchunk,
                      e->prb.as<int>(), e->pre.as<int>(), e->rinfo.as<RestartInfo>(), e->colinfo.as<ColInfo>(),
                      e->stop_iter.as<int>(), e->Gpart.as<double>(), s.g_ld, s.g_split, e->SWpart.as<double>(),
-                     s.sw_total);
+                     s.sw_total, e->wta_pskip ? 1 : 0);
 }
 
 struct ChunkPlan {
@@ -996,12 +931,21 @@
 };
 
 int launch_wta(Sweep& s, const ChunkPlan& cp, int* gsplit) {
+  nmfc_engine* e = s.e;
+  const bool lsum = e->wta_lastsum && cp.tc.wta == 0;
+  auto count = [&](int npt, int ngroups) {
+    e->info.wta_block_iters += 4LL * (e->wta_pskip && !lsum && npt > 1 ? cp.live : npt * ngroups);
+  };
   if (cp.nblk > 0) {
+    e->info.wta_block_iters += cp.nblk;
     launch_wta_narrow(s, cp.nblk);
-  } else if (const int ng = sk_groups(s.e, cp.tc.wta, s.pk.npanels, cp.lp, s.ntj)) {
-    return launch_wta_sk(s, cp.tc.wta == 0, ng, gsplit);
+  } else if (const SkGroups sk = sk_groups(e, cp.tc.wta, s.pk.npanels, cp.lp, cp.live, s.ntj); sk.ng) {
+    count(sk.npt, sk.ng);
+    return launch_wta_sk(s, cp.tc.wta == 0, sk.ng, sk.last_w, gsplit);
   } else {
-    launch_wta2(s, pick_wta2(s.e, cp.tc.wta, s.ntj, cp.live, s.pk.npanels));
+    const Wta2Launch l = pick_wta2(e, cp.tc.wta, s.ntj, cp.live, s.pk.npanels);
+    count(l.tile == 0 ? WTA_NPT : l.tile == 3 ? 2 : 1, l.ngroups);
+    launch_wta2(s, l);
   }
   return 0;
 }
@@ -1019,6 +963,7 @@
 void launch_ahtw(const Sweep& s, const ChunkPlan& cp, int iter) {
   nmfc_engine* e = s.e;
   ++(cp.nblk > 0 ? e->info.ahtw_narrow : cp.tc.ahtw_small ? e->info.ahtw_64 : e->info.ahtw_128);
+  e->info.ahtw_block_iters += cp.nblk > 0 ? cp.nblk : 4LL * cp.lp;
   if (cp.nblk > 0)
     hipLaunchKernelGGL((k_ahtw4<GT / 4, GT_NBUF, 1, 16, 2>), dim3(4 * e->ngt * cp.nblk), dim3(128), 0, e->st,
                        iter, e->H[s.cur].as<double>(), e->n_pad, e->Arm.as<double>(), e->m_pad,
@@ -1123,7 +1068,7 @@
       gone.push_back(r);
   }
   if (archive(s, gone)) return -1;
-  Packing np = pack(live);
+  Packing np = pack(live, e->pack_tight);
   if ((long)np.npanels * PANEL > s.cap_cols) {
     s.stopped_at_pack = stopped;
     ++e->info.repacks_skipped;
@@ -1397,12 +1342,15 @@
     e->force_wta = v == "big" ? 0 : v == "small" ? 1 : v == "tiny" ? 2 : v == "mid" ? 3 : -1;
   }
   if (const char* s = getenv("NMFC_REPACK_DIV")) e->repack_div = std::max(1, atoi(s));
+  if (const char* s = getenv("NMFC_PACK")) e->pack_tight = strcmp(s, "ffd") != 0;
   if (const char* s = getenv("NMFC_NARROW")) e->narrow_ok = atoi(s) != 0;
   if (const char* s = getenv("NMFC_NARROW_MAXB")) e->narrow_maxb = std::min(8, std::max(1, atoi(s)));
   if (const char* s = getenv("NMFC_SMALL")) e->small_ok = atoi(s) != 0;
   if (const char* s = getenv("NMFC_SOLO")) e->solo_ok = atoi(s) != 0;
   if (const char* s = getenv("NMFC_NARROW_LC")) e->narrow_lc = atoi(s) != 0;
   if (const char* s = getenv("NMFC_WTA_SK")) e->wta_sk = atoi(s) != 0;
+  if (const char* s = getenv("NMFC_WTA_PSKIP")) e->wta_pskip = atoi(s) != 0;
+  if (const char* s = getenv("NMFC_SK_EVEN")) e->sk_even = atoi(s) != 0;
   if (const char* s = getenv("NMFC_WTA_SK_MID")) e->wta_sk_mid = atoi(s) != 0;
   if (const char* s = getenv("NMFC_WTA_LASTSUM")) e->wta_lastsum = atoi(s) != 0;
   if (const char* s = getenv("NMFC_SK_DP_XCD")) e->sk_dp_xcd = atoi(s) != 0;
@@ -1580,9 +1528,10 @@
   snprintf(buf, sizeof buf,
            "small=%d;repacks=%d;repacks_skipped=%d;polls=%d;iterations_enqueued=%d;panels_first=%d;panels_min=%d;"
            "wta_narrow=%lld;wta_sk=%lld;wta_big=%lld;wta_mid=%lld;wta_small=%lld;wta_tiny=%lld;"
-           "ahtw_narrow=%lld;ahtw_128=%lld;ahtw_64=%lld",
+           "ahtw_narrow=%lld;ahtw_128=%lld;ahtw_64=%lld;wta_block_iters=%lld;ahtw_block_iters=%lld",
            i.small, e->repacks, i.repacks_skipped, i.polls, i.iterations_enqueued, i.panels_first, i.panels_min,
-           i.wta_narrow, i.wta_sk, i.wta_big, i.wta_mid, i.wta_small, i.wta_tiny, i.ahtw_narrow, i.ahtw_128, i.ahtw_64);
+           i.wta_narrow, i.wta_sk, i.wta_big, i.wta_mid, i.wta_small, i.wta_tiny, i.ahtw_narrow, i.ahtw_128, i.ahtw_64,
+           i.wta_block_iters, i.ahtw_block_iters);
   e->info_str = buf;
   return e->info_str.c_str();
 }
diff --git a/nmfconsensus_amd/csrc/nmfc_kernels.hpp b/nmfconsensus_amd/csrc/nmfc_kernels.hpp
--- a/nmfconsensus_amd/csrc/nmfc_kernels.hpp
+++ b/nmfconsensus_amd/csrc/nmfc_kernels.hpp
@@ -5,7 +5,9 @@
 #include <type_traits>
 
 #include "nmfc_tuning.hpp"
+#include "packing.hpp"
 #include "rmt.hpp"
+#include "sk_split.hpp"
 
 namespace nmfc {
 
@@ -13,7 +15,6 @@
 typedef double d2 __attribute__((ext_vector_type(2)));
 typedef unsigned int u32x2 __attribute__((__vector_size__(2 * sizeof(unsigned int))));
 
-constexpr int PANEL = 64;
 constexpr int BK = 32;
 constexpr int NT = 256;
 constexpr int KMAX = 16;
@@ -334,6 +335,30 @@
     return true;
   }
 
+  __device__ __forceinline__ void run_idle(const double* __restrict__ P, long ldp, const double* __restrict__ Q, long ldq,
+                                           int kbeg, int kend, char* __restrict__ smem) {
+    static_assert(NBUF >= 3, "the ring form of run()");
+    constexpr int D = NBUF - 1;
+    const int nst = (kend - kbeg) / BK2;
+    bind(P, ldp, Q, ldq, kend);
+    const uint32_t base = (uint32_t)(uintptr_t)smem;
+    const int npro = nst < D ? nst : D;
+    for (int q = 0; q < npro; ++q) issue(base + q * STAGE_BYTES, kbeg + q * BK2);
+    wait_stages<D - 1, 0>(npro - 1, false);
+    step_barrier();
+    int b = 0;
+    for (int s = 0; s + 1 < nst; ++s) {
+      if (s + D < nst) {
+        const int bd = (b + D >= NBUF) ? b + D - NBUF : b + D;
+        issue(base + bd * STAGE_BYTES, kbeg + (s + D) * BK2);
+      }
+      const int left = nst - s - 2;
+      wait_stages<D - 1, 0>(left < D - 1 ? left : D - 1, false);
+      step_barrier();
+      b = (b + 1 == NBUF) ? 0 : b + 1;
+    }
+  }
+
   template <int J, int XL>
   __device__ __forceinline__ static void wait_stages(int j, bool xl) {
     if (j >= J) {
@@ -354,20 +379,6 @@
     const int w = wave_id(), l = lane_id();
     return (w % WC) * (RQ / WC) + nb * 16 + (l & 15);
   }
-};
-
-struct RestartInfo {
-  int col0;
-  int k;
-  int rid;
-  int sq_off;
-};
-
-struct ColInfo {
-  int sq_off;
-  int lc0;
-  int k;
-  int rid;
 };
 
 __device__ __forceinline__ bool panel_live(const int* __restrict__ prb, const int* __restrict__ pre, int p,
@@ -403,7 +414,7 @@
                                                               const ColInfo* __restrict__ ci,
                                                               const int* __restrict__ stop_iter, double* __restrict__ Gpart,
                                                               long g_ld, long g_split, double* __restrict__ SWpart,
-                                                              long sw_total) {
+                                                              long sw_total, int pskip) {
   using T = GTile<64 * NPT, RQ, WR, WC, NBUF, ABLK, GREG, SPLIT>;
   static_assert(!GREG || (WR == NPT && GPW == 1 && GRAM && !GITEM), "register Gram: one panel per wave row");
   constexpr int NCAND = 7 * NPT;
@@ -523,6 +534,17 @@
     tl.gj = __builtin_amdgcn_readfirstlane(gj);
   }
   const double* P = W + (long)pg * 64 * NPT * m_pad + kbeg;
+  if constexpr (NPT > 1 && WR % NPT == 0 && NBUF >= 3) {
+    bool lv = live[0];
+#pragma unroll
+    for (int q = 1; q < NPT; ++q)
+      if ((w / WC) / (WR / NPT) == q) lv = live[q];
+    const bool idle = pskip && !lv && !gram && tl.gi < 0;
+    if (__builtin_amdgcn_readfirstlane((int)idle)) {
+      tl.run_idle(P, m_pad, Q, ldq, 0, kend - kbeg, smem);
+      return;
+    }
+  }
   auto lds_gram = [&](const char* stg) {
 #pragma unroll
     for (int x = 0; x < GPW; ++x) {
@@ -633,6 +655,9 @@
   int nsplit;
   unsigned* tcnt;
   int dp_xcd;
+  int pskip;
+  const int* pieces;
+  int maxp;
 };
 typedef const SkArgs __attribute__((address_space(4)))* SkArgsK;
 
@@ -744,11 +769,21 @@
     tl.gj = __builtin_amdgcn_readfirstlane(gj);
   }
   const double* P = W + (long)pg * 64 * NPT * m_pad + kbeg;
+  bool idle = false;
+  if constexpr (!LSUM) {
+    bool lv = live[0];
+#pragma unroll
+    for (int q = 1; q < NPT; ++q)
+      if (w / WC == q) lv = live[q];
+    idle = uni((int)(A->pskip && !lv && tl.gi < 0)) != 0;
+  }
   auto go = [&](auto gc) {
     tl.template run<0, 2, decltype(gc)::value>(P, m_pad, Q, ldq, BK2 * resume, BK2 * s1, smem, load_chains,
                                                [](const char*) {}, [] {});
   };
-  switch (tl.gi < 0 ? -1 : 4 * tl.gi + tl.gj) {
+  if (idle) {
+    tl.run_idle(P, m_pad, Q, ldq, BK2 * resume, BK2 * s1, smem);
+  } else switch (tl.gi < 0 ? -1 : 4 * tl.gi + tl.gj) {
     case 0: go(std::integral_constant<int, 0>{}); break;
     case 5: go(std::integral_constant<int, 5>{}); break;
     case 10: go(std::integral_constant<int, 10>{}); break;
@@ -764,12 +799,14 @@
     flags = A->flags;
     double* dst = fix + (long)r * SK_FIX + 4L * (64 * w);
     const int ln = lane();
-#pragma unroll
-    for (int mb = 0; mb < T::MB; ++mb)
-#pragma unroll
-      for (int nb = 0; nb < T::NB; ++nb)
-        *reinterpret_cast<d4*>(dst + ((long)(mb * T::NB + nb) * SK_THREADS + ln) * 4) = tl.acc[mb][nb];
-    *reinterpret_cast<d4*>(dst + ((long)T::MB * T::NB * SK_THREADS + ln) * 4) = tl.gacc;
+    if (!idle) {
+#pragma unroll
+      for (int mb = 0; mb < T::MB; ++mb)
+#pragma unroll
+        for (int nb = 0; nb < T::NB; ++nb)
+          *reinterpret_cast<d4*>(dst + ((long)(mb * T::NB + nb) * SK_THREADS + ln) * 4) = tl.acc[mb][nb];
+      *reinterpret_cast<d4*>(dst + ((long)T::MB * T::NB * SK_THREADS + ln) * 4) = tl.gacc;
+    }
     asm volatile("s_waitcnt vmcnt(0)" ::: "memory");
     __syncthreads();
     if (w == 0 && ln == 0) {
@@ -779,6 +816,7 @@
     }
     return;
   }
+  if (idle) return;
   A = sk_args();
   const long g_ld = A->g_ld, g_split = A->g_split;
   double* out = A->Gpart + (long)s * g_split + (long)pg * 64 * NPT * g_ld + (long)t * RQ;
@@ -863,56 +901,13 @@
   __shared__ __attribute__((aligned(1024))) char smem[T::LDS_BYTES + 128];
   (void)args;
   SkArgsK A = sk_args();
-  const int nsplit = A->nsplit;
   const int G = gridDim.x;
   const int r = __builtin_amdgcn_readfirstlane(xcd_item(blockIdx.x, G));
-  const int xq = G >> 3, xrem = G & 7, xcd = blockIdx.x & 7;
-  const int xc = xq + (xcd < xrem ? 1 : 0), xb = xcd < xrem ? xcd * (xq + 1) : xrem * (xq + 1) + (xcd - xrem) * xq;
-  const int ipc = A->ngroups * A->ntj;
-  const int nitems = nsplit * ipc;
-  const int nst_full = A->kchunk / BK2;
-  const int nst_last = (int)((A->m_pad - (long)(nsplit - 1) * A->kchunk) / BK2);
-  const int nst_max = nsplit > 1 ? nst_full : nst_last;
-  const int c_last = ipc * (nsplit - 1);
-  auto nst_of = [&](int item) { return item >= c_last ? nst_last : nst_full; };
-  auto off = [&](int item) -> long {
-    return item <= c_last ? (long)item * nst_full : (long)c_last * nst_full + (long)(item - c_last) * nst_last;
-  };
-  auto locate = [&](long x, int& item, int& st) {
-    const long lc = (long)c_last * nst_full;
-    const int it = x < lc ? (int)(x / nst_full) : c_last + (int)((x - lc) / nst_last);
-    item = __builtin_amdgcn_readfirstlane(it);
-    st = __builtin_amdgcn_readfirstlane((int)(x - off(it)));
-  };
-  int D = (nitems / G - 1) * G;
-  if (D < 0) D = 0;
-  while (D > 0 && off(nitems) - off(D) < (long)G * nst_max) D -= G;
-  D = __builtin_amdgcn_readfirstlane(D);
-  const long base = off(D), S = off(nitems) - base;
-  const long b = base + S * r / G, e = base + S * (r + 1) / G;
-  int ib, sb, ie, se;
-  locate(b, ib, sb);
-  locate(e - 1, ie, se);
-  ++se;
-  const bool head = sb > 0;
-  const bool tail = se < nst_of(ie);
-  const int f0 = head ? ib + 1 : ib, f1 = tail ? ie - 1 : ie;
-  const int nfull = f1 >= f0 ? f1 - f0 + 1 : 0;
-  const int ndp = D / G;
-  const int t0 = tail ? 1 : 0;
-  const int npieces = t0 + ndp + nfull + (head ? 1 : 0);
+  const int npieces = uni(A->pieces[(long)r * (4 + 4 * A->maxp)]);
   for (int pc = 0; pc < npieces; ++pc) {
-    int item, s0, s1, mode;
-    if (pc < ndp) {
-      item = A->dp_xcd ? ndp * xb + pc * xc + (r - xb) : pc * G + r;
-      s0 = 0, s1 = nst_of(item), mode = 0;
-    } else if (pc < ndp + t0) {
-      item = ie, s0 = 0, s1 = se, mode = 1;
-    } else if (head && pc == npieces - 1) {
-      item = ib, s0 = sb, s1 = nst_of(ib), mode = 2;
-    } else {
-      item = f0 + pc - t0 - ndp, s0 = 0, s1 = nst_of(item), mode = 0;
-    }
+    SkArgsK B = sk_args();
+    const int* e = B->pieces + (long)r * (4 + 4 * B->maxp) + 4 + 4 * pc;
+    const int item = e[0], s0 = e[1], s1 = e[2], mode = e[3];
     __syncthreads();
     wta_sk_piece<NBUF, NOWAIT, LSUM, NPT>(r, item, s0, s1, mode, smem);
   }
@@ -1471,16 +1466,7 @@
 constexpr int SMALL_PF = NMFC_SMALL_PF;
 constexpr int SMALL_FPF = NMFC_SMALL_FPF;
 constexpr int SMALL_NW = 4;
-constexpr int SMALL_MAXR = 8;
 constexpr int SMALL_GGMAX = 4;
-
-struct SmallBlock {
-  int col0;
-  int nr;
-  int rid[SMALL_MAXR];
-  int k[SMALL_MAXR];
-  int lc0[SMALL_MAXR];
-};
 
 struct SoloJob {
   int col0, k, rid, pad;
diff --git a/nmfconsensus_amd/csrc/packing.hpp b/nmfconsensus_amd/csrc/packing.hpp
--- /dev/null
+++ b/nmfconsensus_amd/csrc/packing.hpp
@@ -0,0 +1,204 @@
+#pragma once
+
+#include <algorithm>
+#include <vector>
+
+namespace nmfc {
+
+constexpr int PANEL = 64;
+
+struct RestartInfo {
+  int col0;
+  int k;
+  int rid;
+  int sq_off;
+};
+
+struct ColInfo {
+  int sq_off;
+  int lc0;
+  int k;
+  int rid;
+};
+
+constexpr int SMALL_MAXR = 8;
+
+struct SmallBlock {
+  int col0;
+  int nr;
+  int rid[SMALL_MAXR];
+  int k[SMALL_MAXR];
+  int lc0[SMALL_MAXR];
+};
+
+}
+
+namespace nmfc_host {
+
+using nmfc::ColInfo;
+using nmfc::PANEL;
+using nmfc::RestartInfo;
+using nmfc::SmallBlock;
+
+constexpr int WTA_NPT = 4;
+
+struct Packing {
+  std::vector<RestartInfo> ri;
+  std::vector<int> prb, pre;
+  std::vector<ColInfo> ci;
+  int npanels = 0;
+};
+
+using Blocks = std::vector<std::vector<RestartInfo>>;
+
+inline std::vector<RestartInfo> pack_order(const std::vector<RestartInfo>& in) {
+  std::vector<RestartInfo> srt(in);
+  std::stable_sort(srt.begin(), srt.end(), [](const RestartInfo& a, const RestartInfo& b) {
+    return a.k != b.k ? a.k > b.k : a.rid < b.rid;
+  });
+  return srt;
+}
+
+inline Blocks place_ffd(const std::vector<RestartInfo>& srt) {
+  std::vector<int> fill;
+  Blocks members;
+  size_t first_open = 0;
+  for (const RestartInfo& r : srt) {
+    size_t b = first_open;
+    while (b < fill.size() && fill[b] + r.k > 16) ++b;
+    if (b == fill.size()) {
+      fill.push_back(0);
+      members.emplace_back();
+    }
+    fill[b] += r.k;
+    members[b].push_back(r);
+    while (first_open < fill.size() && fill[first_open] > 14) ++first_open;
+  }
+  return members;
+}
+
+inline bool fill_exactly(int target, int maxpart, int (&cnt)[17], std::vector<int>& parts) {
+  if (target == 0) return true;
+  for (int p = std::min(maxpart, target); p >= 2; --p) {
+    if (!cnt[p]) continue;
+    --cnt[p];
+    parts.push_back(p);
+    if (fill_exactly(target - p, p, cnt, parts)) return true;
+    parts.pop_back();
+    ++cnt[p];
+  }
+  return false;
+}
+
+inline Blocks place_tight(const std::vector<RestartInfo>& srt) {
+  int cnt[17] = {0};
+  size_t next[17];
+  for (size_t i = srt.size(); i-- > 0;) {
+    ++cnt[srt[i].k];
+    next[srt[i].k] = i;
+  }
+  Blocks members;
+  std::vector<int> parts;
+  for (int kmax = 16; kmax >= 2;) {
+    if (!cnt[kmax]) {
+      --kmax;
+      continue;
+    }
+    parts.assign(1, kmax);
+    --cnt[kmax];
+    for (int target = 16 - kmax; target >= 2; --target)
+      if (fill_exactly(target, 16, cnt, parts)) break;
+    members.emplace_back();
+    for (int p : parts) members.back().push_back(srt[next[p]++]);
+  }
+  return members;
+}
+
+inline bool pack_supported_ks(const std::vector<RestartInfo>& in) {
+  for (const RestartInfo& r : in)
+    if (r.k < 2 || r.k > 16) return false;
+  return true;
+}
+
+inline Packing pack(const std::vector<RestartInfo>& in, bool tight = true) {
+  const std::vector<RestartInfo> srt = pack_order(in);
+  Blocks members = place_ffd(srt);
+  if (tight && pack_supported_ks(in)) {
+    Blocks t = place_tight(srt);
+    if (t.size() < members.size()) members.swap(t);
+  }
+  const int nblocks = (int)members.size();
+  Packing pk;
+  pk.npanels = std::max(1, (nblocks + 3) / 4);
+  for (int p = 0; p < pk.npanels; ++p) {
+    pk.prb.push_back((int)pk.ri.size());
+    for (int b = 4 * p; b < std::min(nblocks, 4 * p + 4); ++b) {
+      int fill = 0;
+      for (RestartInfo r : members[b]) {
+        r.col0 = b * 16 + fill;
+        fill += r.k;
+        pk.ri.push_back(r);
+      }
+    }
+    pk.pre.push_back((int)pk.ri.size());
+  }
+  while (pk.npanels % WTA_NPT) {
+    pk.prb.push_back((int)in.size());
+    pk.pre.push_back((int)in.size());
+    ++pk.npanels;
+  }
+  pk.ci.assign((size_t)pk.npanels * PANEL, ColInfo{0, 0, 0, 0});
+  for (const RestartInfo& r : pk.ri)
+    for (int a = 0; a < r.k; ++a) pk.ci[r.col0 + a] = ColInfo{r.sq_off, r.col0 % PANEL, r.k, r.rid};
+  return pk;
+}
+
+inline int narrow_blocks(const Packing& pk, int maxb) {
+  if (pk.ri.empty()) return 0;
+  int nb = 0;
+  for (const RestartInfo& r : pk.ri) {
+    if (r.col0 / 16 != (r.col0 + r.k - 1) / 16) return 0;
+    nb = std::max(nb, (r.col0 + r.k + 15) / 16);
+  }
+  return nb <= maxb ? nb : 0;
+}
+
+inline Packing pack_small(const std::vector<RestartInfo>& in, std::vector<SmallBlock>& blocks) {
+  const std::vector<RestartInfo> srt = pack_order(in);
+  std::vector<int> fill;
+  blocks.clear();
+  Packing pk;
+  for (RestartInfo r : srt) {
+    size_t b = 0;
+    while (b < fill.size() && (fill[b] + r.k > 16 || blocks[b].nr == nmfc::SMALL_MAXR)) ++b;
+    if (b == fill.size()) {
+      fill.push_back(0);
+      SmallBlock sb{};
+      sb.col0 = (int)b * 16;
+      blocks.push_back(sb);
+    }
+    SmallBlock& sb = blocks[b];
+    r.col0 = sb.col0 + fill[b];
+    sb.rid[sb.nr] = r.rid;
+    sb.k[sb.nr] = r.k;
+    sb.lc0[sb.nr] = fill[b];
+    ++sb.nr;
+    fill[b] += r.k;
+    pk.ri.push_back(r);
+  }
+  pk.npanels = std::max(1, (int)((blocks.size() * 16 + PANEL - 1) / PANEL));
+  while (pk.npanels % WTA_NPT) ++pk.npanels;
+  pk.prb.assign(pk.npanels, 0);
+  pk.pre.assign(pk.npanels, 0);
+  pk.ci.assign((size_t)pk.npanels * PANEL, ColInfo{0, 0, 0, 0});
+  return pk;
+}
+
+inline int live_panels(const Packing& pk) {
+  int np = 0;
+  for (int p = 0; p < pk.npanels; ++p)
+    if (pk.pre[p] > pk.prb[p]) np = p + 1;
+  return np;
+}
+
+}
diff --git a/nmfconsensus_amd/csrc/sk_split.hpp b/nmfconsensus_amd/csrc/sk_split.hpp
--- /dev/null
+++ b/nmfconsensus_amd/csrc/sk_split.hpp
@@ -0,0 +1,169 @@
+#pragma once
+
+#define SK_HD inline
+
+namespace nmfc {
+
+struct SkShape {
+  int ng, ntj, nsplit;
+  int nst_full, nst_last;
+  int npt, last_w;
+  int G;
+};
+
+struct SkRange {
+  int D;
+  int ib, sb, ie, se;
+};
+
+SK_HD int sk_ngf(const SkShape& h) { return h.last_w < h.npt ? h.ng - 1 : h.ng; }
+SK_HD int sk_nitems(const SkShape& h) { return h.nsplit * h.ng * h.ntj; }
+SK_HD int sk_nst_max(const SkShape& h) { return h.nsplit > 1 ? h.nst_full : h.nst_last; }
+SK_HD int sk_nfull(const SkShape& h) { return h.nsplit * sk_ngf(h) * h.ntj; }
+SK_HD int sk_nlight(const SkShape& h) { return sk_nitems(h) - sk_nfull(h); }
+
+SK_HD long sk_wfull(const SkShape& h, int x) {
+  const int before_last = (h.nsplit - 1) * sk_ngf(h) * h.ntj;
+  const int a = x < before_last ? x : before_last;
+  return (long)h.npt * ((long)a * h.nst_full + (long)(x - a) * h.nst_last);
+}
+SK_HD long sk_wlight(const SkShape& h, int y) {
+  const int before_last = (h.nsplit - 1) * (h.ng - sk_ngf(h)) * h.ntj;
+  const int a = y < before_last ? y : before_last;
+  return (long)h.last_w * ((long)a * h.nst_full + (long)(y - a) * h.nst_last);
+}
+
+SK_HD void sk_class(const SkShape& h, int D, int v, bool& light, int& idx) {
+  light = false;
+  idx = v;
+  const int nl = sk_nlight(h);
+  if (v < D || nl == 0) return;
+  const int p = v - D, q = (sk_nfull(h) - D) / nl;
+  if (p >= nl * (q + 1)) {
+    idx = D + p - nl;
+    return;
+  }
+  const int g = p / (q + 1), within = p % (q + 1);
+  light = within == q;
+  idx = light ? g : D + g * q + within;
+}
+
+SK_HD long sk_voff(const SkShape& h, int D, int v) {
+  if (v >= sk_nitems(h)) return sk_wfull(h, sk_nfull(h)) + sk_wlight(h, sk_nlight(h));
+  bool light;
+  int idx;
+  sk_class(h, D, v, light, idx);
+  if (v < D || sk_nlight(h) == 0) return sk_wfull(h, idx);
+  const int p = v - D;
+  return light ? sk_wfull(h, D + p - idx) + sk_wlight(h, idx) : sk_wfull(h, idx) + sk_wlight(h, p - (idx - D));
+}
+
+SK_HD int sk_nst_of(const SkShape& h, int D, int v) {
+  bool light;
+  int idx;
+  sk_class(h, D, v, light, idx);
+  const int per_chunk = (light ? h.ng - sk_ngf(h) : sk_ngf(h)) * h.ntj;
+  return idx < (h.nsplit - 1) * per_chunk ? h.nst_full : h.nst_last;
+}
+
+SK_HD int sk_item(const SkShape& h, int D, int v) {
+  bool light;
+  int idx;
+  sk_class(h, D, v, light, idx);
+  const int ipc = h.ng * h.ntj, nfpc = sk_ngf(h) * h.ntj;
+  return light ? idx / h.ntj * ipc + nfpc + idx % h.ntj : idx / nfpc * ipc + idx % nfpc;
+}
+
+SK_HD void sk_locate(const SkShape& h, int D, long x, int& item, int& st) {
+  int lo = D, hi = sk_nitems(h);
+  while (lo < hi) {
+    const int mid = lo + (hi - lo + 1) / 2;
+    if (sk_voff(h, D, mid) <= x)
+      lo = mid;
+    else
+      hi = mid - 1;
+  }
+  item = lo;
+  st = 0;
+  if (lo < sk_nitems(h)) {
+    bool light;
+    int idx;
+    sk_class(h, D, lo, light, idx);
+    st = (int)((x - sk_voff(h, D, lo)) / (light ? h.last_w : h.npt));
+  }
+}
+
+SK_HD SkRange sk_range(const SkShape& h, int r) {
+  const int G = h.G, nitems = sk_nitems(h);
+  const long total = sk_voff(h, 0, nitems), need = (long)G * h.npt * sk_nst_max(h);
+  SkRange g;
+  int D = (nitems / G - 1) * G;
+  const int dmax = sk_nfull(h) / G * G;
+  if (D > dmax) D = dmax;
+  if (D < 0) D = 0;
+  while (D > 0 && total - sk_wfull(h, D) < need) D -= G;
+  g.D = D;
+  const long base = sk_wfull(h, D), S = total - base;
+  sk_locate(h, D, base + S * r / G, g.ib, g.sb);
+  sk_locate(h, D, base + S * (r + 1) / G, g.ie, g.se);
+  if (g.se == 0) {
+    --g.ie;
+    g.se = sk_nst_of(h, D, g.ie);
+  }
+  return g;
+}
+
+SK_HD int sk_npieces(const SkShape& h, const SkRange& g) {
+  const bool head = g.sb > 0, tail = g.se < sk_nst_of(h, g.D, g.ie);
+  const int f0 = head ? g.ib + 1 : g.ib, f1 = tail ? g.ie - 1 : g.ie;
+  return (tail ? 1 : 0) + g.D / h.G + (f1 >= f0 ? f1 - f0 + 1 : 0) + (head ? 1 : 0);
+}
+
+SK_HD void sk_piece(const SkShape& h, const SkRange& g, int r, int pc, int& v, int& s0, int& s1, int& mode) {
+  const bool head = g.sb > 0, tail = g.se < sk_nst_of(h, g.D, g.ie);
+  const int f0 = head ? g.ib + 1 : g.ib;
+  const int ndp = g.D / h.G, t0 = tail ? 1 : 0;
+  if (pc < ndp) {
+    v = pc * h.G + r;
+    s0 = 0, s1 = sk_nst_of(h, g.D, v), mode = 0;
+  } else if (pc < ndp + t0) {
+    v = g.ie, s0 = 0, s1 = g.se, mode = 1;
+  } else if (head && pc == sk_npieces(h, g) - 1) {
+    v = g.ib, s0 = g.sb, s1 = sk_nst_of(h, g.D, g.ib), mode = 2;
+  } else {
+    v = f0 + pc - t0 - ndp;
+    s0 = 0, s1 = sk_nst_of(h, g.D, v), mode = 0;
+  }
+}
+
+inline int sk_table(const SkShape& h, int dp_xcd, int* table, int maxp) {
+  int most = 0;
+  for (int r = 0; r < h.G; ++r) {
+    const SkRange g = sk_range(h, r);
+    const int np = sk_npieces(h, g), ndp = g.D / h.G;
+    most = np > most ? np : most;
+    if (!table) continue;
+    int* row = table + (long)r * (4 + 4 * maxp);
+    row[0] = np, row[1] = row[2] = row[3] = 0;
+    int xb = 0, xc = h.G;
+    for (int x = 0, b = 0; x < 8; ++x) {
+      const int c = h.G / 8 + (x < h.G % 8 ? 1 : 0);
+      if (r >= b && r < b + c) xb = b, xc = c;
+      b += c;
+    }
+    for (int pc = 0; pc < np && pc < maxp; ++pc) {
+      int v, s0, s1, mode;
+      sk_piece(h, g, r, pc, v, s0, s1, mode);
+      if (pc < ndp && dp_xcd) v = ndp * xb + pc * xc + (r - xb), s1 = sk_nst_of(h, g.D, v);
+      int* e = row + 4 + 4 * pc;
+      e[0] = sk_item(h, g.D, v), e[1] = s0, e[2] = s1, e[3] = mode;
+    }
+  }
+  return most;
+}
+
+SK_HD bool sk_fits(const SkShape& h) {
+  return sk_nitems(h) >= h.G && sk_voff(h, 0, sk_nitems(h)) >= (long)h.G * h.npt * sk_nst_max(h);
+}
+
+}
```

Result: no change. 503.0 (median of 6 runs) (+0.9%).
